# wjmaddox/online_gp

Measured on AMD Instinct MI355X. Metric: streaming updates/sec (WISKI, 50^3 inducing grid), higher is better.
Workload: dtype f32

## Files before the change

include/wiski.h:

```cpp
#ifndef WISKI_H
#define WISKI_H

#include <stdint.h>

#ifdef __cplusplus
extern "C" {
#endif

#define WISKI_OK 0
#define WISKI_E_BADARG (-1)
#define WISKI_E_LAUNCH (-2)
#define WISKI_E_WORKSPACE (-3)
#define WISKI_E_NOTCONV (-4)
#define WISKI_PENDING 1

#define WISKI_MAX_DIM 4

typedef struct wiski_grid {
  int32_t d;
  int32_t g[WISKI_MAX_DIM];
  double g0[WISKI_MAX_DIM];
  double h[WISKI_MAX_DIM];
} wiski_grid;

int wiski_version(void);
int wiski_side_stream_create(int32_t lowest_priority, void** out);

int wiski_interp_f32(const wiski_grid* grid, const float* d_x, int64_t n, int32_t* d_idx, float* d_val, int32_t* d_err, void* stream);
int wiski_interp_f64(const wiski_grid* grid, const double* d_x, int64_t n, int32_t* d_idx, double* d_val, int32_t* d_err, void* stream);

int wiski_gather_f32(const wiski_grid* grid, const float* d_x, int64_t n, const float* d_V, int32_t k, int32_t diag, float* d_out, int32_t* d_err, void* stream);
int wiski_gather_f64(const wiski_grid* grid, const double* d_x, int64_t n, const double* d_V, int32_t k, int32_t diag, double* d_out, int32_t* d_err, void* stream);

int wiski_gather_grad_f32(const wiski_grid* grid, const float* d_x, int64_t n, const float* d_V, int32_t diag, float* d_out, void* stream);
int wiski_gather_grad_f64(const wiski_grid* grid, const double* d_x, int64_t n, const double* d_V, int32_t diag, double* d_out, void* stream);

int wiski_gather_rows_f32(const wiski_grid* grid, const float* d_x, int64_t n, const float* d_Vr, int32_t ncols, float* d_out, int32_t* d_err, void* stream);
int wiski_gather_rows_f64(const wiski_grid* grid, const double* d_x, int64_t n, const double* d_Vr, int32_t ncols, double* d_out, int32_t* d_err, void* stream);
int wiski_gather_rows_vjp_f32(const wiski_grid* grid, const float* d_x, int64_t n, const float* d_Vr, int32_t ncols, const float* d_G, float* d_gx, void* stream);
int wiski_gather_rows_vjp_f64(const wiski_grid* grid, const double* d_x, int64_t n, const double* d_Vr, int32_t ncols, const double* d_G, double* d_gx, void* stream);
int wiski_interp_bilinear_f32(const wiski_grid* grid, const float* d_A, int64_t lda, const float* d_xL, int32_t qL, const float* d_xR, int32_t qR, int64_t nbatch, float* d_out, int32_t* d_err, void* stream);
int wiski_interp_bilinear_f64(const wiski_grid* grid, const double* d_A, int64_t lda, const double* d_xL, int32_t qL, const double* d_xR, int32_t qR, int64_t nbatch, double* d_out, int32_t* d_err, void* stream);
int wiski_interp_bilinear_vjp_f32(const wiski_grid* grid, const float* d_A, int64_t lda, const float* d_xL, int32_t qL, const float* d_xR, int32_t qR, int64_t nbatch, const float* d_G, float* d_gxL, float* d_gxR, void* stream);
int wiski_interp_bilinear_vjp_f64(const wiski_grid* grid, const double* d_A, int64_t lda, const double* d_xL, int32_t qL, const double* d_xR, int32_t qR, int64_t nbatch, const double* d_G, double* d_gxL, double* d_gxR, void* stream);

int wiski_gather_ell_f32(const int32_t* d_idx, const float* d_val, int64_t n, int32_t T, const float* d_v, float* d_out, void* stream);
int wiski_gather_ell_f64(const int32_t* d_idx, const double* d_val, int64_t n, int32_t T, const double* d_v, double* d_out, void* stream);
int wiski_gather_ell_grid_f32(const wiski_grid* grid, const int32_t* d_idx, const float* d_val, int64_t n, const float* d_v, float* d_vpack, float* d_out, void* stream);
int wiski_gather_ell_grid_f64(const wiski_grid* grid, const int32_t* d_idx, const double* d_val, int64_t n, const double* d_v, double* d_vpack, double* d_out, void* stream);
int64_t wiski_gather_ell_pack_elems(const wiski_grid* grid);

int wiski_scatter_stats_f32(const wiski_grid* grid, const float* d_x, const float* d_y, const float* d_wa, const float* d_wb, const float* d_noise, int64_t n, float* d_b, float* d_A_st, double* d_stats, int32_t* d_err, void* stream);
int wiski_scatter_stats_f64(const wiski_grid* grid, const double* d_x, const double* d_y, const double* d_wa, const double* d_wb, const double* d_noise, int64_t n, double* d_b, double* d_A_st, double* d_stats, int32_t* d_err, void* stream);

int wiski_scatter_stats_sym_f32(const wiski_grid* grid, const float* d_x, const float* d_y, const float* d_wa, const float* d_wb, const float* d_noise, int64_t n, float* d_b, float* d_A_half, double* d_stats, int32_t* d_err, void* stream);
int wiski_scatter_stats_sym_f64(const wiski_grid* grid, const double* d_x, const double* d_y, const double* d_wa, const double* d_wb, const double* d_noise, int64_t n, double* d_b, double* d_A_half, double* d_stats, int32_t* d_err, void* stream);
int wiski_scatter_stats_cnt_f32(const wiski_grid* grid, const float* d_x, const float* d_y, const float* d_wa, const float* d_wb, const float* d_noise, int64_t n, float* d_b, float* d_A, int32_t half, float* d_cnt, const float* d_u, float* d_res, double* d_stats, int32_t* d_err, void* stream);
int wiski_scatter_stats_cnt_f64(const wiski_grid* grid, const double* d_x, const double* d_y, const double* d_wa, const double* d_wb, const double* d_noise, int64_t n, double* d_b, double* d_A, int32_t half, double* d_cnt, const double* d_u, double* d_res, double* d_stats, int32_t* d_err, void* stream);
int wiski_stencil_expand_add_f32(const wiski_grid* grid, float* d_A_half, float* d_A_st, void* stream);
int wiski_stencil_expand_add_f64(const wiski_grid* grid, double* d_A_half, double* d_A_st, void* stream);

int wiski_wt_columns_f32(const wiski_grid* grid, const float* d_x, int64_t n, float* d_out, int32_t* d_err, void* stream);
int wiski_wt_columns_f64(const wiski_grid* grid, const double* d_x, int64_t n, double* d_out, int32_t* d_err, void* stream);

int wiski_jet_quadform_f32(const wiski_grid* grid, const float* d_x, int64_t n, const float* d_M, int64_t ldm, float* d_out, int32_t* d_err, void* stream);
int wiski_jet_quadform_f64(const wiski_grid* grid, const double* d_x, int64_t n, const double* d_M, int64_t ldm, double* d_out, int32_t* d_err, void* stream);
int wiski_wt_columns_jet_f32(const wiski_grid* grid, const float* d_x, int64_t n, float* d_out, int32_t* d_err, void* stream);
int wiski_wt_columns_jet_f64(const wiski_grid* grid, const double* d_x, int64_t n, double* d_out, int32_t* d_err, void* stream);
int wiski_gather_jet_f32(const wiski_grid* grid, const float* d_x, int64_t n, const float* d_V, int32_t k, int32_t rows_per_point, float* d_out, int32_t* d_err, void* stream);
int wiski_gather_jet_f64(const wiski_grid* grid, const double* d_x, int64_t n, const double* d_V, int32_t k, int32_t rows_per_point, double* d_out, int32_t* d_err, void* stream);

int wiski_stencil_spmv_f32(const wiski_grid* grid, const float* d_A_st, const float* d_V, int32_t k, const float* d_add, float beta, float* d_out, void* stream);
int wiski_stencil_spmv_f64(const wiski_grid* grid, const double* d_A_st, const double* d_V, int32_t k, const double* d_add, double beta, double* d_out, void* stream);
int wiski_stencil_spmv_sym_f32(const wiski_grid* grid, const float* d_A_half, const float* d_V, int32_t k, const float* d_add, float beta, float* d_out, void* stream);
int wiski_stencil_spmv_sym_f64(const wiski_grid* grid, const double* d_A_half, const double* d_V, int32_t k, const double* d_add, double beta, double* d_out, void* stream);

int wiski_kron_toeplitz_mm_f32(const wiski_grid* grid, const float* d_tcol, const float* d_V, int32_t k, float scale, float* d_tmp, float* d_out, void* stream);
int wiski_kron_toeplitz_mm_f64(const wiski_grid* grid, const double* d_tcol, const double* d_V, int32_t k, double scale, double* d_tmp, double* d_out, void* stream);

int wiski_kron_toeplitz_grad_f32(const wiski_grid* grid, const float* d_tcol, const float* d_X, const float* d_Y, int32_t k, float* d_tmp, double* d_grad, void* stream);
int wiski_kron_toeplitz_grad_f64(const wiski_grid* grid, const double* d_tcol, const double* d_X, const double* d_Y, int32_t k, double* d_tmp, double* d_grad, void* stream);

int wiski_kron_spectral_mm_f32(const wiski_grid* grid, const float* d_evec, const float* d_eval, float kscale, float shift, float pw, float rw, const float* d_V, int32_t k, float* d_tmp, float* d_out, void* stream);
int wiski_kron_spectral_mm_f64(const wiski_grid* grid, const double* d_evec, const double* d_eval, double kscale, double shift, double pw, double rw, const double* d_V, int32_t k, double* d_tmp, double* d_out, void* stream);

int64_t wiski_pcg_workspace_bytes(const wiski_grid* grid, int32_t k, int32_t max_iter, int32_t elem_size);
int wiski_pcg_f32(const wiski_grid* grid, const float* d_A_st, const float* d_tcol, float kscale, const float* d_evec, const float* d_evec2, const float* d_eval, float shift, const float* d_RHS, int32_t k, float* d_U, float* d_Z, int32_t warm, double tol, int32_t max_iter, int32_t check_every, int32_t first_check, void* d_work, int64_t work_bytes, int32_t* h_iters, double* h_relres, const int32_t* d_err, int32_t* h_err, int32_t a_sym, float* d_R, void* stream);
int wiski_pcg_f64(const wiski_grid* grid, const double* d_A_st, const double* d_tcol, double kscale, const double* d_evec, const double* d_evec2, const double* d_eval, double shift, const double* d_RHS, int32_t k, double* d_U, double* d_Z, int32_t warm, double tol, int32_t max_iter, int32_t check_every, int32_t first_check, void* d_work, int64_t work_bytes, int32_t* h_iters, double* h_relres, const int32_t* d_err, int32_t* h_err, int32_t a_sym, double* d_R, void* stream);

typedef int (*wiski_allreduce_fn)(void* ctx, void* d_vec, int64_t n_vec, int32_t elem_bytes, double* d_dots, int64_t n_dots, void* stream);
typedef struct wiski_shard {
  int32_t rank, nranks;
  void* comm;
  wiski_allreduce_fn allreduce;
  void* ctx;
} wiski_shard;
int wiski_shard_groups(int32_t d, int32_t rank, int32_t nranks, int32_t* g_lo, int32_t* g_hi);

typedef struct wiski_twolevel {
  int32_t r;
  int32_t nslab;
  const uint64_t* d_mask;
  const int32_t* d_off;
  const uint16_t* d_pos;
  const float* d_N;
  uint64_t* d_cs;
  float* d_mc;
  int32_t mc_cols;
} wiski_twolevel;

typedef struct wiski_pcg_async {
  int32_t state;
  int32_t it;
  int64_t seq;
  void* poll;
  int32_t prezeroed;
  int32_t guard_ok;
  double shift;
} wiski_pcg_async;
int wiski_pcg_async_f32(const wiski_grid* grid, const float* d_A_st, const float* d_tcol, float kscale, const float* d_evec, const float* d_evec2, const float* d_eval, float shift, const float* d_RHS, int32_t k, float* d_U, float* d_Z, int32_t warm, double tol, int32_t max_iter, int32_t check_every, int32_t first_check, void* d_work, int64_t work_bytes, int32_t* h_iters, double* h_relres, const int32_t* d_err, int32_t* h_err, int32_t a_sym, float* d_R, void* stream, wiski_pcg_async* handle, int32_t mode);
int wiski_pcg_async_f64(const wiski_grid* grid, const double* d_A_st, const double* d_tcol, double kscale, const double* d_evec, const double* d_evec2, const double* d_eval, double shift, const double* d_RHS, int32_t k, double* d_U, double* d_Z, int32_t warm, double tol, int32_t max_iter, int32_t check_every, int32_t first_check, void* d_work, int64_t work_bytes, int32_t* h_iters, double* h_relres, const int32_t* d_err, int32_t* h_err, int32_t a_sym, double* d_R, void* stream, wiski_pcg_async* handle, int32_t mode);
int wiski_pcg_async_free(wiski_pcg_async* handle);
int wiski_pcg_async_guard(const wiski_pcg_async* handle, const void** d_guard, int64_t* expect);
int wiski_pcg_zero_regions_f32(const wiski_grid* grid, int32_t k, int32_t max_iter, void* d_work, int32_t a_sym, void** p1, int64_t* n1_bytes, void** p2, int64_t* n2_bytes);
int wiski_pcg_zero_regions_f64(const wiski_grid* grid, int32_t k, int32_t max_iter, void* d_work, int32_t a_sym, void** p1, int64_t* n1_bytes, void** p2, int64_t* n2_bytes);
int64_t wiski_scatter_bin_bytes(const wiski_grid* grid, int64_t n, int32_t elem_size);
int wiski_scatter_stats_step_f32(const wiski_grid* grid, const float* d_x, const float* d_y, const float* d_wa, const float* d_wb, const float* d_noise, int64_t n, float* d_b, float* d_A_half, float* d_cnt, const float* d_u, float* d_res, float* d_mean_out, double* d_stats, int32_t* d_err, void* z1, int64_t n1_bytes, void* z2, int64_t n2_bytes, const void* d_guard, int64_t guard_expect, void* d_bin, int64_t bin_bytes, void* stream);
int wiski_scatter_stats_step_f64(const wiski_grid* grid, const double* d_x, const double* d_y, const double* d_wa, const double* d_wb, const double* d_noise, int64_t n, double* d_b, double* d_A_half, double* d_cnt, const double* d_u, double* d_res, double* d_mean_out, double* d_stats, int32_t* d_err, void* z1, int64_t n1_bytes, void* z2, int64_t n2_bytes, const void* d_guard, int64_t guard_expect, void* d_bin, int64_t bin_bytes, void* stream);
int wiski_gather_zero_f32(const wiski_grid* grid, const float* d_x, int64_t n, const float* d_V, int32_t k, float* d_out, int32_t* d_err, void* z1, int64_t n1_bytes, void* z2, int64_t n2_bytes, int32_t* zeroed, void* stream);
int wiski_gather_zero_f64(const wiski_grid* grid, const double* d_x, int64_t n, const double* d_V, int32_t k, double* d_out, int32_t* d_err, void* z1, int64_t n1_bytes, void* z2, int64_t n2_bytes, int32_t* zeroed, void* stream);

typedef struct wiski_stream_args_f32 {
  float* d_A_half; float* d_b; float* d_cnt; double* d_stats; int32_t* d_err;
  float* d_U; float* d_Z; float* d_R;
  const float* d_tcol; float kscale; const float* d_evec; const float* d_evec2; const float* d_eval; float shift;
  double tol; int32_t max_iter; int32_t check_every; void* d_work; int64_t work_bytes;
  void* d_bin; int64_t bin_bytes;
  const wiski_shard* shard;
  const wiski_twolevel* two_level;
  int32_t keep[3];
} wiski_stream_args_f32;
typedef struct wiski_stream_args_f64 {
  double* d_A_half; double* d_b; double* d_cnt; double* d_stats; int32_t* d_err;
  double* d_U; double* d_Z; double* d_R;
  const double* d_tcol; double kscale; const double* d_evec; const double* d_evec2; const double* d_eval; double shift;
  double tol; int32_t max_iter; int32_t check_every; void* d_work; int64_t work_bytes;
  void* d_bin; int64_t bin_bytes;
  const wiski_shard* shard;
  const wiski_twolevel* two_level;
  int32_t keep[3];
} wiski_stream_args_f64;
int wiski_stream_step_f32(const wiski_grid* grid, const wiski_stream_args_f32* args, const float* d_x, const float* d_y, const float* d_wa, const float* d_wb, const float* d_noise, int64_t q, float* d_mean_out, int32_t carry, int32_t first_check, int32_t* h_iters, double* h_relres, int32_t* h_err, void* stream, wiski_pcg_async* handle, int32_t defer, int32_t* h_resumed);
int wiski_stream_step_f64(const wiski_grid* grid, const wiski_stream_args_f64* args, const double* d_x, const double* d_y, const double* d_wa, const double* d_wb, const double* d_noise, int64_t q, double* d_mean_out, int32_t carry, int32_t first_check, int32_t* h_iters, double* h_relres, int32_t* h_err, void* stream, wiski_pcg_async* handle, int32_t defer, int32_t* h_resumed);

int wiski_scatter_stats_multi_f32(const wiski_grid* grid, const float* d_x, const float* d_y, const float* d_wa, const float* d_wb, const float* d_noise, int64_t n, int32_t nout, int64_t y_stride, int64_t w_stride, float* d_b, float* d_A_half, int64_t A_stride, float* d_cnt, const float* d_u, float* d_res, double* d_stats, int32_t* d_err, void* stream);
int wiski_scatter_stats_multi_f64(const wiski_grid* grid, const double* d_x, const double* d_y, const double* d_wa, const double* d_wb, const double* d_noise, int64_t n, int32_t nout, int64_t y_stride, int64_t w_stride, double* d_b, double* d_A_half, int64_t A_stride, double* d_cnt, const double* d_u, double* d_res, double* d_stats, int32_t* d_err, void* stream);

int wiski_scatter_stats_grad_f32(const wiski_grid* grid, const float* d_x, const float* d_y, const float* d_wa, const float* d_wb, const float* d_noise, int64_t n, float* d_b, float* d_A_half, float* d_cnt, const float* d_u, float* d_res, float* d_mean_out, double* d_stats, int32_t* d_err, void* stream);
int wiski_scatter_stats_grad_f64(const wiski_grid* grid, const double* d_x, const double* d_y, const double* d_wa, const double* d_wb, const double* d_noise, int64_t n, double* d_b, double* d_A_half, double* d_cnt, const double* d_u, double* d_res, double* d_mean_out, double* d_stats, int32_t* d_err, void* stream);

typedef struct wiski_absorb_args {
  const void* d_x; const void* d_y; const void* d_wa; const void* d_wb; const void* d_noise; int64_t n;
  void* d_b; void* d_A; int32_t half; int32_t channels; void* d_cnt; double* d_stats; int32_t* d_err;
  const void* d_u; void* d_res; void* d_mean_out;
  void* z1; int64_t n1_bytes; void* z2; int64_t n2_bytes;
  const void* d_guard; int64_t guard_expect;
  void* d_bin; int64_t bin_bytes;
  int32_t g_lo; int32_t g_hi; int32_t nout; int32_t reserved;
  int64_t y_stride; int64_t w_stride; int64_t A_stride;
} wiski_absorb_args;
int wiski_absorb_f32(const wiski_grid* grid, const wiski_absorb_args* args, void* stream);
int wiski_absorb_f64(const wiski_grid* grid, const wiski_absorb_args* args, void* stream);

int wiski_scatter_stats_robust_f32(const wiski_grid* grid, const float* d_x, const float* d_y, const float* d_wa, const float* d_wb, const float* d_noise, int64_t n, float* d_b, float* d_A_half, float* d_cnt, const float* d_u, float* d_res, float* d_mean_out, double* d_stats, int32_t* d_err, const float* d_inv_scale, float huber_c, float* d_omega_out, void* stream);
int wiski_scatter_stats_robust_f64(const wiski_grid* grid, const double* d_x, const double* d_y, const double* d_wa, const double* d_wb, const double* d_noise, int64_t n, double* d_b, double* d_A_half, double* d_cnt, const double* d_u, double* d_res, double* d_mean_out, double* d_stats, int32_t* d_err, const double* d_inv_scale, double huber_c, double* d_omega_out, void* stream);
int wiski_absorb_robust_f32(const wiski_grid* grid, const wiski_absorb_args* args, const float* d_inv_scale, float huber_c, float* d_omega_out, void* stream);
int wiski_absorb_robust_f64(const wiski_grid* grid, const wiski_absorb_args* args, const double* d_inv_scale, double huber_c, double* d_omega_out, void* stream);

typedef struct wiski_window_ring {
  void* d_x; void* d_y; void* d_wa; void* d_wb; void* d_noise;
  int64_t cap; int64_t head;
} wiski_window_ring;
int wiski_scatter_stats_window_f32(const wiski_grid* grid, const float* d_x, const float* d_y, const float* d_wa, const float* d_wb, const float* d_noise, int64_t n, const wiski_window_ring* ring, float* d_b, float* d_A_half, float* d_cnt, const float* d_u, float* d_res, float* d_mean_out, double* d_stats, int32_t* d_err, int32_t* d_void_left, void* stream);
int wiski_scatter_stats_window_f64(const wiski_grid* grid, const double* d_x, const double* d_y, const double* d_wa, const double* d_wb, const double* d_noise, int64_t n, const wiski_window_ring* ring, double* d_b, double* d_A_half, double* d_cnt, const double* d_u, double* d_res, double* d_mean_out, double* d_stats, int32_t* d_err, int32_t* d_void_left, void* stream);
int wiski_absorb_window_f32(const wiski_grid* grid, const wiski_absorb_args* args, const wiski_window_ring* ring, int32_t* d_void_left, void* stream);
int wiski_absorb_window_f64(const wiski_grid* grid, const wiski_absorb_args* args, const wiski_window_ring* ring, int32_t* d_void_left, void* stream);

int wiski_scatter_stats_step_sharded_f32(const wiski_grid* grid, const float* d_x, const float* d_y, const float* d_wa, const float* d_wb, const float* d_noise, int64_t n, float* d_b, float* d_A_half, float* d_cnt, const float* d_u, float* d_res, float* d_mean_out, double* d_stats, int32_t* d_err, void* z1, int64_t n1_bytes, void* z2, int64_t n2_bytes, const void* d_guard, int64_t guard_expect, int32_t g_lo, int32_t g_hi, void* stream);
int wiski_scatter_stats_step_sharded_f64(const wiski_grid* grid, const double* d_x, const double* d_y, const double* d_wa, const double* d_wb, const double* d_noise, int64_t n, double* d_b, double* d_A_half, double* d_cnt, const double* d_u, double* d_res, double* d_mean_out, double* d_stats, int32_t* d_err, void* z1, int64_t n1_bytes, void* z2, int64_t n2_bytes, const void* d_guard, int64_t guard_expect, int32_t g_lo, int32_t g_hi, void* stream);
int wiski_pcg_sharded_f32(const wiski_grid* grid, const float* d_A_st, const float* d_tcol, float kscale, const float* d_evec, const float* d_evec2, const float* d_eval, float shift, const float* d_RHS, int32_t k, float* d_U, float* d_Z, int32_t warm, double tol, int32_t max_iter, int32_t check_every, int32_t first_check, void* d_work, int64_t work_bytes, int32_t* h_iters, double* h_relres, const int32_t* d_err, int32_t* h_err, int32_t a_sym, float* d_R, void* stream, wiski_pcg_async* handle, int32_t mode, const wiski_shard* shard);
int wiski_pcg_sharded_f64(const wiski_grid* grid, const double* d_A_st, const double* d_tcol, double kscale, const double* d_evec, const double* d_evec2, const double* d_eval, double shift, const double* d_RHS, int32_t k, double* d_U, double* d_Z, int32_t warm, double tol, int32_t max_iter, int32_t check_every, int32_t first_check, void* d_work, int64_t work_bytes, int32_t* h_iters, double* h_relres, const int32_t* d_err, int32_t* h_err, int32_t a_sym, double* d_R, void* stream, wiski_pcg_async* handle, int32_t mode, const wiski_shard* shard);
int wiski_pcg_twolevel_f32(const wiski_grid* grid, const float* d_A_st, const float* d_tcol, float kscale, const float* d_evec, const float* d_evec2, const float* d_eval, float shift, const float* d_RHS, int32_t k, float* d_U, float* d_Z, int32_t warm, double tol, int32_t max_iter, int32_t check_every, int32_t first_check, void* d_work, int64_t work_bytes, int32_t* h_iters, double* h_relres, const int32_t* d_err, int32_t* h_err, int32_t a_sym, float* d_R, void* stream, wiski_pcg_async* handle, int32_t mode, const wiski_shard* shard, const wiski_twolevel* two_level);
int64_t wiski_twolevel_refresh_workspace_bytes(int32_t r);
int wiski_twolevel_refresh_f32(const wiski_grid* grid, const float* d_x, int64_t n, const float* d_scale, const double* d_V, int32_t kw, const int32_t* d_S, int32_t r, const double* d_lam_unit, double kscale, double gscale, double* d_G, void* d_work, int64_t work_bytes, float* d_N, const uint64_t* d_sticky, int32_t* d_bad, void* stream);
int wiski_precond_apply_f32(const wiski_grid* grid, const float* d_evec, const float* d_evec2, const float* d_eval, float kscale, float shift, const float* d_r, float* d_w0, float* d_w1, float* d_y, float* d_t, double* d_rho, const wiski_twolevel* two_level, void* stream);
int wiski_precond_apply_keep_f32(const wiski_grid* grid, const float* d_evec, const float* d_evec2, const float* d_eval, float kscale, float shift, const float* d_r, float* d_w0, float* d_w1, float* d_y, float* d_t, double* d_rho, const wiski_twolevel* two_level, const int32_t* keep, void* stream);
int wiski_precond_keep_ok(const wiski_grid* grid, const int32_t* keep, int32_t with_two_level);
int wiski_precond_apply_cols_f32(const wiski_grid* grid, const float* d_evec, const float* d_evec2, const float* d_eval, float kscale, float shift, const float* d_r, int32_t k, float* d_w0, float* d_w1, float* d_y, float* d_t, double* d_rho, const wiski_twolevel* two_level, void* stream);

int wiski_gemm_f32(int32_t ta, int32_t tb, int32_t M, int32_t N, int32_t K, float alpha, const float* d_A, int32_t lda, const float* d_B, int32_t ldb, float beta, float* d_C, int32_t ldc, void* stream);
int wiski_gemm_f64(int32_t ta, int32_t tb, int32_t M, int32_t N, int32_t K, double alpha, const double* d_A, int32_t lda, const double* d_B, int32_t ldb, double beta, double* d_C, int32_t ldc, void* stream);
int wiski_potrf_f32(int32_t n, float* d_A, int32_t lda, int32_t* d_info, void* stream);
int wiski_potrf_f64(int32_t n, double* d_A, int32_t lda, int32_t* d_info, void* stream);
int wiski_potrf_inverse_f32(int32_t n, float* d_A, int32_t lda, float* d_X, int32_t ldx, int32_t* d_info, void* stream);
int wiski_potrf_inverse_f64(int32_t n, double* d_A, int32_t lda, double* d_X, int32_t ldx, int32_t* d_info, void* stream);
int wiski_trsm_f32(int32_t trans, int32_t n, int32_t nrhs, const float* d_L, int32_t ldl, float* d_B, int32_t ldb, void* stream);
int wiski_trsm_f64(int32_t trans, int32_t n, int32_t nrhs, const double* d_L, int32_t ldl, double* d_B, int32_t ldb, void* stream);
int wiski_logdiag_f32(int32_t n, const float* d_A, int32_t lda, double* d_out, void* stream);
int wiski_logdiag_f64(int32_t n, const double* d_A, int32_t lda, double* d_out, void* stream);

int wiski_dense_factor_f32(const wiski_grid* grid, const float* d_A_half, const float* d_evec, const float* d_eval, float kscale, float* d_work, int64_t work_elems, float* d_chol, float* d_M, double* d_logdiag, int32_t* d_info, void* stream);
int wiski_dense_factor_f64(const wiski_grid* grid, const double* d_A_half, const double* d_evec, const double* d_eval, double kscale, double* d_work, int64_t work_elems, double* d_chol, double* d_M, double* d_logdiag, int32_t* d_info, void* stream);

int64_t wiski_root_update_workspace_elems(int32_t m, int32_t r, int32_t q);
int wiski_root_update_f32(int32_t m, int32_t r, int32_t q, float* d_L, int32_t ldl, float* d_R, int32_t ldr, const float* d_V, int32_t ldv, float* d_ws, int64_t ws_elems, void* stream);
int wiski_root_update_f64(int32_t m, int32_t r, int32_t q, double* d_L, int32_t ldl, double* d_R, int32_t ldr, const double* d_V, int32_t ldv, double* d_ws, int64_t ws_elems, void* stream);

int wiski_basis_project_f32(const wiski_grid* grid, const float* d_x, int64_t n, const double* d_V, int32_t kmax, const int32_t* d_S, int32_t r, const float* d_scale, const double* d_colscale, const double* d_tcol, double* d_F, int64_t ldf, double* d_prior, int32_t* d_err, void* stream);
int wiski_basis_project_f64(const wiski_grid* grid, const double* d_x, int64_t n, const double* d_V, int32_t kmax, const int32_t* d_S, int32_t r, const double* d_scale, const double* d_colscale, const double* d_tcol, double* d_F, int64_t ldf, double* d_prior, int32_t* d_err, void* stream);
int wiski_basis_project_vjp_f32(const wiski_grid* grid, const float* d_x, int64_t n, const double* d_V, int32_t kmax, const int32_t* d_S, int32_t r, const float* d_scale, const double* d_colscale, const double* d_tcol, const double* d_GF, int64_t ldg, const double* d_Gprior, float* d_gx, void* stream);
int wiski_basis_project_vjp_f64(const wiski_grid* grid, const double* d_x, int64_t n, const double* d_V, int32_t kmax, const int32_t* d_S, int32_t r, const double* d_scale, const double* d_colscale, const double* d_tcol, const double* d_GF, int64_t ldg, const double* d_Gprior, double* d_gx, void* stream);
int wiski_basis_absorb_h_f32(int64_t n, int32_t r, const double* d_F, int64_t ldf, const float* d_wby, const float* d_scale, double* d_h, void* stream);
int wiski_basis_absorb_h_f64(int64_t n, int32_t r, const double* d_F, int64_t ldf, const double* d_wby, const double* d_scale, double* d_h, void* stream);
int wiski_factor_refresh_layout(int32_t d, int64_t nV, int32_t kw, int32_t r_ref, int32_t r, int64_t* off);
int wiski_factor_refresh(int32_t d, const int32_t* d_g, int64_t nV, const double* d_tcol, const double* d_Vin, int32_t kw, int32_t kuse, const double* d_Vref, int32_t kref, int32_t niter, double resid_ok, const int32_t* d_Sref, const int32_t* d_S, int32_t r_ref, int32_t r, double* d_work, double* d_verdict, const double* d_Gref, const double* d_href, double kscale, int32_t* d_info, double* d_out, void* verdict_event, void* stream);
int wiski_basis_pair_reduce(int32_t d, int32_t r, int32_t kmax, const double* d_Wt, const int32_t* d_S, const double* d_ev, double* d_D, void* stream);
int wiski_basis_eig_update(int32_t d, const int32_t* d_g, const double* d_tcol, const double* d_Vin, int32_t kw, int32_t kuse, double* d_Vout, double* d_ev, double* d_resid,
                           const double* d_Vref, int32_t kref, double* d_Tq, void* stream);
int wiski_basis_eig_update_adaptive(int32_t d, const int32_t* d_g, const double* d_tcol, const double* d_Vin, int32_t kw, int32_t kuse, double* d_Vout, double* d_ev, double* d_resid, const double* d_Vref, int32_t kref, double* d_Tq, int32_t niter, double resid_ok, void* stream);
int wiski_basis_change(int32_t d, const int32_t* d_g, int32_t kref, int32_t kw, int32_t r_ref, int32_t r, const double* d_Tq, const int32_t* d_Sref, const int32_t* d_S, const double* d_ev, const double* d_tcol, const double* d_resid, double* d_TS, double* d_lam, double* d_work, double* d_verdict, void* stream);
int wiski_basis_lag_grad(int32_t d, const int32_t* d_g, int32_t kw, const double* d_V, const double* d_D, double scale, const double* d_scale, double* d_out, void* stream);
int wiski_spectral_var(int32_t n, int32_t r, const double* d_Y, const double* d_F, const double* d_prior, double kscale, double* d_diag, double* d_tail, void* stream);
#define WISKI_HYPER_MAX_PARAMS 6
typedef struct {
  void* raw;
  void* exp_avg;
  void* exp_avg_sq;
  void* step;
  int32_t numel;
  int32_t step_numel;
  int32_t role;
  int32_t kind;
  double lower, upper;
} wiski_hyper_param;
typedef struct {
  int32_t count;
  int32_t reserved;
  wiski_hyper_param p[WISKI_HYPER_MAX_PARAMS];
} wiski_hyper_plan;
int wiski_hyper_columns_f32(const wiski_hyper_plan* plan, const wiski_grid* grid, int32_t kind, float* d_ell, float* d_scale, float* d_s2, double* d_s2_f64, double* d_tcol64, float* d_tcol, void* stream);
int wiski_hyper_columns_f64(const wiski_hyper_plan* plan, const wiski_grid* grid, int32_t kind, double* d_ell, double* d_scale, double* d_s2, double* d_s2_f64, double* d_tcol64, double* d_tcol, void* stream);
int wiski_hyper_mid_f32(const double* d_bMb, const double* d_logdet, const float* d_s2, const double* d_c, const double* d_ld, const double* d_n, double* d_out, double* d_loss, void* stream);
int wiski_hyper_mid_f64(const double* d_bMb, const double* d_logdet, const double* d_s2, const double* d_c, const double* d_ld, const double* d_n, double* d_out, double* d_loss, void* stream);
int wiski_hyper_adam_f32(const wiski_hyper_plan* plan, const float* d_scale, const float* d_s2, const float* d_gell, const float* d_gscale, const double* d_mid, const double* d_gkap, const double* d_n, double lr, double beta1, double beta2, double eps, void* stream);
int wiski_hyper_adam_f64(const wiski_hyper_plan* plan, const double* d_scale, const double* d_s2, const double* d_gell, const double* d_gscale, const double* d_mid, const double* d_gkap, const double* d_n, double lr, double beta1, double beta2, double eps, void* stream);
#define WISKI_COPY_MAX_SEGMENTS 12
typedef struct {
  const void* src[WISKI_COPY_MAX_SEGMENTS];
  void* dst[WISKI_COPY_MAX_SEGMENTS];
  int64_t n[WISKI_COPY_MAX_SEGMENTS];
  int32_t count;
  int32_t reserved;
  double scalar;
  void* scalar_dst;
} wiski_copy_plan;
int wiski_multi_copy_f64(const wiski_copy_plan* plan, void* stream);
int wiski_spectral_evaluate_f32(int32_t n, int32_t r, const double* d_F, const double* d_prior, const double* d_Linv, int32_t ldl, const double* d_t, double kscale, const float* d_s2, const float* d_y, const int32_t* d_err, double* d_ws, double* d_out, float* d_mean, float* d_var, void* stream);
int wiski_spectral_evaluate_f64(int32_t n, int32_t r, const double* d_F, const double* d_prior, const double* d_Linv, int32_t ldl, const double* d_t, double kscale, const double* d_s2, const double* d_y, const int32_t* d_err, double* d_ws, double* d_out, double* d_mean, double* d_var, void* stream);
int wiski_spectral_evaluate_y_f32(int32_t n, int32_t r, const double* d_Y, const double* d_F, const double* d_prior, const double* d_t, double kscale, const float* d_s2, const float* d_y, const int32_t* d_err, double* d_ws, double* d_out, float* d_mean, float* d_var, void* stream);
int wiski_spectral_evaluate_y_f64(int32_t n, int32_t r, const double* d_Y, const double* d_F, const double* d_prior, const double* d_t, double kscale, const double* d_s2, const double* d_y, const int32_t* d_err, double* d_ws, double* d_out, double* d_mean, double* d_var, void* stream);
int wiski_factor_tail(int32_t r_ref, int32_t r, const double* d_TS, const double* d_href, const double* d_sq, const double* d_Linv, const double* d_chol, double* d_out, void* stream);
int wiski_woodbury_c(int32_t r, const double* d_G, const double* d_lam_kuu, double kscale, double* d_C, double* d_lam, double* d_sq, double* d_sqG, void* stream);
int wiski_mll_weights(int32_t r, const double* d_G, const double* d_P, const double* d_zeta, const double* d_lam_kuu, const double* d_gb, const double* d_gld, double* d_Wt, double* d_gkap, void* stream);

int wiski_comm_unique_id_bytes(void);
int wiski_comm_unique_id(void* id_out);
int wiski_comm_init_rank(const void* id_bytes, int32_t nranks, int32_t rank, void** comm_out);
int wiski_comm_destroy(void* comm);
int wiski_comm_info(void* comm, int32_t* version_out, int32_t* nranks_out, int32_t* rank_out);
int wiski_allreduce_stats_f32(void* comm, float* d_half, int64_t n_half, float* d_b, int64_t n_b, float* d_cnt, int64_t n_cnt, double* d_scal, int64_t n_scal, void* stream);
int wiski_allreduce_stats_f64(void* comm, double* d_half, int64_t n_half, double* d_b, int64_t n_b, double* d_cnt, int64_t n_cnt, double* d_scal, int64_t n_scal, void* stream);

int wiski_read_flag(const int32_t* d_flag, int32_t* h_value, void* stream);

int wiski_prof_start(int32_t max_launches);
int wiski_prof_stop(double* total_ms, int64_t* launches);
int wiski_prof_stamps(double* total_ms, int64_t* launches, double* each_us, int64_t each_cap);
int wiski_prof_stamps_raw(int64_t i, uint64_t* pairs, int64_t cap, int64_t* nwaves);
int wiski_prof_enable(int32_t on);
int wiski_prof_empty(int32_t n, double* avg_us, void* stream);

int wiski_stationary_columns_f32(const wiski_grid* grid, int32_t kind, const float* d_ell, int32_t nell, const float* d_scale, double* d_out, void* stream);
int wiski_stationary_columns_f64(const wiski_grid* grid, int32_t kind, const double* d_ell, int32_t nell, const double* d_scale, double* d_out, void* stream);
int wiski_stationary_columns_grad_f32(const wiski_grid* grid, int32_t kind, const float* d_ell, int32_t nell, const float* d_scale, const double* d_gout, float* d_gell, float* d_gscale, void* stream);
int wiski_stationary_columns_grad_f64(const wiski_grid* grid, int32_t kind, const double* d_ell, int32_t nell, const double* d_scale, const double* d_gout, double* d_gell, double* d_gscale, void* stream);
int wiski_mll_value_f32(const double* d_bMb, const double* d_logdet, const float* d_s2, const double* d_c, const double* d_ld, double n, const double* d_n, double* d_val, double* d_coef, void* stream);
int wiski_mll_value_f64(const double* d_bMb, const double* d_logdet, const double* d_s2, const double* d_c, const double* d_ld, double n, const double* d_n, double* d_val, double* d_coef, void* stream);
int wiski_mll_s2_grad_f32(const double* d_g, const double* d_coef, const float* d_s2, double n, const double* d_n, const double* d_gkap, float* d_gs2, void* stream);
int wiski_mll_s2_grad_f64(const double* d_g, const double* d_coef, const double* d_s2, double n, const double* d_n, const double* d_gkap, double* d_gs2, void* stream);
int wiski_gaussian_metrics_f32(int64_t n, const float* d_mu, const float* d_var, const float* d_y, const float* d_add_var, float* d_out, void* stream);
int wiski_gaussian_metrics_f64(int64_t n, const double* d_mu, const double* d_var, const double* d_y, const double* d_add_var, double* d_out, void* stream);

int wiski_scatter_probes_f32(const wiski_grid* grid, const float* d_x, const float* d_wa, int64_t q, int64_t first_index, uint64_t seed, int32_t S, float* d_P, int32_t* d_err, void* stream);
// ... 32 lines not shown
```

online_gp_amd/csrc/pcg.h:

```cpp
#pragma once
#include "wiski_common.h"

template <typename real>
struct PcgArgs {
  const real* A = nullptr;
  bool a_sym = false;
  const real* RHS = nullptr;
  int k = 0;
  const real* tcol = nullptr;
  real kscale = (real)0;
  const real* evec = nullptr;
  const real* evec2 = nullptr;
  const real* eval = nullptr;
  real shift = (real)0;
  const wiski_twolevel* two_level = nullptr;
  int keep[3] = {0, 0, 0};
  real* U = nullptr;
  real* Z = nullptr;
  real* R = nullptr;
  int warm = 0;
  double tol = 0;
  int max_iter = 0;
  int check_every = 0;
  int first_check = 0;
  void* work = nullptr;
  int64_t work_bytes = 0;
  int32_t* h_iters = nullptr;
  double* h_relres = nullptr;
  const int32_t* d_err = nullptr;
  int32_t* h_err = nullptr;
  wiski_pcg_async* handle = nullptr;
  int mode = 0;
  const wiski_shard* shard = nullptr;
};

template <typename real>
struct PcgLayout {
  static constexpr int SLOTS = 20;
  static int64_t align(int64_t v) { return (v + 255) / 256 * 256; }
  static int64_t bytes(int m, int k, int max_iter, int elem_size = (int)sizeof(real)) {
    return SLOTS * align((int64_t)k * m * elem_size) + align(PcgScal::doubles(k, max_iter) * 8);
  }
  real *r, *y, *p, *pt, *hp, *tmp;
  real* part;
  real* ty;
  real *sa, *sb;
  PcgScal S;
  int64_t km;
  int64_t nscal;
  PcgLayout(int m, int k, int max_iter, void* work) : km((int64_t)k * m), nscal(PcgScal::doubles(k, max_iter)) {
    char* w = static_cast<char*>(work);
    const int64_t vec = align(km * (int64_t)sizeof(real));
    auto at = [&](int slot) { return reinterpret_cast<real*>(w + slot * vec); };
    r = at(0); y = at(1); p = at(2); pt = at(3); hp = at(4); tmp = at(5); part = at(6); ty = at(14); sa = at(16); sb = at(18);
    double* base = reinterpret_cast<double*>(at(SLOTS));
    S = PcgScal{base, k, base + PcgScal::scalars(k, max_iter)};
  }
  double* zero1() const { return S.base; }
  int64_t zero1_count() const { return nscal; }
  real* zero2(int nch) const { return part + (int64_t)(nch > 0 ? nch - 1 : 0) * km; }
  int64_t zero2_count(int zl) const { return zl ? km : 0; }
};

template <typename real>
int pcg(const wiski_grid* grid, const PcgArgs<real>& args, void* stream);

template <typename real>
int pcg_zero_regions(const wiski_grid* grid, int k, int max_iter, void* work, bool a_sym, void** p1, int64_t* n1_bytes, void** p2, int64_t* n2_bytes);
int pcg_guard(const wiski_pcg_async* handle, const void** d_guard, int64_t* expect);
```

online_gp_amd/csrc/solve.hip:

```cpp
#include "pcg.h"

#include <hip/hip_ext.h>

#include <chrono>
#include <cstdlib>
#include <map>
#include <mutex>
#include <vector>

static struct WiskiProf {
  bool on = false;
  bool armed = false;
  std::vector<hipEvent_t> ev;
  size_t used = 0;
  unsigned long long* d_stamp = nullptr;
  size_t stamp_pairs = 0, stamp_used = 0;
  struct Span { size_t off, n; };
  std::vector<Span> spans;
} g_prof;
constexpr unsigned long long PROF_CLOCK_MASK = 0xffffffffffffull;
constexpr size_t PROF_STAMP_ARENA_PAIRS = (size_t)1 << 20;

extern "C" int wiski_prof_start(int max_launches) {
  if (max_launches < 1) return WISKI_E_BADARG;
  while (g_prof.ev.size() < (size_t)max_launches * 2) {
    hipEvent_t e;
    if (hipEventCreate(&e) != hipSuccess) return WISKI_E_LAUNCH;
    g_prof.ev.push_back(e);
  }
  if (!g_prof.d_stamp) {
    if (hipMalloc(&g_prof.d_stamp, PROF_STAMP_ARENA_PAIRS * 2 * sizeof(unsigned long long)) == hipSuccess) g_prof.stamp_pairs = PROF_STAMP_ARENA_PAIRS;
    else { (void)hipGetLastError(); g_prof.d_stamp = nullptr; }
  }
  if (g_prof.d_stamp && g_prof.stamp_used &&
      hipMemset(g_prof.d_stamp, 0, g_prof.stamp_used * 2 * sizeof(unsigned long long)) != hipSuccess) return WISKI_E_LAUNCH;
  if (g_prof.d_stamp && !g_prof.stamp_used && hipMemset(g_prof.d_stamp, 0, g_prof.stamp_pairs * 2 * sizeof(unsigned long long)) != hipSuccess) return WISKI_E_LAUNCH;
  g_prof.stamp_used = 0;
  g_prof.spans.clear();
  g_prof.used = 0;
  g_prof.on = true;
  g_prof.armed = true;
  return WISKI_OK;
}

extern "C" int wiski_prof_enable(int32_t on) {
  g_prof.on = on != 0;
  return WISKI_OK;
}

static inline unsigned long long* prof_stamp_pairs(size_t nwaves) {
  static const bool off = getenv("WISKI_PROF_NOSTAMP") != nullptr;
  if (off || !g_prof.armed || !g_prof.d_stamp || g_prof.stamp_used + nwaves > g_prof.stamp_pairs) return nullptr;
  g_prof.spans.push_back(WiskiProf::Span{g_prof.stamp_used, nwaves});
  g_prof.stamp_used += nwaves;
  return g_prof.d_stamp + 2 * g_prof.spans.back().off;
}

extern "C" int wiski_prof_stop(double* total_ms, int64_t* launches) {
  g_prof.on = false;
  g_prof.armed = false;
  double tot = 0;
  for (size_t i = 0; i + 1 < g_prof.used; i += 2) {
    float ms = 0;
    if (hipEventElapsedTime(&ms, g_prof.ev[i], g_prof.ev[i + 1]) != hipSuccess) return WISKI_E_LAUNCH;
    tot += ms;
  }
  if (total_ms) *total_ms = tot;
  if (launches) *launches = (int64_t)(g_prof.used / 2);
  g_prof.used = 0;
  return WISKI_OK;
}

extern "C" int wiski_prof_stamps(double* total_ms, int64_t* launches, double* each_us, int64_t each_cap) {
  const size_t nd = g_prof.spans.size();
  double tot = 0;
  int64_t cnt = 0;
  if (nd && g_prof.d_stamp && g_prof.stamp_used) {
    std::vector<unsigned long long> h(2 * g_prof.stamp_used);
    if (hipMemcpy(h.data(), g_prof.d_stamp, h.size() * sizeof(unsigned long long), hipMemcpyDeviceToHost) != hipSuccess) return WISKI_E_LAUNCH;
    for (size_t i = 0; i < nd; ++i) {
      const WiskiProf::Span sp = g_prof.spans[i];
      unsigned long long lo = ~0ull, hi = 0;
      for (size_t w = 0; w < sp.n; ++w) {
        unsigned long long b = h[2 * (sp.off + w)] & PROF_CLOCK_MASK, e = h[2 * (sp.off + w) + 1];
        if (!e) continue;
        if (e < b) e += PROF_CLOCK_MASK + 1;
        if (b < lo) lo = b;
        if (e > hi) hi = e;
      }
      if (hi > lo) {
        if (each_us && cnt < each_cap) each_us[cnt] = (double)(hi - lo) * 1e-2;
        tot += (double)(hi - lo) * 1e-5;
        ++cnt;
      }
    }
  }
  if (total_ms) *total_ms = tot;
  if (launches) *launches = cnt;
  return WISKI_OK;
}

extern "C" int wiski_prof_stamps_raw(int64_t i, uint64_t* pairs, int64_t cap, int64_t* nwaves) {
  if (!nwaves || i < 0) return WISKI_E_BADARG;
  *nwaves = 0;
  if ((size_t)i >= g_prof.spans.size() || !g_prof.d_stamp) return WISKI_OK;
  const WiskiProf::Span sp = g_prof.spans[(size_t)i];
  *nwaves = (int64_t)sp.n;
  if (!pairs || !sp.n) return WISKI_OK;
  const size_t n = (size_t)cap < sp.n ? (size_t)cap : sp.n;
  if (hipMemcpy(pairs, g_prof.d_stamp + 2 * sp.off, n * 2 * sizeof(unsigned long long), hipMemcpyDeviceToHost) != hipSuccess) return WISKI_E_LAUNCH;
  return WISKI_OK;
}

__global__ void k_prof_empty() {}
extern "C" int wiski_prof_empty(int32_t n, double* avg_us, void* stream) {
  if (n < 1 || !avg_us) return WISKI_E_BADARG;
  hipStream_t s = (hipStream_t)stream;
  std::vector<hipEvent_t> ev(2 * (size_t)n);
  for (auto& e : ev)
    if (hipEventCreate(&e) != hipSuccess) return WISKI_E_LAUNCH;
  for (int i = 0; i < n; ++i) hipExtLaunchKernelGGL(k_prof_empty, dim3(1), dim3(64), 0, s, ev[2 * i], ev[2 * i + 1], 0);
  int rc = hipStreamSynchronize(s) == hipSuccess ? WISKI_OK : WISKI_E_LAUNCH;
  double tot = 0;
  for (int i = 0; i < n && rc == WISKI_OK; ++i) {
    float ms = 0;
    if (hipEventElapsedTime(&ms, ev[2 * i], ev[2 * i + 1]) != hipSuccess) rc = WISKI_E_LAUNCH;
    tot += ms;
  }
  for (auto& e : ev) (void)hipEventDestroy(e);
  *avg_us = tot * 1e3 / n;
  return rc;
}

template <typename real, int KC, bool DOT>
__global__ __launch_bounds__(256) void k_stencil_spmv(GridDev<real> G, const real* __restrict__ A_st, const real* __restrict__ V,
                                                      int k, const real* __restrict__ add, real beta, real* __restrict__ out,
                                                      double* __restrict__ dots) {
  extern __shared__ __attribute__((aligned(16))) char smem[];
  int* s_off = reinterpret_cast<int*>(smem);
  const int R = G.R, m = G.m, d = G.d;
  for (int o = threadIdx.x; o < R; o += blockDim.x) {
    int rem = o, f = 0;
    for (int q = d - 1; q >= 0; --q) {
      int c = rem % 7;
      rem /= 7;
      f += (c - 3) * G.stride[q];
    }
    s_off[o] = f;
  }
  __syncthreads();
  const int i = blockIdx.x * blockDim.x + threadIdx.x;
  const int c0 = blockIdx.y * KC;
  real acc[KC];
#pragma unroll
  for (int c = 0; c < KC; ++c) acc[c] = (real)0;
  if (i < m) {
// ... 1349 lines not shown
        const Vec4<real> r4 = load4<real>(r + e);
        rr[0] = r4.x; rr[1] = r4.y; rr[2] = r4.z; rr[3] = r4.w;
      } else {
      Vec4<real> t4;
      t4.x = t4.y = t4.z = t4.w = (real)0;
      if (t) t4 = load4<real>(t + e);
      Vec4<real> pp[8];
#pragma unroll
      for (int ch = 0; ch < 8; ++ch)
        if (ch < nch) pp[ch] = load4<real>(part + (int64_t)ch * km + e);
      if (zl) store4<real>(part + (int64_t)(nch - 1) * km + e, (real)0, (real)0, (real)0, (real)0);
      rr[0] = f[0] - t4.x; rr[1] = f[1] - t4.y; rr[2] = f[2] - t4.z; rr[3] = f[3] - t4.w;
#pragma unroll
      for (int ch = 0; ch < 8; ++ch)
        if (ch < nch) { rr[0] -= pp[ch].x; rr[1] -= pp[ch].y; rr[2] -= pp[ch].z; rr[3] -= pp[ch].w; }
      store4<real>(r + e, rr[0], rr[1], rr[2], rr[3]);
      }
    } else {
      f[0] = rhs[e];
      if (given) {
        rr[0] = r[e];
      } else {
        rr[0] = t ? f[0] - t[e] : f[0];
        for (int ch = 0; ch < nch; ++ch) rr[0] -= part[(int64_t)ch * km + e];
        if (zl) part[(int64_t)(nch - 1) * km + e] = (real)0;
        r[e] = rr[0];
      }
    }
#pragma unroll
    for (int q = 0; q < VEC; ++q) {
      a += (double)f[q] * f[q];
      bsum += (double)rr[q] * rr[q];
    }
  }
  a = block_reduce_sum(a, s_red);
  bsum = block_reduce_sum(bsum, s_red);
  if (threadIdx.x == 0) {
    unsafeAtomicAdd(S.rn0() + c, a);
    unsafeAtomicAdd(S.rn(0) + c, bsum);
  }
}


template <typename real, int VEC>
__global__ __launch_bounds__(256) void k_pcg_update_p(int m, int it, double tol2, const real* __restrict__ y, const real* __restrict__ r,
                                                      real* __restrict__ p, real* __restrict__ pt, PcgScal S) {
  const int c = blockIdx.y;
  double beta = 0;
  if (it > 0) {
    const double den = S.rho(it - 1)[c];
    beta = den > 0 ? S.rho(it)[c] / den : 0;
  }
  const real bt = (real)beta;
  const int64_t cm = (int64_t)c * m;
  for (int i = (blockIdx.x * blockDim.x + threadIdx.x) * VEC; i < m; i += gridDim.x * blockDim.x * VEC) {
    real yv[VEC], rv[VEC], pv[VEC], ptv[VEC];
    if constexpr (VEC == 4) {
      const Vec4<real> a = load4<real>(y + cm + i), b = load4<real>(r + cm + i);
      yv[0] = a.x; yv[1] = a.y; yv[2] = a.z; yv[3] = a.w;
      rv[0] = b.x; rv[1] = b.y; rv[2] = b.z; rv[3] = b.w;
      if (it > 0) {
        const Vec4<real> cpp = load4<real>(p + cm + i), dpp = load4<real>(pt + cm + i);
        pv[0] = cpp.x; pv[1] = cpp.y; pv[2] = cpp.z; pv[3] = cpp.w;
        ptv[0] = dpp.x; ptv[1] = dpp.y; ptv[2] = dpp.z; ptv[3] = dpp.w;
      }
    } else {
      yv[0] = y[cm + i]; rv[0] = r[cm + i];
      if (it > 0) { pv[0] = p[cm + i]; ptv[0] = pt[cm + i]; }
    }
#pragma unroll
    for (int u = 0; u < VEC; ++u) {
      pv[u] = it == 0 ? yv[u] : yv[u] + bt * pv[u];
      ptv[u] = it == 0 ? rv[u] : rv[u] + bt * ptv[u];
    }
    if constexpr (VEC == 4) {
      store4<real>(p + cm + i, pv[0], pv[1], pv[2], pv[3]);
      store4<real>(pt + cm + i, ptv[0], ptv[1], ptv[2], ptv[3]);
    } else {
      p[cm + i] = pv[0]; pt[cm + i] = ptv[0];
    }
  }
}

template <typename real, int VEC>
__global__ __launch_bounds__(256) void k_pcg_update_x(int m, int it, double tol2, const real* __restrict__ p, const real* __restrict__ pt,
                                                      const real* __restrict__ hp, real* __restrict__ part, int nch, int zl,
                                                      real* __restrict__ u, real* __restrict__ z, real* __restrict__ r, PcgScal S,
                                                      double* __restrict__ poll = nullptr, const int32_t* __restrict__ err = nullptr,
                                                      long long seq = 0, long long* __restrict__ guard = nullptr) {
  __shared__ double s_red[16];
  const int c = blockIdx.y;
  double alpha = 0;
  const double den = S.php_sum(it, c);
  if (blockIdx.x == 0) pcg_dot_clear(S.php(it + 1), c, 1, S.k);
  if (pcg_active(S, it, c, tol2) && den > 0) alpha = S.rho(it)[c] / den;
  const real al = (real)alpha;
  double acc = 0;
  const int64_t cm = (int64_t)c * m;
  const int64_t km = (int64_t)S.k * m;
  for (int i = (blockIdx.x * blockDim.x + threadIdx.x) * VEC; i < m; i += gridDim.x * blockDim.x * VEC) {
    const int64_t e = cm + i;
    real pv[VEC], ptv[VEC], hv[VEC], uv[VEC], zv[VEC], rv[VEC];
    if constexpr (VEC == 4) {
      const Vec4<real> a = load4<real>(p + e), b = load4<real>(pt + e), cu = load4<real>(u + e), cz = load4<real>(z + e), cr = load4<real>(r + e);
      pv[0] = a.x; pv[1] = a.y; pv[2] = a.z; pv[3] = a.w;
      ptv[0] = b.x; ptv[1] = b.y; ptv[2] = b.z; ptv[3] = b.w;
      uv[0] = cu.x; uv[1] = cu.y; uv[2] = cu.z; uv[3] = cu.w;
      zv[0] = cz.x; zv[1] = cz.y; zv[2] = cz.z; zv[3] = cz.w;
      rv[0] = cr.x; rv[1] = cr.y; rv[2] = cr.z; rv[3] = cr.w;
      if (nch > 0) {
        Vec4<real> pp[8];
#pragma unroll
        for (int ch = 0; ch < 8; ++ch)
          if (ch < nch) pp[ch] = load4<real>(part + (int64_t)ch * km + e);
        if (zl) store4<real>(part + (int64_t)(nch - 1) * km + e, (real)0, (real)0, (real)0, (real)0);
#pragma unroll
        for (int q = 0; q < 4; ++q) hv[q] = ptv[q];
#pragma unroll
        for (int ch = 0; ch < 8; ++ch)
          if (ch < nch) { hv[0] += pp[ch].x; hv[1] += pp[ch].y; hv[2] += pp[ch].z; hv[3] += pp[ch].w; }
      } else {
        const Vec4<real> h4 = load4<real>(hp + e);
        hv[0] = h4.x; hv[1] = h4.y; hv[2] = h4.z; hv[3] = h4.w;
      }
    } else {
      pv[0] = p[e]; ptv[0] = pt[e]; uv[0] = u[e]; zv[0] = z[e]; rv[0] = r[e];
      if (nch > 0) {
        hv[0] = ptv[0];
        for (int ch = 0; ch < nch; ++ch) hv[0] += part[(int64_t)ch * km + e];
        if (zl) part[(int64_t)(nch - 1) * km + e] = (real)0;
      } else {
        hv[0] = hp[e];
      }
    }
#pragma unroll
    for (int q = 0; q < VEC; ++q) {
      uv[q] += al * pv[q];
      zv[q] += al * ptv[q];
      rv[q] -= al * hv[q];
      acc += (double)rv[q] * rv[q];
    }
    if constexpr (VEC == 4) {
      store4<real>(u + e, uv[0], uv[1], uv[2], uv[3]);
      store4<real>(z + e, zv[0], zv[1], zv[2], zv[3]);
      store4<real>(r + e, rv[0], rv[1], rv[2], rv[3]);
    } else {
      u[e] = uv[0]; z[e] = zv[0]; r[e] = rv[0];
    }
  }
  acc = block_reduce_sum(acc, s_red);
  if (poll == nullptr) {
    if (threadIdx.x == 0) unsafeAtomicAdd(S.rn(it + 1) + c, acc);
  } else {
    __shared__ int s_last;
    if (threadIdx.x == 0) {
      const double prev = atomicAdd(S.rn(it + 1) + c, acc);
      unsigned one = 1u;
      asm volatile("" : "+v"(one) : "v"(prev));
      const unsigned t = atomicAdd(S.ticket(), one);
      s_last = t == gridDim.x * gridDim.y - 1;
    }
    __syncthreads();
    if (s_last) {
      const int k = S.k;
      int ok = 1;
      for (int c2 = threadIdx.x; c2 < k; c2 += blockDim.x) {
        const double r0 = __hip_atomic_load(S.rn0() + c2, __ATOMIC_RELAXED, __HIP_MEMORY_SCOPE_AGENT);
        const double r1 = __hip_atomic_load(S.rn(it + 1) + c2, __ATOMIC_RELAXED, __HIP_MEMORY_SCOPE_AGENT);
        poll[1 + c2] = r0;
        poll[1 + k + c2] = r1;
        if (r0 > 0 && r1 > tol2 * r0) ok = 0;
      }
      ok = __syncthreads_and(ok);
      if (threadIdx.x == 0) {
        const double e = err ? (double)*err : 0.0;
        const long long gv = (ok && e == 0.0) ? seq : -seq;
        poll[1 + 2 * k] = e;
        poll[2 + 2 * k] = (double)gv;
        if (guard) *guard = gv;
        __hip_atomic_store(S.ticket(), 0u, __ATOMIC_RELAXED, __HIP_MEMORY_SCOPE_AGENT);
      }
      __threadfence_system();
      __syncthreads();
      if (threadIdx.x == 0) __hip_atomic_store(reinterpret_cast<long long*>(poll), seq, __ATOMIC_RELEASE, __HIP_MEMORY_SCOPE_SYSTEM);
    }
  }
}

template <typename real>
__global__ __launch_bounds__(256) void k_shard_reduce(int m4, int m, const real* __restrict__ part, int np, real* __restrict__ acc,
                                                      real* __restrict__ out) {
  for (int i = blockIdx.x * blockDim.x + threadIdx.x; i < m4; i += gridDim.x * blockDim.x) {
    Vec4<real> t = load4<real>(acc + 4 * i);
    for (int p = 0; p < np; ++p) {
      const Vec4<real> v = load4<real>(part + (int64_t)p * m + 4 * i);
      t.x += v.x; t.y += v.y; t.z += v.z; t.w += v.w;
    }
    store4<real>(out + 4 * i, t.x, t.y, t.z, t.w);
    store4<real>(acc + 4 * i, (real)0, (real)0, (real)0, (real)0);
  }
}


struct PcgPath {
  bool wide;
  bool sym;
  bool spectral;
  bool fused_cg;
  bool sharded;
  template <typename real>
  PcgPath(const GridDev<real>& G, const PcgArgs<real>& a)
      : wide(G.m % 4 == 0), sym(a.a_sym), spectral(a.evec != nullptr && a.eval != nullptr), fused_cg(spectral && wide && spectral_fused_ok<real>(G)),
        sharded(wiski_shard_active(a.shard)) {}
};

template <typename real>
static int pcg_validate(const GridDev<real>& G, const PcgArgs<real>& a, const PcgPath& path) {
  if (!a.A || !a.RHS || !a.U || !a.Z || !a.work || a.k < 1 || a.max_iter < 1) return WISKI_E_BADARG;
  if (a.mode != 0 && !a.handle) return WISKI_E_BADARG;
  if (a.mode == 2 && a.handle->state != 1) return WISKI_E_BADARG;
  if (!path.spectral && !a.tcol) return WISKI_E_BADARG;
  if (a.work_bytes < PcgLayout<real>::bytes(G.m, a.k, a.max_iter)) return WISKI_E_WORKSPACE;
  if (path.sharded) {
    if (!path.sym || !path.wide || a.k != 1 || a.shard->rank < 0 || a.shard->rank >= a.shard->nranks) return WISKI_E_BADARG;
    if (!a.shard->comm && !a.shard->allreduce) return WISKI_E_BADARG;
  }
  if (a.mode != 2 && a.warm == 2 && !a.R) return WISKI_E_BADARG;
  if (a.two_level && !(path.fused_cg && sizeof(real) == 4)) return WISKI_E_BADARG;
  if (a.keep[0] != 0 || a.keep[1] != 0 || a.keep[2] != 0) {
    if constexpr (sizeof(real) == 4) {
      if (!path.fused_cg || a.k != 1 || !spectral_keep_ok(G, a.keep, a.two_level != nullptr)) return WISKI_E_BADARG;
    } else {
      return WISKI_E_BADARG;
    }
  }
  return WISKI_OK;
}

template <typename real>
static int pcg_partials(const GridDev<real>& G, int k, bool sym, int* zl) {
  *zl = 0;
  if (G.m % 4 != 0) return 0;
  return sym ? sym_partials<real>(G, k, zl) : spmv_nch(G.d);
}

template <typename real>
struct PcgPlan {
  const GridDev<real>& G;
  const PcgArgs<real>& a;
  const PcgPath path;
  const hipStream_t s;
  const int m, k;
  const PcgLayout<real> L;
  real* r;
  int nch, zl;
  SymDmaParts stab{};
  int sh_lo = 0, sh_hi = 0;
  bool sh_dma = false;
  real* cpart;
  int cnch, czl;
  dim3 egrid, vgrid;
  const double tol2;
  bool init_in_fwd;

  PcgPlan(const GridDev<real>& G_, const PcgArgs<real>& a_, const PcgPath& path_, hipStream_t s_)
      : G(G_), a(a_), path(path_), s(s_), m(G_.m), k(a_.k), L(G_.m, a_.k, a_.max_iter, a_.work), tol2(a_.tol * a_.tol) {
    r = a.R ? a.R : L.r;
    nch = pcg_partials<real>(G, k, path.sym, &zl);
    if (path.sharded) {
      shard_group_range(sym_groups(G.d), a.shard->rank, a.shard->nranks, &sh_lo, &sh_hi);
      sh_dma = sym_use_dma<real>(G, k);
      if (sh_dma) shard_parts_d3(sh_lo, sh_hi, &stab);
    }
    cpart = path.sharded ? L.hp : L.part;
    cnch = path.sharded ? 1 : nch;
    czl = path.sharded ? 0 : zl;
    int bcap = m / 4096;
    bcap = bcap < 32 ? 32 : (bcap > 256 ? 256 : bcap);
    if (k < 16 && bcap < 1024 / k) bcap = 1024 / k;
    int eb = (m + 255) / 256;
    if (eb > bcap) eb = bcap;
    egrid = dim3((unsigned)eb, (unsigned)k);
    int vb = (m / 4 + 255) / 256;
    if (vb < 1) vb = 1;
    if (vb > bcap) vb = bcap;
    vgrid = dim3((unsigned)vb, (unsigned)k);
    init_in_fwd = a.mode != 2 && a.warm == 2 && sizeof(real) == 4 && path.fused_cg;
  }

  int product_wide(const real* v, const real* add, real beta, double* dots) const {
    real* part = L.part;
    if (!path.sharded)
      return path.sym ? launch_spmv4_sym<real>(G, a.A, v, k, part, add, beta, dots, s) : launch_spmv4<real>(G, a.A, v, k, part, add, beta, dots, s);
    int np = 0;
    if (sh_dma) {
      if (stab.n) {
        if (int r1 = launch_spmv4_sym<real>(G, a.A, v, k, part, add, beta, dots, s, &stab)) return r1;
      }
      np = stab.n;
    } else if (sh_hi > sh_lo) {
      if (int r1 = launch_spmv4_sym<real>(G, a.A, v, k, part, add, beta, dots, s, nullptr, sh_lo, sh_hi)) return r1;
      np = nch - 1;
    }
    const int m4 = m / 4;
    hipLaunchKernelGGL((k_shard_reduce<real>), dim3((unsigned)((m4 + 255) / 256)), dim3(256), 0, s, m4, m, (const real*)part, np,
                       part + (int64_t)(nch - 1) * k * m, L.hp);
    if (hipGetLastError() != hipSuccess) return WISKI_E_LAUNCH;
    const int64_t nd = dots ? (int64_t)k * PCG_DOT_COL : 0;
    const wiski_shard* shard = a.shard;
    if (shard->comm) {
      if constexpr (sizeof(real) == 4) return wiski_allreduce_stats_f32(shard->comm, nullptr, 0, (float*)L.hp, m, nullptr, 0, dots, nd, s);
      else return wiski_allreduce_stats_f64(shard->comm, nullptr, 0, (double*)L.hp, m, nullptr, 0, dots, nd, s);
    }
    return shard->allreduce(shard->ctx, L.hp, (int64_t)m, (int32_t)sizeof(real), dots, nd, s);
  }
  int product(const real* v, const real* add, real beta, double* dots) const {
    if (path.wide) return product_wide(v, add, beta, dots);
    return path.sym ? launch_spmv_sym<real>(G, a.A, v, k, add, beta, L.hp, dots, s) : launch_spmv<real>(G, a.A, v, k, add, beta, L.hp, dots, s);
  }
};

#define PCG_VEC_LAUNCH(plan, K, ...)                                                                          \
  do {                                                                                                        \
    if ((plan).path.wide) hipLaunchKernelGGL((K<real, 4>), (plan).vgrid, dim3(256), 0, (plan).s, __VA_ARGS__); \
    else hipLaunchKernelGGL((K<real, 1>), (plan).egrid, dim3(256), 0, (plan).s, __VA_ARGS__);                  \
  } while (0)

template <typename real>
static int pcg_start(const PcgPlan<real>& plan) {
  const PcgArgs<real>& a = plan.a;
  const PcgLayout<real>& L = plan.L;
  const hipStream_t s = plan.s;
  const int m = plan.m, k = plan.k;
  if (a.handle && a.handle->prezeroed) {
    a.handle->prezeroed = 0;
  } else {
    const int64_t nscal = L.zero1_count(), nvec = L.zero2_count(plan.zl);
    int64_t zb = ((nscal > nvec ? nscal : nvec) + 255) / 256;
    if (zb > 1024) zb = 1024;
    hipLaunchKernelGGL((k_pcg_zero<real>), dim3((unsigned)zb), dim3(256), 0, s, L.zero1(), nscal, L.zero2(plan.nch), nvec);
  }
  if (a.warm == 2 && plan.init_in_fwd) {
  } else if (a.warm == 2) {
    PCG_VEC_LAUNCH(plan, k_pcg_init, m, a.RHS, (const real*)nullptr, (real*)nullptr, 0, 0, 1, plan.r, L.S);
  } else if (a.warm) {
    if (plan.path.wide) {
      if (int rc = plan.product(a.U, nullptr, (real)0, nullptr)) return rc;
      hipLaunchKernelGGL((k_pcg_init<real, 4>), plan.vgrid, dim3(256), 0, s, m, a.RHS, (const real*)a.Z, plan.cpart, plan.cnch, plan.czl, 0, plan.r, L.S);
    } else {
      if (int rc = plan.product(a.U, a.Z, (real)1, nullptr)) return rc;
      hipLaunchKernelGGL((k_pcg_init<real, 1>), plan.egrid, dim3(256), 0, s, m, a.RHS, (const real*)L.hp, (real*)nullptr, 0, 0, 0, plan.r, L.S);
    }
  } else {
    if (hipMemsetAsync(a.U, 0, (size_t)k * m * sizeof(real), s) != hipSuccess) return WISKI_E_LAUNCH;
    if (hipMemsetAsync(a.Z, 0, (size_t)k * m * sizeof(real), s) != hipSuccess) return WISKI_E_LAUNCH;
    hipLaunchKernelGGL((k_pcg_init<real, 1>), plan.egrid, dim3(256), 0, s, m, a.RHS, (const real*)nullptr, (real*)nullptr, 0, 0, 0, plan.r, L.S);
  }
  return WISKI_OK;
}

template <typename real>
static int pcg_iterate(const PcgPlan<real>& plan) {
  const GridDev<real>& G = plan.G;
  const PcgArgs<real>& a = plan.a;
  const PcgLayout<real>& L = plan.L;
  const PcgScal& S = L.S;
  const hipStream_t s = plan.s;
  const int m = plan.m, k = plan.k, max_iter = a.max_iter;
  const double tol2 = plan.tol2;
  const bool spectral = plan.path.spectral;
  real *const r = plan.r, *const p = L.p, *const pt = L.pt, *const hp = L.hp, *const cpart = plan.cpart;
  const int cnch = plan.cnch, czl = plan.czl;
  wiski_pcg_async* const as = a.handle;
  int mode = a.mode, first_check = a.first_check;
  const int check_every = a.check_every < 1 ? 10 : a.check_every;
  int rc = WISKI_OK;

  std::vector<double> h_rn0(k), h_rn(k);
  double err_seen = 0;
  int dev = 0;
  if (hipGetDevice(&dev) != hipSuccess) return WISKI_E_LAUNCH;
  std::unique_lock<std::mutex> poll_lock(g_poll_mu, std::defer_lock);
  WiskiPoll* Pp = nullptr;
  if (as) {
    if (!as->poll) as->poll = new WiskiPoll();
    Pp = static_cast<WiskiPoll*>(as->poll);
  } else {
    poll_lock.lock();
    Pp = &g_polls[dev];
  }
  WiskiPoll& P = *Pp;
  if (poll_reserve(P, k) != WISKI_OK) return WISKI_E_LAUNCH;
  auto collect = [&]() {
    for (int c = 0; c < k; ++c) {
      h_rn0[c] = P.h[1 + c];
      h_rn[c] = P.h[1 + k + c];
    }
    err_seen = P.h[1 + 2 * k];
  };
  bool deferred = false;
  auto fetch = [&](int slot, long long queued_seq = 0) -> int {
    long long seq = queued_seq;
    if (!seq) {
      seq = ++P.seq;
      hipLaunchKernelGGL(k_pcg_publish, dim3(1), dim3(64), 0, s, S, slot, P.d, a.d_err, seq, tol2, P.g);
    }
    if (hipGetLastError() != hipSuccess) return WISKI_E_LAUNCH;
    if (mode == 1) {
      as->state = 1;
      as->it = slot;
      as->seq = seq;
      deferred = true;
      return WISKI_OK;
    }
    if (int prc = poll_wait(P, seq, s)) return prc;
    collect();
    return WISKI_OK;
  };
  auto converged = [&]() {
    for (int c = 0; c < k; ++c)
      if (h_rn0[c] > 0 && h_rn[c] > tol2 * h_rn0[c]) return false;
    return true;
  };

  int it = 0;
  bool done = false;
  if (mode == 2) {
    it = as->it;
    as->state = 0;
    if (int prc = poll_wait(P, as->seq, s)) return prc;
    collect();
    as->guard_ok = (long long)P.h[2 + 2 * k] == as->seq ? 1 : 0;
    done = converged();
    first_check = it;
    mode = 0;
  }
  if (first_check < 1) first_check = check_every;
  if (first_check > max_iter) first_check = max_iter;
  auto due = [&](int i) { return i == max_iter || i == first_check || (i > first_check && (i - first_check) % check_every == 0); };
  bool pending = false;
  auto flush_update = [&](bool publish = false) -> long long {
    long long seq = 0;
    if (pending) {
      if (publish) seq = ++P.seq;
      hipLaunchKernelGGL((k_pcg_update_x<real, 4>), plan.vgrid, dim3(256), 0, s, m, it - 1, tol2, (const real*)p, (const real*)pt, (const real*)hp,
                         cpart, cnch, czl, a.U, a.Z, r, S, publish ? P.d : (double*)nullptr, a.d_err, seq, P.g);
      pending = false;
    }
    return seq;
  };
  while (!done && it < max_iter) {
    if (plan.path.fused_cg) {
      constexpr bool fuse_upd = sizeof(real) == 4;
      if (!fuse_upd) flush_update();
      const bool init_now = plan.init_in_fwd && it == 0;
      rc = launch_spectral_fused_cg<real>(G, a.evec, a.evec2, a.eval, a.kscale, a.shift, r, k, L.sa, L.sb, it, pending ? 1 : 0, tol2, p, pt, cpart, cnch,
                                          czl, a.U, a.Z, S, s, init_now ? a.RHS : (const real*)nullptr, a.two_level, a.keep);
      pending = false;
      if (rc) return rc;
      rc = plan.product_wide(p, pt, (real)1, S.php(it));
      if (rc) return rc;
      pending = true;
      ++it;
      if (due(it)) {
        rc = fetch(it, flush_update(true));
        if (rc) return rc;
        if (deferred) return WISKI_PENDING;
        done = converged();
      }
      continue;
    }
    if (spectral) {
      rc = launch_spectral_precond<real>(G, a.evec, a.evec2, a.eval, a.kscale, a.shift, r, k, L.sa, L.sb, L.ty, S.rho(it), s);
      if (rc) return rc;
      PCG_VEC_LAUNCH(plan, k_pcg_update_p, m, it, tol2, (const real*)(L.ty + (int64_t)k * m), (const real*)L.ty, p, pt, S);
    } else {
      rc = launch_kron<real>(G, a.tcol, r, k, a.kscale, L.tmp, L.y, r, S.rho(it), s);
      if (rc) return rc;
      PCG_VEC_LAUNCH(plan, k_pcg_update_p, m, it, tol2, (const real*)L.y, (const real*)r, p, pt, S);
    }
    rc = plan.product(p, pt, (real)1, S.php(it));
    if (rc) return rc;
    const bool pub = due(it + 1);
    const long long useq = pub ? ++P.seq : 0;
    PCG_VEC_LAUNCH(plan, k_pcg_update_x, m, it, tol2, (const real*)p, (const real*)pt, (const real*)hp, cpart, cnch, czl, a.U, a.Z, r, S,
                   pub ? P.d : (double*)nullptr, a.d_err, useq, P.g);
    ++it;
    if (due(it)) {
      rc = fetch(it, useq);
      if (rc) return rc;
      if (deferred) return WISKI_PENDING;
      done = converged();
    }
  }
  flush_update();
  if (hipGetLastError() != hipSuccess) return WISKI_E_LAUNCH;
  if (it == 0) {
    rc = fetch(0);
    if (rc) return rc;
  }
  if (a.h_iters) *a.h_iters = it;
  if (a.h_err) *a.h_err = (int32_t)err_seen;
  if (a.h_relres)
    for (int c = 0; c < k; ++c) a.h_relres[c] = h_rn0[c] > 0 ? sqrt(h_rn[c] / h_rn0[c]) : 0.0;
  return done ? WISKI_OK : WISKI_E_NOTCONV;
}
#undef PCG_VEC_LAUNCH

template <typename real>
int pcg(const wiski_grid* grid, const PcgArgs<real>& a, void* stream) {
  GridDev<real> G;
  int rc = make_grid_dev<real>(grid, &G);
  if (rc) return rc;
  const PcgPath path(G, a);
  rc = pcg_validate(G, a, path);
  if (rc) return rc;
  const PcgPlan<real> plan(G, a, path, (hipStream_t)stream);
  if (a.mode != 2) rc = pcg_start(plan);
  return rc ? rc : pcg_iterate(plan);
}
template int pcg<float>(const wiski_grid*, const PcgArgs<float>&, void*);
template int pcg<double>(const wiski_grid*, const PcgArgs<double>&, void*);

template <typename real>
static int spmv_impl(const wiski_grid* grid, const real* d_A, const real* d_V, int32_t k, const real* d_add, real beta, real* d_out, void* stream) {
  GridDev<real> G;
  int rc = make_grid_dev<real>(grid, &G);
  if (rc) return rc;
  if (!d_A || !d_V || !d_out || k < 1) return WISKI_E_BADARG;
  hipStream_t s = (hipStream_t)stream;
  if (G.m % 4 != 0) return launch_spmv<real>(G, d_A, d_V, k, d_add, beta, d_out, nullptr, s);
  const int nch = spmv_nch(G.d);
  const int64_t km = (int64_t)k * G.m;
  real* part = nullptr;
  if (hipMallocAsync((void**)&part, (size_t)nch * km * sizeof(real), s) != hipSuccess) return WISKI_E_LAUNCH;
  rc = launch_spmv4<real>(G, d_A, d_V, k, part, nullptr, (real)0, nullptr, s);
  if (rc == WISKI_OK) {
    int64_t blocks = (km + 255) / 256;
    if (blocks > 4096) blocks = 4096;
    hipLaunchKernelGGL((k_spmv_reduce<real>), dim3((unsigned)blocks), dim3(256), 0, s, km, nch, part, d_add, beta, d_out, 0);
    if (hipGetLastError() != hipSuccess) rc = WISKI_E_LAUNCH;
  }
  (void)hipFreeAsync(part, s);
  return rc;
}

template <typename real>
static int spmv_sym_impl(const wiski_grid* grid, const real* d_A, const real* d_V, int32_t k, const real* d_add, real beta, real* d_out, void* stream) {
  GridDev<real> G;
  int rc = make_grid_dev<real>(grid, &G);
  if (rc) return rc;
  if (!d_A || !d_V || !d_out || k < 1 || d_out == d_V) return WISKI_E_BADARG;
  hipStream_t s = (hipStream_t)stream;
  if (G.m % 4 != 0) return launch_spmv_sym<real>(G, d_A, d_V, k, d_add, beta, d_out, nullptr, s);
  int zl = 0;
  const int nch = sym_partials<real>(G, k, &zl);
  const int64_t km = (int64_t)k * G.m;
  real* part = nullptr;
  const int64_t slots = zl ? nch : 8;
  if (hipMallocAsync((void**)&part, (size_t)slots * km * sizeof(real), s) != hipSuccess) return WISKI_E_LAUNCH;
  if (zl && hipMemsetAsync(part + (int64_t)(nch - 1) * km, 0, (size_t)km * sizeof(real), s) != hipSuccess) rc = WISKI_E_LAUNCH;
#ifdef WISKI_PROBE_DOTS
  static double* probe_dots = nullptr;
  if (!probe_dots) { (void)hipMalloc((void**)&probe_dots, sizeof(double) * 2 * 64 * PCG_DOT_COL); (void)hipMemset(probe_dots, 0, sizeof(double) * 2 * 64 * PCG_DOT_COL); }
  if (rc == WISKI_OK) rc = launch_spmv4_sym<real>(G, d_A, d_V, k, part, d_V, (real)1, k <= 64 ? probe_dots : nullptr, s);
#else
  if (rc == WISKI_OK) rc = launch_spmv4_sym<real>(G, d_A, d_V, k, part, nullptr, (real)0, nullptr, s);
#endif
  if (rc == WISKI_OK) {
    int64_t blocks = (km + 255) / 256;
    if (blocks > 4096) blocks = 4096;
    hipLaunchKernelGGL((k_spmv_reduce<real>), dim3((unsigned)blocks), dim3(256), 0, s, km, nch, part, d_add, beta, d_out, 0);
    if (hipGetLastError() != hipSuccess) rc = WISKI_E_LAUNCH;
  }
  (void)hipFreeAsync(part, s);
  return rc;
}

template <typename real>
static int kron_impl(const wiski_grid* grid, const real* d_tcol, const real* d_V, int32_t k, real scale, real* d_tmp, real* d_out, void* stream) {
  GridDev<real> G;
  int rc = make_grid_dev<real>(grid, &G);
  if (rc) return rc;
  if (!d_tcol || !d_V || !d_out || k < 1 || d_out == d_V) return WISKI_E_BADARG;
  return launch_kron<real>(G, d_tcol, d_V, k, scale, d_tmp, d_out, nullptr, nullptr, (hipStream_t)stream);
}

template <typename real>
int pcg_zero_regions(const wiski_grid* grid, int k, int max_iter, void* work, bool a_sym, void** p1, int64_t* n1_bytes, void** p2, int64_t* n2_bytes) {
  GridDev<real> G;
  int rc = make_grid_dev<real>(grid, &G);
  if (rc) return rc;
  if (!work || !p1 || !n1_bytes || !p2 || !n2_bytes || k < 1 || max_iter < 1) return WISKI_E_BADARG;
  const PcgLayout<real> L(G.m, k, max_iter, work);
  int zl = 0;
  const int nch = pcg_partials<real>(G, k, a_sym, &zl);
  *p1 = L.zero1();
  *n1_bytes = L.zero1_count() * (int64_t)sizeof(double);
  *p2 = L.zero2(nch);
  *n2_bytes = L.zero2_count(zl) * (int64_t)sizeof(real);
  return WISKI_OK;
}
template int pcg_zero_regions<float>(const wiski_grid*, int, int, void*, bool, void**, int64_t*, void**, int64_t*);
template int pcg_zero_regions<double>(const wiski_grid*, int, int, void*, bool, void**, int64_t*, void**, int64_t*);

int pcg_guard(const wiski_pcg_async* as, const void** d_guard, int64_t* expect) {
  if (!as || !d_guard || !expect || as->state != 1 || !as->poll) return WISKI_E_BADARG;
  const WiskiPoll* P = static_cast<const WiskiPoll*>(as->poll);
  if (!P->g) return WISKI_E_BADARG;
  *d_guard = P->g;
  *expect = as->seq;
  return WISKI_OK;
}

#define PCG_ABI(real)                                                                                                                                           \
  const real* A, const real* tcol, real kscale, const real* evec, const real* evec2, const real* eval, real shift, const real* RHS, int32_t k, real* U, real* Z, \
      int32_t warm, double tol, int32_t max_iter, int32_t check_every, int32_t first_check, void* work, int64_t wb, int32_t* iters, double* relres,             \
      const int32_t* d_err, int32_t* h_err, int32_t a_sym, real* R
#define PCG_ABI_NAMES \
  A, tcol, kscale, evec, evec2, eval, shift, RHS, k, U, Z, warm, tol, max_iter, check_every, first_check, work, wb, iters, relres, d_err, h_err, a_sym, R
template <typename real>
static PcgArgs<real> pcg_args(PCG_ABI(real), wiski_pcg_async* as = nullptr, int32_t amode = 0, const wiski_shard* shard = nullptr,
                              const wiski_twolevel* two_level = nullptr) {
  PcgArgs<real> a;
  a.A = A; a.a_sym = a_sym != 0; a.RHS = RHS; a.k = k;
  a.tcol = tcol; a.kscale = kscale; a.evec = evec; a.evec2 = evec2; a.eval = eval; a.shift = shift; a.two_level = two_level;
  a.U = U; a.Z = Z; a.R = R; a.warm = warm;
  a.tol = tol; a.max_iter = max_iter; a.check_every = check_every; a.first_check = first_check;
  a.work = work; a.work_bytes = wb;
  a.h_iters = iters; a.h_relres = relres; a.d_err = d_err; a.h_err = h_err;
  a.handle = as; a.mode = amode;
  a.shard = shard;
  return a;
}

extern "C" {
int wiski_pcg_zero_regions_f32(const wiski_grid* g, int32_t k, int32_t max_iter, void* work, int32_t a_sym, void** p1, int64_t* n1, void** p2, int64_t* n2) { return pcg_zero_regions<float>(g, k, max_iter, work, a_sym != 0, p1, n1, p2, n2); }
int wiski_pcg_zero_regions_f64(const wiski_grid* g, int32_t k, int32_t max_iter, void* work, int32_t a_sym, void** p1, int64_t* n1, void** p2, int64_t* n2) { return pcg_zero_regions<double>(g, k, max_iter, work, a_sym != 0, p1, n1, p2, n2); }
int wiski_stencil_spmv_f32(const wiski_grid* g, const float* A, const float* V, int32_t k, const float* add, float beta, float* out, void* s) { return spmv_impl<float>(g, A, V, k, add, beta, out, s); }
int wiski_stencil_spmv_f64(const wiski_grid* g, const double* A, const double* V, int32_t k, const double* add, double beta, double* out, void* s) { return spmv_impl<double>(g, A, V, k, add, beta, out, s); }
int wiski_stencil_spmv_sym_f32(const wiski_grid* g, const float* A, const float* V, int32_t k, const float* add, float beta, float* out, void* s) { return spmv_sym_impl<float>(g, A, V, k, add, beta, out, s); }
int wiski_stencil_spmv_sym_f64(const wiski_grid* g, const double* A, const double* V, int32_t k, const double* add, double beta, double* out, void* s) { return spmv_sym_impl<double>(g, A, V, k, add, beta, out, s); }
int wiski_kron_toeplitz_mm_f32(const wiski_grid* g, const float* tcol, const float* V, int32_t k, float scale, float* tmp, float* out, void* s) { return kron_impl<float>(g, tcol, V, k, scale, tmp, out, s); }
int wiski_kron_toeplitz_mm_f64(const wiski_grid* g, const double* tcol, const double* V, int32_t k, double scale, double* tmp, double* out, void* s) { return kron_impl<double>(g, tcol, V, k, scale, tmp, out, s); }
int wiski_kron_toeplitz_grad_f32(const wiski_grid* g, const float* tcol, const float* X, const float* Y, int32_t k, float* tmp, double* grad, void* s) { return kron_grad_impl<float>(g, tcol, X, Y, k, tmp, grad, s); }
int wiski_kron_toeplitz_grad_f64(const wiski_grid* g, const double* tcol, const double* X, const double* Y, int32_t k, double* tmp, double* grad, void* s) { return kron_grad_impl<double>(g, tcol, X, Y, k, tmp, grad, s); }
int wiski_kron_spectral_mm_f32(const wiski_grid* g, const float* evec, const float* eval, float kscale, float shift, float pw, float rw, const float* V, int32_t k, float* tmp, float* out, void* s) { return spectral_mm_impl<float>(g, evec, eval, kscale, shift, pw, rw, V, k, tmp, out, s); }
int wiski_kron_spectral_mm_f64(const wiski_grid* g, const double* evec, const double* eval, double kscale, double shift, double pw, double rw, const double* V, int32_t k, double* tmp, double* out, void* s) { return spectral_mm_impl<double>(g, evec, eval, kscale, shift, pw, rw, V, k, tmp, out, s); }
int64_t wiski_pcg_workspace_bytes(const wiski_grid* grid, int32_t k, int32_t max_iter, int32_t elem_size) {
  if (!grid || grid->d < 1 || grid->d > WISKI_MAX_DIM || k < 1 || max_iter < 1) return WISKI_E_BADARG;
  int64_t m = 1;
  for (int q = 0; q < grid->d; ++q) m *= grid->g[q];
  return PcgLayout<float>::bytes((int)m, k, max_iter, elem_size);
}
int wiski_pcg_async_f32(const wiski_grid* g, PCG_ABI(float), void* s, wiski_pcg_async* as, int32_t amode) { return pcg(g, pcg_args<float>(PCG_ABI_NAMES, as, amode), s); }
int wiski_pcg_async_f64(const wiski_grid* g, PCG_ABI(double), void* s, wiski_pcg_async* as, int32_t amode) { return pcg(g, pcg_args<double>(PCG_ABI_NAMES, as, amode), s); }
int wiski_pcg_sharded_f32(const wiski_grid* g, PCG_ABI(float), void* s, wiski_pcg_async* as, int32_t amode, const wiski_shard* shard) { return pcg(g, pcg_args<float>(PCG_ABI_NAMES, as, amode, shard), s); }
int wiski_pcg_sharded_f64(const wiski_grid* g, PCG_ABI(double), void* s, wiski_pcg_async* as, int32_t amode, const wiski_shard* shard) { return pcg(g, pcg_args<double>(PCG_ABI_NAMES, as, amode, shard), s); }
int wiski_pcg_twolevel_f32(const wiski_grid* g, PCG_ABI(float), void* s, wiski_pcg_async* as, int32_t amode, const wiski_shard* shard, const wiski_twolevel* two_level) { return pcg(g, pcg_args<float>(PCG_ABI_NAMES, as, amode, shard, two_level), s); }
int wiski_precond_apply_cols_f32(const wiski_grid* grid, const float* evec, const float* evec2, const float* eval, float kscale, float shift, const float* d_r, int32_t k, float* w0, float* w1, float* d_y, float* d_t, double* d_rho, const wiski_twolevel* two_level, void* stream) {
  GridDev<float> G;
  if (int rc = make_grid_dev<float>(grid, &G)) return rc;
  if (!evec || !eval || !d_r || !w0 || !w1 || !d_y || !d_t || !d_rho || k < 1 || !spectral_fused_ok<float>(G) || G.m % 4) return WISKI_E_BADARG;
  PcgScal S{d_rho - k, k, nullptr};
  return launch_spectral_fused_cg<float>(G, evec, evec2, eval, kscale, shift, const_cast<float*>(d_r), k, w0, w1, 0, 0, 0.0, d_y, d_t, (float*)nullptr, 0, 0,
                                         (float*)nullptr, (float*)nullptr, S, (hipStream_t)stream, (const float*)nullptr, two_level);
}
int wiski_precond_apply_f32(const wiski_grid* grid, const float* evec, const float* evec2, const float* eval, float kscale, float shift, const float* d_r, float* w0, float* w1, float* d_y, float* d_t, double* d_rho, const wiski_twolevel* two_level, void* stream) {
  return wiski_precond_apply_cols_f32(grid, evec, evec2, eval, kscale, shift, d_r, 1, w0, w1, d_y, d_t, d_rho, two_level, stream);
}
int wiski_precond_apply_keep_f32(const wiski_grid* grid, const float* evec, const float* evec2, const float* eval, float kscale, float shift, const float* d_r, float* w0, float* w1, float* d_y, float* d_t, double* d_rho, const wiski_twolevel* two_level, const int32_t* keep, void* stream) {
  GridDev<float> G;
  if (int rc = make_grid_dev<float>(grid, &G)) return rc;
  if (!evec || !eval || !d_r || !w0 || !w1 || !d_y || !d_t || !d_rho || !keep || !spectral_fused_ok<float>(G) || G.m % 4) return WISKI_E_BADARG;
  const int kp[3] = {keep[0], keep[1], keep[2]};
  const bool any = kp[0] != 0 || kp[1] != 0 || kp[2] != 0;
  if (any && !spectral_keep_ok(G, kp, two_level != nullptr)) return WISKI_E_BADARG;
  PcgScal S{d_rho - 1, 1, nullptr};
  return launch_spectral_fused_cg<float>(G, evec, evec2, eval, kscale, shift, const_cast<float*>(d_r), 1, w0, w1, 0, 0, 0.0, d_y, d_t, (float*)nullptr, 0, 0,
                                         (float*)nullptr, (float*)nullptr, S, (hipStream_t)stream, (const float*)nullptr, two_level, any ? kp : (const int*)nullptr);
}
int wiski_precond_keep_ok(const wiski_grid* grid, const int32_t* keep, int32_t with_two_level) {
  GridDev<float> G;
  if (!keep || make_grid_dev<float>(grid, &G)) return 0;
  const int kp[3] = {keep[0], keep[1], keep[2]};
  return spectral_fused_ok<float>(G) && G.m % 4 == 0 && spectral_keep_ok(G, kp, with_two_level != 0) ? 1 : 0;
}
int wiski_shard_groups(int32_t d, int32_t rank, int32_t nranks, int32_t* g_lo, int32_t* g_hi) {
  if (d < 1 || d > WISKI_MAX_DIM || nranks < 1 || rank < 0 || rank >= nranks || !g_lo || !g_hi) return WISKI_E_BADARG;
  int lo, hi;
  shard_group_range(sym_groups(d), rank, nranks, &lo, &hi);
  *g_lo = lo;
  *g_hi = hi;
  return WISKI_OK;
}
int wiski_pcg_async_free(wiski_pcg_async* as) {
  if (!as) return WISKI_E_BADARG;
  if (as->poll) {
    WiskiPoll* P = static_cast<WiskiPoll*>(as->poll);
    if (P->h) (void)hipHostFree(P->h);
    if (P->g) (void)hipFree(P->g);
    delete P;
    as->poll = nullptr;
  }
  as->state = 0;
  return WISKI_OK;
}
int wiski_pcg_async_guard(const wiski_pcg_async* as, const void** d_guard, int64_t* expect) { return pcg_guard(as, d_guard, expect); }
int wiski_pcg_f32(const wiski_grid* g, PCG_ABI(float), void* s) { return pcg(g, pcg_args<float>(PCG_ABI_NAMES), s); }
int wiski_pcg_f64(const wiski_grid* g, PCG_ABI(double), void* s) { return pcg(g, pcg_args<double>(PCG_ABI_NAMES), s); }
}
```

online_gp_amd/csrc/spectral_keep.h:

```cpp
#pragma once

constexpr int KEEP_MAX = 24;
constexpr int KEEP_NS = 2;
constexpr int KEEP_LDK = 48;
constexpr int KEEP_LDC = 36;
constexpr size_t KEEP_LDS_BUDGET = 144 * 1024;

struct KeepDev {
  int K[3];
  int o[3];
};

__host__ __device__ static inline int keep_cube_ld(int KK) { return (KK % 64 == 16 || KK % 64 == 48) ? KK : KK + 16; }
static inline size_t keep_bwd_lds(const int* K, bool tl) {
  const int ksk = (K[0] > 16 || K[1] > 16 || K[2] > 16) ? 6 : 4;
  const size_t cubes = (size_t)2 * 4 * ksk * keep_cube_ld(K[1] * K[2]), slab = 2 * 64 * SPEC_LDN;
  return ((size_t)64 * KEEP_LDK + 2 * 64 * KEEP_LDC + (cubes > slab ? cubes : slab) + 2 * 32 * KEEP_LDC + 4 * 64 * KEEP_LDC + 96 +
          (tl ? 4 * SPEC_TL_MAXR + 80 : 0)) * sizeof(float);
}
constexpr size_t KEEP_FWD_LDS = (size_t)(64 * SPEC_LDN + 3 * 64 * KEEP_LDK) * sizeof(float);

static bool keep_counts_ok(const GridDev<float>& G, const int* K, bool tl) {
  if (G.d != 3 || G.stride[0] % 4 != 0) return false;
  for (int q = 0; q < 3; ++q)
    if (G.g[q] > 64 || K[q] < 4 || K[q] % 4 != 0 || K[q] > KEEP_MAX || K[q] > G.g[q]) return false;
  return keep_bwd_lds(K, tl) <= KEEP_LDS_BUDGET;
}

template <int KS>
__device__ __forceinline__ spec_f32x4 keep_tile(const float* __restrict__ pa, int sax, int sab, const float* __restrict__ pb, int sbb, int sby, int lane) {
  const int l15 = lane & 15, l4 = lane >> 4;
  const float* qa = pa + l15 * sax + l4 * sab;
  const float* qb = pb + l4 * sbb + l15 * sby;
  float af[KS], bf[KS];
#pragma unroll
  for (int i = 0; i < KS; ++i) {
    af[i] = qa[4 * i * sab];
    bf[i] = qb[4 * i * sbb];
  }
  spec_f32x4 acc = {0.f, 0.f, 0.f, 0.f};
#pragma unroll
  for (int i = 0; i < KS; ++i) acc = __builtin_amdgcn_mfma_f32_16x16x4f32(af[i], bf[i], acc, 0, 0, 0);
  return acc;
}

template <int W, int NT = 256>
struct KeepCols {
  static constexpr int NP = 64 * W / NT;
  float v[NP];
  __device__ __forceinline__ void issue(const float* __restrict__ M, int g, int o, int K) {
#pragma unroll
    for (int j = 0; j < NP; ++j) {
      const int idx = (int)threadIdx.x + NT * j, row = idx / W, col = idx % W;
      const bool ok = row < g && col < K;
      const float x = M[ok ? row * g + o + col : 0];
      v[j] = ok ? x : 0.f;
    }
  }
  __device__ __forceinline__ void commit(float* __restrict__ dst, int ld) const {
#pragma unroll
    for (int j = 0; j < NP; ++j) {
      const int idx = (int)threadIdx.x + NT * j;
      dst[(idx / W) * ld + idx % W] = v[j];
    }
  }
};

__device__ __forceinline__ void keep_range(int n4, int h, int* lo, int* hi) {
  const int per = (n4 + KEEP_NS - 1) / KEEP_NS;
  *lo = h * per;
  *hi = *lo + per < n4 ? *lo + per : n4;
}

template <int KS, int W>
__global__ __launch_bounds__(256) void k_keep_fwd(GridDev<float> G, KeepDev kp, const float* __restrict__ X1, const float* __restrict__ X2,
                                                  float* __restrict__ r, float* __restrict__ T, int it, int apply, double tol2,
                                                  const float* __restrict__ p, const float* __restrict__ pt, PcgScal S,
                                                  float* __restrict__ part, int nch, int zl, float* __restrict__ u, float* __restrict__ z) {
  extern __shared__ __attribute__((aligned(16))) char smem[];
  __shared__ double s_red[16];
  float* sR = reinterpret_cast<float*>(smem);
  float* sX1 = sR + 64 * SPEC_LDN;
  float* sX2 = sX1 + 64 * KEEP_LDK;
  float* sC = sX2 + 64 * KEEP_LDK;
  const int g1 = G.g[1], g2 = G.g[2], m = G.m, sl = g1 * g2;
  const int K1 = kp.K[1], K2 = kp.K[2];
  const int i0 = blockIdx.x, h = blockIdx.y;
  const int t = threadIdx.x, lane = t & 63, w = t >> 6, l15 = lane & 15, l4 = lane >> 4;
  int lo, hi;
  keep_range(sl >> 2, h, &lo, &hi);
  for (int e = t; e < 64 * SPEC_LDN / 4; e += 256) reinterpret_cast<float4*>(sR)[e] = make_float4(0.f, 0.f, 0.f, 0.f);
  KeepCols<W> c1, c2;
  c1.issue(X1, g1, kp.o[1], K1);
  c2.issue(X2, g2, kp.o[2], K2);
  float al = 0.f;
  if (apply == 1) {
    const double den = S.php_sum(it - 1, 0);
    if (i0 == 0 && h == 0) pcg_dot_clear(S.php(it), 0, 1, S.k);
    if (pcg_active(S, it - 1, 0, tol2) && den > 0) al = (float)(S.rho(it - 1)[0] / den);
  }
  float4 tin[2];
  float rn_part = 0.f, rhs_part = 0.f;
#pragma unroll
  for (int q = 0; q < 2; ++q) {
    const int f = lo + t + 256 * q;
    const bool ok = f < hi;
    const int64_t e = ok ? (int64_t)i0 * sl + 4 * f : 0;
    tin[q] = *reinterpret_cast<const float4*>(r + e);
    if (!ok) tin[q] = make_float4(0.f, 0.f, 0.f, 0.f);
    if (apply == 2 && ok) {
      const float4 f4 = *reinterpret_cast<const float4*>(p + e), rv = tin[q];
      rhs_part += f4.x * f4.x + f4.y * f4.y + f4.z * f4.z + f4.w * f4.w;
      rn_part += rv.x * rv.x + rv.y * rv.y + rv.z * rv.z + rv.w * rv.w;
    }
    if (apply == 1 && ok) {
      const float4 pv = *reinterpret_cast<const float4*>(p + e), ptv = *reinterpret_cast<const float4*>(pt + e);
      float4 uv = *reinterpret_cast<const float4*>(u + e), zv = *reinterpret_cast<const float4*>(z + e);
      float4 pp[8];
#pragma unroll
      for (int ch = 0; ch < 8; ++ch)
        if (ch < nch) pp[ch] = *reinterpret_cast<const float4*>(part + (int64_t)ch * m + e);
      if (zl) *reinterpret_cast<float4*>(part + (int64_t)(nch - 1) * m + e) = make_float4(0.f, 0.f, 0.f, 0.f);
      float4 hv = ptv;
#pragma unroll
      for (int ch = 0; ch < 8; ++ch)
        if (ch < nch) { hv.x += pp[ch].x; hv.y += pp[ch].y; hv.z += pp[ch].z; hv.w += pp[ch].w; }
      uv.x += al * pv.x; uv.y += al * pv.y; uv.z += al * pv.z; uv.w += al * pv.w;
      zv.x += al * ptv.x; zv.y += al * ptv.y; zv.z += al * ptv.z; zv.w += al * ptv.w;
      float4 rv = tin[q];
      rv.x -= al * hv.x; rv.y -= al * hv.y; rv.z -= al * hv.z; rv.w -= al * hv.w;
      rn_part += rv.x * rv.x + rv.y * rv.y + rv.z * rv.z + rv.w * rv.w;
      *reinterpret_cast<float4*>(u + e) = uv;
      *reinterpret_cast<float4*>(z + e) = zv;
      *reinterpret_cast<float4*>(r + e) = rv;
      tin[q] = rv;
    }
  }
  if (apply) {
    const double tot = block_reduce_sum((double)rn_part, s_red);
    if (t == 0) unsafeAtomicAdd(S.rn(it), tot);
    if (apply == 2) {
      const double tot0 = block_reduce_sum((double)rhs_part, s_red);
      if (t == 0) unsafeAtomicAdd(S.rn0(), tot0);
    }
  }
  __syncthreads();
  c1.commit(sX1, KEEP_LDK);
  c2.commit(sX2, KEEP_LDK);
#pragma unroll
  for (int q = 0; q < 2; ++q) {
    const int f = lo + t + 256 * q;
    if (f < hi) {
      const float v[4] = {tin[q].x, tin[q].y, tin[q].z, tin[q].w};
      int row = (4 * f) / g2, col = 4 * f - row * g2;
#pragma unroll
      for (int j = 0; j < 4; ++j) {
        if (col == g2) { col = 0; ++row; }
        sR[row * SPEC_LDN + col] = v[j];
        ++col;
      }
    }
  }
  __syncthreads();
#pragma unroll
  for (int ct = 0; ct < W / 16; ++ct) {
    const spec_f32x4 acc = keep_tile<KS>(sR + 16 * w * SPEC_LDN, SPEC_LDN, 1, sX2 + 16 * ct, KEEP_LDK, 1, lane);
#pragma unroll
    for (int q = 0; q < 4; ++q) sC[(16 * w + 4 * l4 + q) * KEEP_LDK + 16 * ct + l15] = acc[q];
  }
  __syncthreads();
  constexpr int NT1 = W / 16;
  if (w < NT1 * NT1) {
    const int mt = w / NT1, nt = w % NT1;
    const spec_f32x4 acc = keep_tile<KS>(sX1 + 16 * mt, 1, KEEP_LDK, sC + 16 * nt, KEEP_LDK, 1, lane);
    float* __restrict__ out = T + (int64_t)(i0 * KEEP_NS + h) * K1 * K2;
    const int k2 = 16 * nt + l15;
#pragma unroll
    for (int q = 0; q < 4; ++q) {
      const int k1 = 16 * mt + 4 * l4 + q;
      if (k1 < K1 && k2 < K2) out[k1 * K2 + k2] = acc[q];
    }
  }
}

template <int KS0, int KSK, bool TL>
__global__ __launch_bounds__(1024) void k_keep_bwd(GridDev<float> G, KeepDev kp, const float* __restrict__ X0, const float* __restrict__ Z0,
                                                   const float* __restrict__ X1, const float* __restrict__ X2, const float* __restrict__ Z1,
                                                   const float* __restrict__ Z2, const float* __restrict__ evals, float kscale, float shift,
                                                   const float* __restrict__ T, const float* __restrict__ r, float* __restrict__ p,
                                                   float* __restrict__ pt, int it, PcgScal S, double* __restrict__ rho, TwoLevelDev tl) {
  extern __shared__ __attribute__((aligned(16))) char smem[];
  __shared__ double s_red[16];
  constexpr int KR = 4 * KSK;
  constexpr int W = KSK == 4 ? 16 : 32;
  const int g0 = G.g[0], g1 = G.g[1], g2 = G.g[2], sl = g1 * g2, n4 = sl >> 2;
  const int K0 = kp.K[0], K1 = kp.K[1], K2 = kp.K[2], KK = K1 * K2, ldc = keep_cube_ld(KK);
  const int i0 = blockIdx.x;
  float* sXt = reinterpret_cast<float*>(smem);
  float* sXn = sXt + 64 * KEEP_LDK;
  float* sZn = sXn + 64 * KEEP_LDC;
  float* sEh = sXt;
  float* sCY = sZn + 64 * KEEP_LDC;
  float* sCT = sCY + KR * ldc;
  float* sO = sCY;
  const int cube = 2 * KR * ldc > 2 * 64 * SPEC_LDN ? 2 * KR * ldc : 2 * 64 * SPEC_LDN;
  float* sS = sCY + cube;
  float* sM = sS + 2 * 32 * KEEP_LDC;
  float* sE = sM + 4 * 64 * KEEP_LDC;
  float* sCs = sE + 96;
  float* sD = sCs + SPEC_TL_MAXR;
  float* sLam = sD + SPEC_TL_MAXR;
  int* sIdx = reinterpret_cast<int*>(sLam + SPEC_TL_MAXR);
  int* sOff = sIdx + SPEC_TL_MAXR;
  const int t = threadIdx.x, lane = t & 63, w = t >> 6, l15 = lane & 15, l4 = lane >> 4;
  const int nnt = KK / 16, ntile = ((KR + 15) / 16) * nnt;
  const int tr = TL ? (tl.r < SPEC_TL_MAXR ? tl.r : SPEC_TL_MAXR) : 0;
  const bool v_ok = t < n4;
  const int64_t ve = (int64_t)i0 * sl + (v_ok ? 4 * t : 0);
  KeepCols<W, 1024> cx2, cz2, cx1, cz1;
  cx2.issue(X2, g2, kp.o[2], K2);
  cz2.issue(Z2, g2, kp.o[2], K2);
  cx1.issue(X1, g1, kp.o[1], K1);
  cz1.issue(Z1, g1, kp.o[1], K1);
  for (int e = t; e < 2 * 32 * KEEP_LDC / 4; e += 1024) reinterpret_cast<float4*>(sS)[e] = make_float4(0.f, 0.f, 0.f, 0.f);
  unsigned ppos = 0;
  if constexpr (TL) {
    if (t < tr) ppos = tl.pos[t];
    if (t <= g0) sOff[t] = tl.off[t];
  }
  float xi[2], zi[2], ev = 0.f;
#pragma unroll
  for (int j = 0; j < 2; ++j) {
    const int idx = t + 1024 * j, row = idx >> 5, col = idx & 31;
    const bool ok = row < g0 && col < K0;
    const float x = X0[ok ? row * g0 + kp.o[0] + col : 0], zv = Z0[ok ? row * g0 + kp.o[0] + col : 0];
    xi[j] = ok ? x : 0.f;
    zi[j] = ok ? zv : 0.f;
  }
  if (t < 96) {
    const int q = t >> 5, j = t & 31;
    const int base = q == 0 ? kp.o[0] : (q == 1 ? g0 + kp.o[1] : g0 + g1 + kp.o[2]);
    const bool ok = j < (q == 0 ? K0 : (q == 1 ? K1 : K2));
    const float e = evals[ok ? base + j : 0];
    ev = ok ? e : 0.f;
  }
  float bf[KS0];
  unsigned long long mrow[4];
  auto load_b = [&](int tile) {
    const int mt = tile / nnt, n = 16 * (tile - mt * nnt) + l15;
#pragma unroll
    for (int i = 0; i < KS0; ++i) {
      const int b0 = 4 * i + l4;
      const bool ok = b0 < g0;
      const float* q = T + (int64_t)(ok ? b0 : 0) * KEEP_NS * KK + n;
      float v = q[0];
#pragma unroll
      for (int hh = 1; hh < KEEP_NS; ++hh) v += q[hh * KK];
      bf[i] = ok ? v : 0.f;
    }
    if constexpr (TL) {
      const int k1 = n / K2;
#pragma unroll
      for (int q = 0; q < 4; ++q) {
        const int k0 = 16 * mt + 4 * l4 + q;
        mrow[q] = k0 < K0 ? tl.mask[(kp.o[0] + k0) * 64 + kp.o[1] + k1] : 0ull;
      }
    }
  };
  int tile = w;
  if (tile < ntile) load_b(tile);
  constexpr int PF_ROWS = 12, PF_CH = 3;
  constexpr bool PF = TL && KSK == 4;
  float npf[PF ? PF_ROWS : 1][PF ? PF_CH : 1];
  const bool pf = PF && tr <= 64 * PF_CH && tr <= 16 * PF_ROWS;
  if constexpr (PF) {
    if (pf) {
#pragma unroll
      for (int i = 0; i < PF_ROWS; ++i) {
        const int e = w + 16 * i;
        const float* __restrict__ nrow = tl.N + (int64_t)(e < tr ? e : 0) * tl.r;
#pragma unroll
        for (int j = 0; j < PF_CH; ++j) npf[i][j] = (e < tr && lane + 64 * j < tr) ? nrow[lane + 64 * j] : 0.f;
      }
    }
  }
#pragma unroll
  for (int j = 0; j < 2; ++j) {
    const int idx = t + 1024 * j, row = idx >> 5, col = idx & 31;
    sXt[row * KEEP_LDK + col] = xi[j];
    sXn[row * KEEP_LDC + col] = xi[j];
    sZn[row * KEEP_LDC + col] = zi[j];
  }
  if (t < 96) sE[t] = ev;
// ... 8 lines not shown
#pragma unroll
      for (int i = 0; i < KS0; ++i) af[i] = qa[4 * i * KEEP_LDK];
#pragma unroll
      for (int i = 0; i < KS0; ++i) acc = __builtin_amdgcn_mfma_f32_16x16x4f32(af[i], bf[i], acc, 0, 0, 0);
    }
    const int k1 = n / K2, k2 = n - k1 * K2;
    const float e1 = sE[32 + k1], e2 = sE[64 + k2];
#pragma unroll
    for (int q = 0; q < 4; ++q) {
      const int k0 = 16 * mt + 4 * l4 + q;
      if (k0 < KR) {
        const float lam = kscale * sE[k0] * e1 * e2;
        const float al = shift * lam, f1 = __frcp_rn(1.f + al);
        const float v = acc[q];
        float cy = (lam * f1) * v, ct = (al * f1) * v;
        bool sel = false;
        if constexpr (TL) sel = (mrow[q] >> (kp.o[2] + k2)) & 1ull;
        if (sel) cy = ct = v;
        else rho_lane += cy * v;
        sCY[k0 * ldc + n] = cy;
        sCT[k0 * ldc + n] = ct;
      }
    }
    tile += 16;
    if (tile < ntile) load_b(tile);
  }
  __syncthreads();
  const float4 rv = *reinterpret_cast<const float4*>(r + ve);
  float4 pv = make_float4(0.f, 0.f, 0.f, 0.f), ptv = pv;
  if (it > 0) {
    pv = *reinterpret_cast<const float4*>(p + ve);
    ptv = *reinterpret_cast<const float4*>(pt + ve);
  }
  if constexpr (TL) {
    if (t < tr) {
      int lo_ = 0, hi_ = g0 - 1;
      while (lo_ < hi_) {
        const int mid = (lo_ + hi_ + 1) >> 1;
        if (sOff[mid] <= t) lo_ = mid;
        else hi_ = mid - 1;
      }
      const int x = ppos >> 8, y = ppos & 255u;
      const int k0 = lo_ - kp.o[0], k1 = x - kp.o[1], k2 = y - kp.o[2];
      const bool in = k0 >= 0 && k1 >= 0 && k1 < K1 && k2 >= 0 && k2 < K2;
      const int idx = in ? k0 * ldc + k1 * K2 + k2 : -1;
      sIdx[t] = idx;
      sCs[t] = in ? sCY[idx] : 0.f;
      sLam[t] = in ? kscale * sE[k0] * sE[32 + k1] * sE[64 + k2] : 1.f;
    }
    __syncthreads();
    bool rows_done = false;
    if constexpr (PF) {
     if (pf) {
      rows_done = true;
      float cq[PF_CH];
#pragma unroll
      for (int j = 0; j < PF_CH; ++j) cq[j] = lane + 64 * j < tr ? sCs[lane + 64 * j] : 0.f;
#pragma unroll
      for (int i = 0; i < PF_ROWS; ++i) {
        const int e = w + 16 * i;
        if (e < tr) {
          float d = 0.f;
#pragma unroll
          for (int j = 0; j < PF_CH; ++j) d += npf[i][j] * cq[j];
          d = wave_reduce_sum<float>(d);
          if (lane == 0) sD[e] = d;
        }
      }
     }
    }
    if (!rows_done) {
      for (int e = w; e < tr; e += 16) {
        const float* __restrict__ nrow = tl.N + (int64_t)e * tl.r;
        float d = 0.f;
        for (int q = lane; q < tr; q += 64) d += nrow[q] * sCs[q];
        d = wave_reduce_sum<float>(d);
        if (lane == 0) sD[e] = d;
      }
    }
    __syncthreads();
    for (int e = t; e < tr; e += 1024) {
      const int idx = sIdx[e];
      if (idx >= 0) {
        const float d = sD[e], cs = sCs[e];
        sCY[idx] = d;
        sCT[idx] = cs - d / sLam[e];
        rho_lane += cs * d;
      }
    }
  }
  {
    const double ws = wave_reduce_sum<double>((double)rho_lane);
    if (lane == 0) s_red[w] = ws;
  }
  __syncthreads();
  double rho_it = 0;
#pragma unroll
  for (int i = 0; i < 16; ++i) rho_it += s_red[i];
  float bt = 0.f;
  if (it > 0) {
    const double den = S.rho(it - 1)[0];
    bt = (float)(den > 0 ? rho_it / den : 0.0);
  }
  if (t < KK) {
    float sy = 0.f, st = 0.f;
    for (int k0 = 0; k0 < K0; ++k0) {
      sy += sXn[i0 * KEEP_LDC + k0] * sCY[k0 * ldc + t];
      st += sZn[i0 * KEEP_LDC + k0] * sCT[k0 * ldc + t];
    }
    const int k1 = t / K2, k2 = t - k1 * K2;
    sS[k1 * KEEP_LDC + k2] = sy;
    sS[32 * KEEP_LDC + k1 * KEEP_LDC + k2] = st;
  }
  cx2.commit(sM, KEEP_LDC);
  cz2.commit(sM + 64 * KEEP_LDC, KEEP_LDC);
  cx1.commit(sM + 2 * 64 * KEEP_LDC, KEEP_LDC);
  cz1.commit(sM + 3 * 64 * KEEP_LDC, KEEP_LDC);
  __syncthreads();
  constexpr int MT = W / 16;
  for (int id = w; id < 2 * MT * 4; id += 16) {
    const int hh = id / (MT * 4), mt = (id / 4) % MT, ct = id % 4;
    const spec_f32x4 acc = keep_tile<KSK>(sS + hh * 32 * KEEP_LDC + 16 * mt * KEEP_LDC, KEEP_LDC, 1, sM + hh * 64 * KEEP_LDC + 16 * ct * KEEP_LDC, 1, KEEP_LDC, lane);
#pragma unroll
    for (int q = 0; q < 4; ++q) sEh[hh * 32 * SPEC_LDT + (16 * mt + 4 * l4 + q) * SPEC_LDT + 16 * ct + l15] = acc[q];
  }
  __syncthreads();
  for (int id = w; id < 2 * 4 * 4; id += 16) {
    const int hh = id / 16, rt = (id / 4) % 4, ct = id % 4;
    if (16 * rt >= g1) continue;
    const spec_f32x4 acc = keep_tile<KSK>(sM + (2 + hh) * 64 * KEEP_LDC + 16 * rt * KEEP_LDC, KEEP_LDC, 1, sEh + hh * 32 * SPEC_LDT + 16 * ct, SPEC_LDT, 1, lane);
#pragma unroll
    for (int q = 0; q < 4; ++q) sO[hh * 64 * SPEC_LDN + (16 * rt + 4 * l4 + q) * SPEC_LDN + 16 * ct + l15] = acc[q];
  }
  __syncthreads();
  if (v_ok) {
    const float rr[4] = {rv.x, rv.y, rv.z, rv.w};
    const float po[4] = {pv.x, pv.y, pv.z, pv.w}, pto[4] = {ptv.x, ptv.y, ptv.z, ptv.w};
    float pn[4], ptn[4];
    int row = (4 * t) / g2, col = 4 * t - row * g2;
#pragma unroll
    for (int j = 0; j < 4; ++j) {
      if (col == g2) { col = 0; ++row; }
      const float y = sO[row * SPEC_LDN + col], tv = rr[j] - sO[64 * SPEC_LDN + row * SPEC_LDN + col];
      pn[j] = it > 0 ? y + bt * po[j] : y;
      ptn[j] = it > 0 ? tv + bt * pto[j] : tv;
      ++col;
    }
    *reinterpret_cast<float4*>(p + ve) = make_float4(pn[0], pn[1], pn[2], pn[3]);
    *reinterpret_cast<float4*>(pt + ve) = make_float4(ptn[0], ptn[1], ptn[2], ptn[3]);
  }
  if (i0 == 0 && t == 0 && rho != nullptr) unsafeAtomicAdd(rho, rho_it);
}

static int launch_spectral_keep_cg(const GridDev<float>& G, const float* evec, const float* evec2, const float* evals, float kscale, float shift,
                                   float* r, float* w1, int it, int apply, double tol2, float* p, float* pt, float* part, int nch, int zl,
                                   float* u, float* z, PcgScal S, hipStream_t s, const float* rhs0, const wiski_twolevel* two_level, const int* keep) {
  const int g0 = G.g[0], g1 = G.g[1], g2 = G.g[2];
  if (!keep_counts_ok(G, keep, two_level != nullptr) || S.k != 1 || nch > 8) return WISKI_E_BADARG;
  if (two_level && (two_level->r < 1 || two_level->r > SPEC_TL_MAXR || !two_level->d_mask || !two_level->d_off || !two_level->d_pos || !two_level->d_N))
    return WISKI_E_BADARG;
  if (rhs0 && apply) return WISKI_E_BADARG;
  if (!evec2) evec2 = evec;
  const float *X0 = evec, *X1 = evec + g0 * g0, *X2 = X1 + g1 * g1;
  const float *Z0 = evec2, *Z1 = evec2 + g0 * g0, *Z2 = Z1 + g1 * g1;
  KeepDev kp;
  for (int q = 0; q < 3; ++q) { kp.K[q] = keep[q]; kp.o[q] = G.g[q] - keep[q]; }
  TwoLevelDev tl{};
  if (two_level)
    tl = TwoLevelDev{two_level->r, two_level->nslab, (const unsigned long long*)two_level->d_mask, two_level->d_off, two_level->d_pos, two_level->d_N,
                     nullptr, 0u};
  const bool wide = keep[0] > 16 || keep[1] > 16 || keep[2] > 16;
  const size_t bwd_lds = keep_bwd_lds(keep, two_level != nullptr);
  const dim3 grd((unsigned)g0, KEEP_NS);
  int dev = 0;
  if (hipGetDevice(&dev) != hipSuccess) return WISKI_E_LAUNCH;
#define KEEP_LDS_OPT_IN(fn, bytes)                                                                                                     \
  do {                                                                                                                                 \
    static size_t set_[16] = {0};                            \
    if ((size_t)(bytes) > set_[dev & 15]) {                                                                                            \
      if (hipFuncSetAttribute((const void*)(fn), hipFuncAttributeMaxDynamicSharedMemorySize, (int)(bytes)) != hipSuccess) return WISKI_E_LAUNCH; \
      set_[dev & 15] = (bytes);                                                                                                        \
    }                                                                                                                                  \
  } while (0)
  {
    const int gm = g1 > g2 ? g1 : g2;
    const float* pin = rhs0 ? rhs0 : p;
    const int ap = rhs0 ? 2 : apply;
#define KEEP_FWD2(KS, WW)                                                                                                                  \
  do {                                                                                                                                     \
    KEEP_LDS_OPT_IN((k_keep_fwd<KS, WW>), KEEP_FWD_LDS);                                                                                   \
    hipLaunchKernelGGL((k_keep_fwd<KS, WW>), grd, dim3(256), KEEP_FWD_LDS, s, G, kp, X1, X2, r, w1, it, ap, tol2, pin, (const float*)pt, S, \
                       part, nch, zl, u, z);                                                                                               \
  } while (0)
#define KEEP_FWD(KS, VW_UNUSED)          \
  do {                                   \
    if (wide) KEEP_FWD2(KS, 32);         \
    else KEEP_FWD2(KS, 16);              \
  } while (0)
    SPEC_DISPATCH_KS_VW(gm, true, KEEP_FWD);
#undef KEEP_FWD
#undef KEEP_FWD2
    if (hipGetLastError() != hipSuccess) return WISKI_E_LAUNCH;
  }
  {
#define KEEP_BWD3(KS, KSK, TLV)                                                                                                          \
  do {                                                                                                                                   \
    KEEP_LDS_OPT_IN((k_keep_bwd<KS, KSK, TLV>), bwd_lds);                                                                                \
    hipLaunchKernelGGL((k_keep_bwd<KS, KSK, TLV>), dim3((unsigned)g0), dim3(1024), bwd_lds, s, G, kp, X0, Z0, X1, X2, Z1, Z2, evals, kscale, \
                       shift, (const float*)w1, (const float*)r, p, pt, it, S, S.rho(it), tl);                                           \
  } while (0)
#define KEEP_BWD(KS, VW_UNUSED)                    \
  do {                                             \
    if (wide) {                                    \
      if (two_level) KEEP_BWD3(KS, 6, true);       \
      else KEEP_BWD3(KS, 6, false);                \
    } else {                                       \
      if (two_level) KEEP_BWD3(KS, 4, true);       \
      else KEEP_BWD3(KS, 4, false);                \
    }                                              \
  } while (0)
    SPEC_DISPATCH_KS_VW(g0, true, KEEP_BWD);
#undef KEEP_BWD
#undef KEEP_BWD3
  }
#undef KEEP_LDS_OPT_IN
  return hipGetLastError() == hipSuccess ? WISKI_OK : WISKI_E_LAUNCH;
}
```

online_gp_amd/csrc/stream_step.hip:

```cpp
#include "absorb.h"
#include "pcg.h"

template <typename real>
struct StreamArgs;
template <>
struct StreamArgs<float> { using type = wiski_stream_args_f32; };
template <>
struct StreamArgs<double> { using type = wiski_stream_args_f64; };

template <typename real>
static int absorb_batch(const wiski_grid* g, const typename StreamArgs<real>::type* a, AbsorbArgs<real> r, int carry, int zero, void* s) {
  r.b = a->d_b; r.A = a->d_A_half; r.half = true; r.cnt = a->d_cnt; r.stats = a->d_stats; r.err = a->d_err;
  r.u = carry || r.mean_out ? a->d_U : nullptr;
  r.res = carry ? a->d_R : nullptr;
  if (!r.mean_out) return absorb(g, r, s);
  if (zero) {
    if (int rc = pcg_zero_regions<real>(g, 1, a->max_iter, a->d_work, true, &r.z1, &r.n1_bytes, &r.z2, &r.n2_bytes)) return rc;
  }
  if (wiski_shard_active(a->shard)) {
    int32_t glo = 0, ghi = 0;
    if (int rc = wiski_shard_groups(g->d, a->shard->rank, a->shard->nranks, &glo, &ghi)) return rc;
    r.g_lo = glo; r.g_hi = ghi;
  } else {
    r.bin = a->d_bin; r.bin_bytes = a->bin_bytes;
  }
  return absorb(g, r, s);
}
template <typename real>
static PcgArgs<real> solve_args(const typename StreamArgs<real>::type* a, int carry, int first_check) {
  PcgArgs<real> p;
  p.A = a->d_A_half; p.a_sym = true; p.RHS = a->d_b; p.k = 1;
  p.tcol = a->d_tcol; p.kscale = a->kscale; p.evec = a->d_evec; p.evec2 = a->d_evec2; p.eval = a->d_eval; p.shift = a->shift; p.two_level = a->two_level;
  for (int q = 0; q < 3; ++q) p.keep[q] = a->keep[q];
  p.U = a->d_U; p.Z = a->d_Z; p.R = a->d_R; p.warm = carry ? 2 : 1;
  p.tol = a->tol; p.max_iter = a->max_iter; p.check_every = a->check_every; p.first_check = first_check;
  p.work = a->d_work; p.work_bytes = a->work_bytes;
  p.d_err = a->d_err;
  p.shard = a->shard;
  return p;
}

template <typename real>
static int stream_step_impl(const wiski_grid* grid, const typename StreamArgs<real>::type* a, const real* d_x, const real* d_y, const real* d_wa,
                            const real* d_wb, const real* d_noise, int64_t q, real* d_mean_out, int32_t carry, int32_t first_check, int32_t* h_iters,
                            double* h_relres, int32_t* h_err, void* stream, wiski_pcg_async* as, int32_t defer, int32_t* h_resumed) {
  if (!grid || !a || q < 0 || !a->d_A_half || !a->d_b || !a->d_U || !a->d_Z || !a->d_R) return WISKI_E_BADARG;
  if (q > 0 && (!d_x || !d_y || !d_wa || !d_wb || !d_noise)) return WISKI_E_BADARG;
  if (wiski_shard_active(a->shard) && q > 0 && !d_mean_out) return WISKI_E_BADARG;
  int rc = WISKI_OK;
  if (h_resumed) *h_resumed = 0;
  PcgArgs<real> solve = solve_args<real>(a, carry, first_check);
  solve.h_iters = h_iters; solve.h_relres = h_relres; solve.h_err = h_err; solve.handle = as;
  AbsorbArgs<real> batch;
  batch.x = d_x; batch.y = d_y; batch.wa = d_wa; batch.wb = d_wb; batch.noise = d_noise; batch.n = q; batch.mean_out = d_mean_out;
  bool absorbed = false;
  if (as && as->state == 1) {
    bool spec = false;
    if (q > 0 && d_mean_out) {
      const void* guard = nullptr;
      int64_t expect = 0;
      if (pcg_guard(as, &guard, &expect) == WISKI_OK) {
        AbsorbArgs<real> spec_batch = batch;
        spec_batch.guard = guard; spec_batch.guard_expect = expect;
        rc = absorb_batch<real>(grid, a, spec_batch, carry, 1, stream);
        if (rc) return rc;
        spec = true;
      }
    }
    {
      PcgArgs<real> resume = solve;
      resume.shift = (real)as->shift;
      resume.mode = 2;
      rc = pcg(grid, resume, stream);
    }
    if (h_resumed) *h_resumed = 1;
    if (rc != WISKI_OK && rc != WISKI_E_NOTCONV) return rc;
    absorbed = spec && as->guard_ok;
    if (q == 0) return rc;
    if (!absorbed && h_err && *h_err) return rc;
  } else if (q == 0 && as) {
    return WISKI_OK;
  }
  const int resumed_rc = rc;
  if (absorbed) {
    as->prezeroed = 1;
  } else if (q > 0) {
    if (d_mean_out) {
      rc = absorb_batch<real>(grid, a, batch, carry, as ? 1 : 0, stream);
      if (rc) return rc;
      if (as) as->prezeroed = 1;
    } else {
      rc = absorb_batch<real>(grid, a, batch, carry, 0, stream);
      if (rc) return rc;
    }
  }
  if (!as) return pcg(grid, solve, stream);
  if (defer) {
    as->shift = (double)a->shift;
    solve.h_iters = nullptr; solve.h_relres = nullptr; solve.h_err = nullptr;
    solve.mode = 1;
    rc = pcg(grid, solve, stream);
    return rc == WISKI_PENDING ? (resumed_rc == WISKI_E_NOTCONV ? WISKI_E_NOTCONV : WISKI_PENDING) : rc;
  }
  if (h_resumed && *h_resumed == 1) *h_resumed = 2;
  rc = pcg(grid, solve, stream);
  return rc == WISKI_OK && resumed_rc == WISKI_E_NOTCONV ? WISKI_E_NOTCONV : rc;
}

extern "C" {
int wiski_stream_step_f32(const wiski_grid* grid, const wiski_stream_args_f32* a, const float* d_x, const float* d_y, const float* d_wa, const float* d_wb, const float* d_noise, int64_t q, float* d_mean_out, int32_t carry, int32_t first_check, int32_t* h_iters, double* h_relres, int32_t* h_err, void* stream, wiski_pcg_async* as, int32_t defer, int32_t* h_resumed) {
  return stream_step_impl<float>(grid, a, d_x, d_y, d_wa, d_wb, d_noise, q, d_mean_out, carry, first_check, h_iters, h_relres, h_err, stream, as, defer, h_resumed);
}
int wiski_stream_step_f64(const wiski_grid* grid, const wiski_stream_args_f64* a, const double* d_x, const double* d_y, const double* d_wa, const double* d_wb, const double* d_noise, int64_t q, double* d_mean_out, int32_t carry, int32_t first_check, int32_t* h_iters, double* h_relres, int32_t* h_err, void* stream, wiski_pcg_async* as, int32_t defer, int32_t* h_resumed) {
  return stream_step_impl<double>(grid, a, d_x, d_y, d_wa, d_wb, d_noise, q, d_mean_out, carry, first_check, h_iters, h_relres, h_err, stream, as, defer, h_resumed);
}
}
```

online_gp_amd/csrc/wiski_common.h:

```cpp
#pragma once
#include <hip/hip_runtime.h>
#include <stdint.h>

#include "../../include/wiski.h"

#define WISKI_VERSION 1

template <typename real>
struct GridDev {
  int d;
  int g[WISKI_MAX_DIM];
  int stride[WISKI_MAX_DIM];
  real g0[WISKI_MAX_DIM];
  real h[WISKI_MAX_DIM];
  real hi[WISKI_MAX_DIM];
  int m;
  int T;
  int R;
};

template <typename real>
static inline int make_grid_dev(const wiski_grid* grid, GridDev<real>* out) {
  if (!grid || grid->d < 1 || grid->d > WISKI_MAX_DIM) return WISKI_E_BADARG;
  GridDev<real> G;
// ... 86 lines not shown

template <typename real, int D>
__device__ __forceinline__ real gather_one(const GridDev<real>& G, const int j0[D], const real w[D][4], const real* __restrict__ v) {
  constexpr int off = 0;
  real acc = (real)0;
  if constexpr (D == 1) {
#pragma unroll
    for (int c0 = 0; c0 < 4; ++c0) acc += w[0][c0] * v[j0[0] + c0];
  } else if constexpr (D == 2) {
#pragma unroll
    for (int c0 = 0; c0 < 4; ++c0) {
      const real* r0 = v + (j0[0] + c0) * G.stride[off] + j0[1];
      real s = (real)0;
#pragma unroll
      for (int c1 = 0; c1 < 4; ++c1) s += w[1][c1] * r0[c1];
      acc += w[0][c0] * s;
    }
  } else if constexpr (D == 3) {
#pragma unroll
    for (int c0 = 0; c0 < 4; ++c0) {
      real s0 = (real)0;
#pragma unroll
      for (int c1 = 0; c1 < 4; ++c1) {
        const real* r = v + (j0[0] + c0) * G.stride[off] + (j0[1] + c1) * G.stride[off + 1] + j0[2];
        real s1 = (real)0;
#pragma unroll
        for (int c2 = 0; c2 < 4; ++c2) s1 += w[2][c2] * r[c2];
        s0 += w[1][c1] * s1;
      }
      acc += w[0][c0] * s0;
    }
  } else {
#pragma unroll
    for (int c0 = 0; c0 < 4; ++c0) {
      real s0 = (real)0;
#pragma unroll
      for (int c1 = 0; c1 < 4; ++c1) {
        real s1 = (real)0;
#pragma unroll
        for (int c2 = 0; c2 < 4; ++c2) {
          const real* r = v + (j0[0] + c0) * G.stride[0] + (j0[1] + c1) * G.stride[1] + (j0[2] + c2) * G.stride[2] + j0[3];
          real s2 = (real)0;
#pragma unroll
          for (int c3 = 0; c3 < 4; ++c3) s2 += w[3][c3] * r[c3];
          s1 += w[2][c2] * s2;
        }
        s0 += w[1][c1] * s1;
      }
      acc += w[0][c0] * s0;
    }
  }
  return acc;
}

__device__ __forceinline__ void atomic_add_real(float* p, float v) { unsafeAtomicAdd(p, v); }
__device__ __forceinline__ void atomic_add_real(double* p, double v) { unsafeAtomicAdd(p, v); }

template <int CTRL, int ROW_MASK>
__device__ __forceinline__ float wave_dpp_add(float v) {
  return v + __builtin_bit_cast(float, __builtin_amdgcn_update_dpp(0, __builtin_bit_cast(int, v), CTRL, ROW_MASK, 0xf, true));
}
template <int CTRL, int ROW_MASK>
__device__ __forceinline__ double wave_dpp_add(double v) {
  const long long b = __builtin_bit_cast(long long, v);
  const int lo = __builtin_amdgcn_update_dpp(0, (int)(b & 0xffffffffll), CTRL, ROW_MASK, 0xf, true);
  const int hi = __builtin_amdgcn_update_dpp(0, (int)(b >> 32), CTRL, ROW_MASK, 0xf, true);
  return v + __builtin_bit_cast(double, ((long long)hi << 32) | (long long)(unsigned)lo);
}
template <typename T>
__device__ __forceinline__ T wave_reduce_sum(T v) {
  v = wave_dpp_add<0x111, 0xf>(v);
  v = wave_dpp_add<0x112, 0xf>(v);
  v = wave_dpp_add<0x114, 0xf>(v);
  v = wave_dpp_add<0x118, 0xf>(v);
  v = wave_dpp_add<0x142, 0xa>(v);
  v = wave_dpp_add<0x143, 0xc>(v);
  if constexpr (sizeof(T) == 8) {
    const long long b = __builtin_bit_cast(long long, v);
    const int lo = __builtin_amdgcn_readlane((int)(b & 0xffffffffll), 63), hi = __builtin_amdgcn_readlane((int)(b >> 32), 63);
    return __builtin_bit_cast(T, ((long long)hi << 32) | (long long)(unsigned)lo);
  } else {
    return __builtin_bit_cast(T, __builtin_amdgcn_readlane(__builtin_bit_cast(int, v), 63));
  }
}

__device__ __forceinline__ double block_reduce_sum(double v, double* sm) {
  v = wave_reduce_sum<double>(v);
  int lane = threadIdx.x & 63, wid = threadIdx.x >> 6;
  if (lane == 0) sm[wid] = v;
  __syncthreads();
  double r = 0;
  if (threadIdx.x == 0) {
    int nw = (blockDim.x + 63) >> 6;
    for (int i = 0; i < nw; ++i) r += sm[i];
  }
  __syncthreads();
  return r;
}

#define WISKI_LAUNCH_CHECK()                          \
  do {                                                \
    if (hipGetLastError() != hipSuccess) return WISKI_E_LAUNCH; \
  } while (0)

#define WISKI_DISPATCH_D(d, CALL) \
  switch (d) {                    \
    case 1: { CALL(1); break; }   \
    case 2: { CALL(2); break; }   \
    case 3: { CALL(3); break; }   \
    case 4: { CALL(4); break; }   \
    default: return WISKI_E_BADARG; \
  }

constexpr int PCG_DOT_SLOTS = 16;
constexpr int PCG_DOT_STRIDE = 16;
constexpr int PCG_DOT_COL = PCG_DOT_SLOTS * PCG_DOT_STRIDE;
static inline bool wiski_shard_active(const wiski_shard* s) { return s && (s->nranks > 1 || (s->nranks == 1 && s->comm)); }

struct PcgScal {
  double* base;
  int k;
  double* ring;
  __host__ __device__ double* rn0() const { return base; }
  __host__ __device__ double* rho(int it) const { return base + (int64_t)k * (1 + 2 * it); }
  __host__ __device__ double* rn(int it) const { return base + (int64_t)k * (2 + 2 * it); }
  __host__ __device__ double* php(int it) const { return ring + (int64_t)(it & 1) * k * PCG_DOT_COL; }
  __device__ double php_sum(int it, int c) const {
    const double* q = php(it) + (int64_t)c * PCG_DOT_COL;
    double t = 0;
#pragma unroll
    for (int j = 0; j < PCG_DOT_SLOTS; ++j) t += q[j * PCG_DOT_STRIDE];
    return t;
  }
  static int64_t scalars(int k, int max_iter) { return (int64_t)k * (1 + 2 * (int64_t)(max_iter + 2)) + 1; }
  __host__ __device__ unsigned* ticket() const { return reinterpret_cast<unsigned*>(ring) - 2; }
  static int64_t doubles(int k, int max_iter) { return scalars(k, max_iter) + 2 * (int64_t)k * PCG_DOT_COL; }
};

__device__ __forceinline__ void pcg_dot_add(double* dots, int col, double v) {
  unsafeAtomicAdd(dots + (int64_t)col * PCG_DOT_COL + (blockIdx.x & (PCG_DOT_SLOTS - 1)) * PCG_DOT_STRIDE, v);
}
__device__ __forceinline__ void pcg_dot_clear(double* dots_next, int col0, int ncol, int k) {
  for (int idx = threadIdx.x; idx < ncol * PCG_DOT_COL; idx += blockDim.x) {
    const int c = col0 + idx / PCG_DOT_COL;
    if (c < k) dots_next[(int64_t)c * PCG_DOT_COL + idx % PCG_DOT_COL] = 0.0;
  }
}

__device__ __forceinline__ bool pcg_active(const PcgScal& S, int it, int c, double tol2) {
  const double rn0 = S.rn0()[c];
  return rn0 > 0 && S.rn(it)[c] > tol2 * rn0;
}

template <typename real>
bool spectral_fused_ok(const GridDev<real>& G);
template <typename real>
int launch_spectral_fused(const GridDev<real>& G, const real* evec, const real* evec2, const real* evals, real kscale, real shift, const real* r,
                          int k, real* w0, real* w1, real* ty, double* rho, hipStream_t s);

template <typename real>
int launch_spectral_fused_cg(const GridDev<real>& G, const real* evec, const real* evec2, const real* evals, real kscale, real shift, real* r,
                             int k, real* w0, real* w1, int it, int apply, double tol2, real* p, real* pt, real* part, int nch, int zl, real* u,
                             real* z, PcgScal S, hipStream_t s, const real* rhs0 = nullptr, const wiski_twolevel* two_level = nullptr,
                             const int* keep = nullptr);
bool spectral_keep_ok(const GridDev<float>& G, const int* keep, bool two_level);
```

online_gp_amd/grid_ops.py:

```python
import ctypes
import math
import warnings

import numpy as np

import torch

from . import _hip


class GridSpec:

    def __init__(self, grid_bounds, grid_size):
        gb = [[float(lo), float(hi)] for lo, hi in (torch.as_tensor(grid_bounds, dtype=torch.float64).reshape(-1, 2).tolist())]
        d = len(gb)
        if not 1 <= d <= _hip.MAX_DIM:
            raise ValueError(f"grid dimension must be 1..{_hip.MAX_DIM}, got {d}")
        if isinstance(grid_size, int):
            g = [grid_size] * d
        else:
            g = [int(v) for v in grid_size]
        if len(g) != d:
            raise ValueError("grid_size / grid_bounds mismatch")
        if min(g) < 4:
            raise ValueError("cubic interpolation needs at least 4 grid points per dim")
        self.d = d
        self.g = g
        self.grid_bounds = gb
        delta = [(hi - lo) / (gi - 2) for (lo, hi), gi in zip(gb, g)]
        self.g0 = [lo - dl for (lo, hi), dl in zip(gb, delta)]
        self.h = [((hi + dl) - g0) / (gi - 1) for (lo, hi), dl, g0, gi in zip(gb, delta, self.g0, g)]
        from . import settings

        if settings.float32_grid.on():
            for q, ((lo, hi), gi) in enumerate(zip(gb, g)):
                dl = torch.tensor(hi - lo, dtype=torch.float32) / (gi - 2)
                pts = torch.linspace(float(torch.tensor(lo, dtype=torch.float32) - dl), float(torch.tensor(hi, dtype=torch.float32) + dl), gi,
                                     dtype=torch.float32)
                self.g0[q] = float(pts[0])
                self.h[q] = float(pts[1] - pts[0])
        self.m = int(math.prod(g))
        self.T = 4 ** d
        self.R = 7 ** d
        c = _hip.wiski_grid()
        c.d = d
        for q in range(d):
            c.g[q] = g[q]
            c.g0[q] = self.g0[q]
            c.h[q] = self.h[q]
        self.c = c

    @property
    def ref(self):
        return ctypes.byref(self.c)

    def shifted(self, below, above):
        a = [int(below)] * self.d if isinstance(below, int) else [int(v) for v in below]
        b = [int(above)] * self.d if isinstance(above, int) else [int(v) for v in above]
        if len(a) != self.d or len(b) != self.d:
            raise ValueError(f"below / above need one entry per grid dim ({self.d})")
        g = [gq + aq + bq for gq, aq, bq in zip(self.g, a, b)]
        if min(g) < 4:
            raise ValueError("cubic interpolation needs at least 4 grid points per dim")
        if any(aq <= -gq or aq >= gn for gq, aq, gn in zip(self.g, a, g)):
            raise ValueError("the shifted grid must share at least one node with the old one in every dim")
        from . import settings

        new = object.__new__(GridSpec)
        new.d, new.g, new.h = self.d, g, list(self.h)
        new.g0 = [g0 - aq * h for g0, aq, h in zip(self.g0, a, self.h)]
        if settings.float32_grid.on():
            new.g0 = [float(torch.tensor(v, dtype=torch.float32)) for v in new.g0]
        new.grid_bounds = [[g0 + h * (gq - 1) / gq, g0 + h * (gq - 1) ** 2 / gq] for g0, h, gq in zip(new.g0, new.h, g)]
        new.m = int(math.prod(g))
        new.T, new.R = self.T, self.R
        c = _hip.wiski_grid()
        c.d = new.d
        for q in range(new.d):
            c.g[q], c.g0[q], c.h[q] = g[q], new.g0[q], new.h[q]
        new.c = c
        return new

    def grid_points(self, dtype=torch.float64, device="cpu"):
        return [self.g0[q] + self.h[q] * torch.arange(self.g[q], dtype=dtype, device=device) for q in range(self.d)]

    def stencil_offsets(self, device="cpu"):
        offs = torch.zeros(1, dtype=torch.int64)
        stride = [int(math.prod(self.g[q + 1:])) for q in range(self.d)]
        for q in range(self.d):
            offs = (offs[:, None] + (torch.arange(7) - 3)[None, :] * stride[q]).reshape(-1)
        return offs.to(device)


def new_err_flag(device):
    return torch.zeros(1, dtype=torch.int32, device=device)


def read_flag(flag):
    val = ctypes.c_int32(0)
    rc = _hip.lib().wiski_read_flag(_hip.dptr(flag), ctypes.byref(val), _hip.stream_ptr(flag.device))
    _hip.check(rc, "wiski_read_flag")
    return int(val.value)


def _x2d(x, grid):
    if x.dim() != 2 or x.shape[1] != grid.d:
        raise ValueError(f"expected inputs of shape [n, {grid.d}], got {tuple(x.shape)}")
    return x.contiguous()


def interp(grid, x, err):
    x = _x2d(x, grid)
    n = x.shape[0]
    idx = torch.empty((n, grid.T), dtype=torch.int32, device=x.device)
    val = torch.empty((n, grid.T), dtype=x.dtype, device=x.device)
    rc = _hip.fn("wiski_interp", x.dtype)(grid.ref, _hip.dptr(x), ctypes.c_int64(n), _hip.dptr(idx), _hip.dptr(val), _hip.dptr(err),
                                          _hip.stream_ptr(x.device))
    _hip.check(rc, "wiski_interp")
    return idx, val


def gather(grid, x, V, err, diag=False):
    x = _x2d(x, grid)
    V = V.contiguous()
    if V.dim() == 1:
        V = V[None]
    k = V.shape[0]
    n = x.shape[0]
    assert V.shape[1] == grid.m and V.dtype == x.dtype
    out = torch.empty((n,) if diag else (n, k), dtype=x.dtype, device=x.device)
    rc = _hip.fn("wiski_gather", x.dtype)(grid.ref, _hip.dptr(x), ctypes.c_int64(n), _hip.dptr(V), ctypes.c_int32(k), ctypes.c_int32(int(diag)),
                                          _hip.dptr(out), _hip.dptr(err), _hip.stream_ptr(x.device))
    _hip.check(rc, "wiski_gather")
    return out


def gather_grad(grid, x, V, diag=False):
    x = _x2d(x, grid)
    V = V.contiguous()
    out = torch.empty((x.shape[0], grid.d), dtype=x.dtype, device=x.device)
    rc = _hip.fn("wiski_gather_grad", x.dtype)(grid.ref, _hip.dptr(x), ctypes.c_int64(x.shape[0]), _hip.dptr(V), ctypes.c_int32(int(diag)),
                                               _hip.dptr(out), _hip.stream_ptr(x.device))
    _hip.check(rc, "wiski_gather_grad")
    return out


class InterpDot(torch.autograd.Function):

    @staticmethod
    def forward(ctx, grid, x, V, diag, err):
        xd = x.detach().contiguous()
        Vd = V.detach().contiguous().reshape(-1, grid.m)
        ctx.grid, ctx.diag = grid, diag
        ctx.save_for_backward(xd, Vd)
        out = gather(grid, xd, Vd, err, diag=diag)
        return out if diag else out[:, 0]

    @staticmethod
    def backward(ctx, g):
        xd, Vd = ctx.saved_tensors
        gx = gather_grad(ctx.grid, xd, Vd, diag=ctx.diag) * g[:, None]
# ... 418 lines not shown
    f = _hip.fn("wiski_regrid_stats", dtype)
    c_below = (ctypes.c_int32 * old_grid.d)(*a)
    c_above = (ctypes.c_int32 * old_grid.d)(*[gn - go - aq for gn, go, aq in zip(new_grid.g, old_grid.g, a)])
    c_new = (ctypes.c_int32 * old_grid.d)(*new_grid.g)
    i = 0
    while i < len(regs):
        plan = _hip.wiski_regrid_plan()
        base = None
        n = 0
        while i < len(regs) and n < _hip.REGRID_MAX_REGIONS:
            src, dst, k, w, r0, report = regs[i]
            if report >= 0:
                if base is None:
                    base = report
                if not (0 <= report - base < _hip.REGRID_MAX_REPORTS):
                    break
            plan.src[n], plan.dst[n], plan.k[n], plan.w[n], plan.r0[n] = _hip.dptr(src).value, _hip.dptr(dst).value, k, w, r0
            plan.report[n] = report - base if report >= 0 else -1
            n += 1
            i += 1
        plan.count = n
        rc = f(old_grid.ref, c_below, c_above, c_new, ctypes.byref(plan), _hip.dptr(record[base:]) if base is not None else None, _hip.stream_ptr(dev))
        _hip.check(rc, "wiski_regrid_stats")
    if record is None:
        return [], []
    rec = record.tolist()
    return [int(r[0]) for r in rec], [float(r[1]) for r in rec]


def stencil_expand_add(grid, A_half, A_st):
    rc = _hip.fn("wiski_stencil_expand_add", A_st.dtype)(grid.ref, _hip.dptr(A_half), _hip.dptr(A_st), _hip.stream_ptr(A_st.device))
    _hip.check(rc, "wiski_stencil_expand_add")


def wt_columns(grid, x, err):
    x = _x2d(x, grid)
    out = torch.zeros((x.shape[0], grid.m), dtype=x.dtype, device=x.device)
    rc = _hip.fn("wiski_wt_columns", x.dtype)(grid.ref, _hip.dptr(x), ctypes.c_int64(x.shape[0]), _hip.dptr(out), _hip.dptr(err),
                                              _hip.stream_ptr(x.device))
    _hip.check(rc, "wiski_wt_columns")
    return out


def wt_columns_jet(grid, x, err):
    x = _x2d(x, grid)
    out = torch.zeros((x.shape[0] * (grid.d + 1), grid.m), dtype=x.dtype, device=x.device)
    rc = _hip.fn("wiski_wt_columns_jet", x.dtype)(grid.ref, _hip.dptr(x), ctypes.c_int64(x.shape[0]), _hip.dptr(out), _hip.dptr(err),
                                                  _hip.stream_ptr(x.device))
    _hip.check(rc, "wiski_wt_columns_jet")
    return out


def jet_quadform(grid, x, M, err):
    x = _x2d(x, grid)
    assert M.dim() == 2 and M.shape[0] == grid.m and M.shape[1] >= grid.m and M.stride(1) == 1 and M.dtype == x.dtype
    C = grid.d + 1
    out = torch.empty((x.shape[0], C, C), dtype=x.dtype, device=x.device)
    if not M.is_cuda:
        raise _hip.WiskiError("online_gp_amd ops need ROCm device tensors (no CPU fallback)")
    rc = _hip.fn("wiski_jet_quadform", x.dtype)(grid.ref, _hip.dptr(x), ctypes.c_int64(x.shape[0]), ctypes.c_void_p(M.data_ptr()),
                                                ctypes.c_int64(M.stride(0)), _hip.dptr(out), _hip.dptr(err), _hip.stream_ptr(x.device))
    _hip.check(rc, "wiski_jet_quadform")
    return out


def gather_jet(grid, x, V, err, rows_per_point=0):
    x = _x2d(x, grid)
    V = V.contiguous()
    if V.dim() == 1:
        V = V[None]
    n, B = x.shape[0], int(rows_per_point)
    assert V.shape[1] == grid.m and V.dtype == x.dtype and (B == 0 or V.shape[0] == n * B)
    k = B if B > 0 else V.shape[0]
    out = torch.empty((n, k, grid.d + 1), dtype=x.dtype, device=x.device)
    rc = _hip.fn("wiski_gather_jet", x.dtype)(grid.ref, _hip.dptr(x), ctypes.c_int64(n), _hip.dptr(V), ctypes.c_int32(max(k, 1)), ctypes.c_int32(B),
                                              _hip.dptr(out), _hip.dptr(err), _hip.stream_ptr(x.device))
    _hip.check(rc, "wiski_gather_jet")
    return out


def is_half_stencil(grid, A_st):
    rows = A_st.shape[-2]
    if rows == (grid.R + 1) // 2:
        return True
    if rows == grid.R:
        return False
    raise ValueError(f"stencil with {rows} rows matches neither the full ({grid.R}) nor the half ({(grid.R + 1) // 2}) layout")


def half_stencil_from_offset_major(grid, A_om):
    H, m = A_om.shape
    flat = torch.empty(H * m, dtype=A_om.dtype, device=A_om.device)
    flat[:4 * m] = A_om[:4].t().reshape(-1)
    if H > 4:
        flat[4 * m:] = A_om[4:].reshape(-1, 7, m).transpose(1, 2).reshape(-1)
    return flat.view(H, m)


def half_stencil_to_offset_major(grid, A_h):
    H, m = A_h.shape
    flat = A_h.reshape(-1)
    out = torch.empty((H, m), dtype=A_h.dtype, device=A_h.device)
    out[:4] = flat[:4 * m].view(m, 4).t()
    if H > 4:
        out[4:] = flat[4 * m:].view(-1, m, 7).transpose(1, 2).reshape(H - 4, m)
    return out


def stencil_spmv(grid, A_st, V, add=None, beta=1.0):
    V2 = V.contiguous().reshape(-1, grid.m)
    out = torch.empty_like(V2)
    cr = _hip.creal(V2.dtype)
    name = "wiski_stencil_spmv_sym" if is_half_stencil(grid, A_st) else "wiski_stencil_spmv"
    rc = _hip.fn(name, V2.dtype)(grid.ref, _hip.dptr(A_st), _hip.dptr(V2), ctypes.c_int32(V2.shape[0]),
                                 _hip.dptr(add.contiguous().reshape(-1, grid.m)) if add is not None else None, cr(beta),
                                 _hip.dptr(out), _hip.stream_ptr(V2.device))
    _hip.check(rc, name)
    return out.reshape(V.shape)


def kron_toeplitz_mm(grid, tcol, V, scale=1.0):
    V2 = V.contiguous().reshape(-1, grid.m)
    out = torch.empty_like(V2)
    tmp = torch.empty_like(V2) if grid.d > 1 else None
    cr = _hip.creal(V2.dtype)
    rc = _hip.fn("wiski_kron_toeplitz_mm", V2.dtype)(grid.ref, _hip.dptr(tcol.contiguous()), _hip.dptr(V2), ctypes.c_int32(V2.shape[0]), cr(scale),
                                                     _hip.dptr(tmp), _hip.dptr(out), _hip.stream_ptr(V2.device))
    _hip.check(rc, "wiski_kron_toeplitz_mm")
    return out.reshape(V.shape)


class PCGWorkspace:

    def __init__(self):
        self.buf = None

    def get(self, grid, k, max_iter, dtype, device):
        es = 4 if dtype == torch.float32 else 8
        need = int(_hip.lib().wiski_pcg_workspace_bytes(grid.ref, ctypes.c_int32(k), ctypes.c_int32(max_iter), ctypes.c_int32(es)))
        if need < 0:
            raise _hip.WiskiError("wiski_pcg_workspace_bytes: bad arguments")
        if self.buf is None or self.buf.numel() < need or self.buf.device != device:
            self.buf = torch.empty(need, dtype=torch.uint8, device=device)
        return self.buf, need


class _StreamArgs32(ctypes.Structure):
    _fields_ = [("d_A_half", ctypes.c_void_p), ("d_b", ctypes.c_void_p), ("d_cnt", ctypes.c_void_p), ("d_stats", ctypes.c_void_p),
                ("d_err", ctypes.c_void_p), ("d_U", ctypes.c_void_p), ("d_Z", ctypes.c_void_p), ("d_R", ctypes.c_void_p),
                ("d_tcol", ctypes.c_void_p), ("kscale", ctypes.c_float), ("d_evec", ctypes.c_void_p), ("d_evec2", ctypes.c_void_p),
                ("d_eval", ctypes.c_void_p), ("shift", ctypes.c_float), ("tol", ctypes.c_double), ("max_iter", ctypes.c_int32),
                ("check_every", ctypes.c_int32), ("d_work", ctypes.c_void_p), ("work_bytes", ctypes.c_int64),
                ("d_bin", ctypes.c_void_p), ("bin_bytes", ctypes.c_int64), ("shard", ctypes.c_void_p), ("two_level", ctypes.c_void_p),
                ("keep", ctypes.c_int32 * 3)]


ALLREDUCE_FN = ctypes.CFUNCTYPE(ctypes.c_int, ctypes.c_void_p, ctypes.c_void_p, ctypes.c_int64, ctypes.c_int32, ctypes.c_void_p, ctypes.c_int64,
                                ctypes.c_void_p)


class _Shard(ctypes.Structure):
    _fields_ = [("rank", ctypes.c_int32), ("nranks", ctypes.c_int32), ("comm", ctypes.c_void_p), ("allreduce", ALLREDUCE_FN), ("ctx", ctypes.c_void_p)]


class TwoLevelStruct(ctypes.Structure):
    _fields_ = [("r", ctypes.c_int32), ("nslab", ctypes.c_int32), ("d_mask", ctypes.c_void_p), ("d_off", ctypes.c_void_p), ("d_pos", ctypes.c_void_p),
                ("d_N", ctypes.c_void_p), ("d_cs", ctypes.c_void_p), ("d_mc", ctypes.c_void_p), ("mc_cols", ctypes.c_int32)]


def shard_groups(d, rank, nranks):
    lo, hi = ctypes.c_int32(0), ctypes.c_int32(0)
    _hip.check(_hip.lib().wiski_shard_groups(ctypes.c_int32(d), ctypes.c_int32(rank), ctypes.c_int32(nranks), ctypes.byref(lo), ctypes.byref(hi)),
               "wiski_shard_groups")
    return int(lo.value), int(hi.value)


def half_stencil_group_slices(grid, g_lo, g_hi):
    m = grid.m
    out = []
    for g in range(g_lo, g_hi):
        out.append((0, 4 * m) if g == 0 else ((7 * g - 3) * m, (7 * g + 4) * m))
    return out


class _StreamArgs64(ctypes.Structure):
    _fields_ = [(n, ctypes.c_double if t is ctypes.c_float else t) for n, t in _StreamArgs32._fields_]



class _PcgAsync(ctypes.Structure):
    _fields_ = [("state", ctypes.c_int32), ("it", ctypes.c_int32), ("seq", ctypes.c_int64), ("poll", ctypes.c_void_p),
                ("prezeroed", ctypes.c_int32), ("guard_ok", ctypes.c_int32), ("shift", ctypes.c_double)]


class StreamStep:

    def __init__(self, grid, dtype, device, A_half, b, cnt, stats, err, U, Z, R, tcol, workspace, max_iter):
        self.grid, self.dtype, self.device = grid, dtype, device
        self.keep = (A_half, b, cnt, stats, err, U, Z, R, tcol)
        self.args = (_StreamArgs32 if dtype == torch.float32 else _StreamArgs64)()
        a = self.args
        a.d_A_half, a.d_b, a.d_cnt, a.d_stats, a.d_err = A_half.data_ptr(), b.data_ptr(), cnt.data_ptr(), stats.data_ptr(), err.data_ptr()
        a.d_U, a.d_Z, a.d_R, a.d_tcol = U.data_ptr(), Z.data_ptr(), R.data_ptr(), tcol.data_ptr()
        buf, need = workspace.get(grid, 1, max_iter, dtype, device)
        self.keep += (buf,)
        a.d_work, a.work_bytes, a.max_iter = buf.data_ptr(), need, max_iter
        self.bin_buf = None
        self.fn = _hip.fn("wiski_stream_step", dtype)
        self.it, self.herr, self.rr = ctypes.c_int32(0), ctypes.c_int32(0), ctypes.c_double(0)
        self.eig_keep = None
        self.handle = _PcgAsync()
        self.resumed = ctypes.c_int32(0)

    @property
    def pending(self):
        return self.handle.state == 1

    def __del__(self):
        try:
            if self.handle.poll:
                _hip.lib().wiski_pcg_async_free(ctypes.byref(self.handle))
        except Exception:
            pass

    def set_shard(self, rank, nranks, comm=None, allreduce=None):
        if nranks < 1 or (nranks == 1 and not comm):
            self.args.shard = None
            self._shard = None
            return
        buf = self.keep[-1]
        base = buf.data_ptr()

        def cb(ctx, d_vec, n_vec, elem_bytes, d_dots, n_dots, stream):
            try:
                dt = torch.float32 if elem_bytes == 4 else torch.float64
                vec = buf[d_vec - base:d_vec - base + n_vec * elem_bytes].view(dt)
                dots = buf[d_dots - base:d_dots - base + n_dots * 8].view(torch.float64) if (d_dots and n_dots) else None
                allreduce(vec, dots)
                return 0
            except Exception:
                import traceback

                traceback.print_exc()
                return -2

        self._shard_cb = ALLREDUCE_FN(cb) if allreduce is not None else ALLREDUCE_FN()
        self._shard = _Shard(rank, nranks, comm, self._shard_cb, None)
        self.args.shard = ctypes.addressof(self._shard)

    def set_two_level(self, tl):
        self._two_level = tl
        self.args.two_level = ctypes.addressof(tl) if tl is not None else None

    def set_keep(self, keep):
        k = tuple(int(v) for v in keep) if keep is not None else (0, 0, 0)
        if tuple(self.args.keep) != k:
            self.args.keep[:] = k

    def set_solver(self, kscale, eig, shift, tol, check_every):
        a = self.args
        evec, evals, evec2 = (tuple(eig) + (None,))[:3]
        self.eig_keep = (evec, evals, evec2)
        a.kscale, a.shift, a.tol, a.check_every = kscale, shift, tol, check_every
        a.d_evec, a.d_eval = evec.data_ptr(), evals.data_ptr()
        a.d_evec2 = evec2.data_ptr() if evec2 is not None else None

    def __call__(self, x, y, wa, wb, noise, mean_out, carry, first_check, defer=False):
        q = x.shape[0] if x is not None else 0
        if q >= 4096 and self.grid.d == 3 and (self.bin_buf is None or self.bin_q < q):
            f = _hip.lib().wiski_scatter_bin_bytes
            f.restype = ctypes.c_int64
            need = int(f(self.grid.ref, ctypes.c_int64(q), ctypes.c_int32(4 if self.dtype == torch.float32 else 8)))
            if need > 0:
                self.bin_buf, self.bin_q = torch.zeros(need, dtype=torch.uint8, device=self.device), q
                self.args.d_bin, self.args.bin_bytes = self.bin_buf.data_ptr(), need
        use_handle = defer or self.pending
        self.herr.value = 0
        rc = self.fn(self.grid.ref, ctypes.byref(self.args), _hip.dptr(x), _hip.dptr(y), _hip.dptr(wa), _hip.dptr(wb), _hip.dptr(noise),
                     ctypes.c_int64(q), _hip.dptr(mean_out), ctypes.c_int32(int(carry)), ctypes.c_int32(int(first_check)), ctypes.byref(self.it),
                     ctypes.byref(self.rr), ctypes.byref(self.herr), _hip.stream_ptr(self.device),
                     ctypes.byref(self.handle) if use_handle else None, ctypes.c_int32(int(defer)), ctypes.byref(self.resumed))
        if rc == -4:
            warnings.warn(f"wiski_pcg stopped at max_iter={self.args.max_iter} with relative residual {self.rr.value:.3e}", RuntimeWarning)
        elif rc != 1:
            _hip.check(rc, "wiski_stream_step")
        res = (int(self.it.value), float(self.rr.value), int(self.herr.value), rc != -4)
        if not use_handle:
            return res
        return (res if self.resumed.value == 1 else None), self.pending


def precond_apply(grid, eig, kscale, shift, r, two_level=None):
    Y, T, rho = precond_apply_cols(grid, eig, kscale, shift, r.reshape(1, grid.m), two_level=two_level)
    return Y.reshape(r.shape), T.reshape(r.shape), rho[0]


KEEP_EPS = 2.0 ** -30


def keep_counts(D_host, kscale, shift, eps=KEEP_EPS):
    import numpy as np

    if not (shift > 0 and kscale > 0):
        return None, 0.0, 0.0
    tau = eps / (1.0 - eps)
    dmax = [float(D[-1]) for D in D_host]
    if min(dmax) <= 0:
        return None, 0.0, 0.0
    K, lo, hi = [], 0.0, np.inf
    for q, D in enumerate(D_host):
        g = len(D)
        d = np.where(D < g * 2.0 ** -52 * dmax[q], 0.0, D)
        c = kscale * float(np.prod([dmax[p] for p in range(len(D_host)) if p != q]))
        first = int(np.searchsorted(d, tau / (shift * c), side="right"))
        K.append(g - first)
        if first < g:
            lo = max(lo, tau / (c * d[first]))
        if first > 0 and d[first - 1] > 0:
            hi = min(hi, tau / (c * d[first - 1]))
    out = []
    for q, D in enumerate(D_host):
        g, k4 = len(D), -(-K[q] // 4) * 4
        if K[q] < 1 or (k4 > g and g % 4 != 0):
            return None, lo, hi
        out.append(min(k4, g))
    if all(k == len(D) for k, D in zip(out, D_host)):
        return None, lo, hi
    return tuple(out), lo, hi


def keep_accepts(grid, keep, two_level=False):
    return bool(_hip.lib().wiski_precond_keep_ok(grid.ref, (ctypes.c_int32 * 3)(*[int(v) for v in keep]), ctypes.c_int32(int(bool(two_level)))))


def precond_apply_keep(grid, eig, kscale, shift, r, keep, two_level=None):
    evec, evals, evec2 = (tuple(eig) + (None,))[:3]
    r = r.contiguous()
    m = r.numel()
    w0 = torch.empty(m, dtype=r.dtype, device=r.device)
    w1 = torch.empty(2 * m, dtype=r.dtype, device=r.device)
    y, t = torch.empty_like(r), torch.empty_like(r)
    rho = torch.zeros(1, dtype=torch.float64, device=r.device)
    kp = (ctypes.c_int32 * 3)(*([int(v) for v in keep] if keep is not None else [0, 0, 0]))
    rc = _hip.lib().wiski_precond_apply_keep_f32(grid.ref, _hip.dptr(evec), _hip.dptr(evec2), _hip.dptr(evals), ctypes.c_float(kscale), ctypes.c_float(shift),
                                                 _hip.dptr(r), _hip.dptr(w0), _hip.dptr(w1), _hip.dptr(y), _hip.dptr(t), _hip.dptr(rho),
                                                 ctypes.byref(two_level) if two_level is not None else None, kp, _hip.stream_ptr(r.device))
    _hip.check(rc, "wiski_precond_apply_keep")
    return y, t, rho[0]


def precond_apply_cols(grid, eig, kscale, shift, R, two_level=None):
    evec, evals, evec2 = (tuple(eig) + (None,))[:3]
    R = R.contiguous()
    k, m = R.shape
    w0 = torch.empty(k * m, dtype=R.dtype, device=R.device)
    w1 = torch.empty(2 * k * m, dtype=R.dtype, device=R.device)
    Y, T = torch.empty_like(R), torch.empty_like(R)
    rho = torch.zeros(k, dtype=torch.float64, device=R.device)
    rc = _hip.lib().wiski_precond_apply_cols_f32(grid.ref, _hip.dptr(evec), _hip.dptr(evec2), _hip.dptr(evals), ctypes.c_float(kscale), ctypes.c_float(shift),
                                                 _hip.dptr(R), ctypes.c_int32(k), _hip.dptr(w0), _hip.dptr(w1), _hip.dptr(Y), _hip.dptr(T), _hip.dptr(rho),
                                                 ctypes.byref(two_level) if two_level is not None else None, _hip.stream_ptr(R.device))
    _hip.check(rc, "wiski_precond_apply_cols")
    return Y, T, rho


def kron_eigen(grid, tcol, profiles=None, host_out=None, dtype=None):
    import numpy as np

    tc = tcol.detach().to("cpu", torch.float64).numpy()
    X, Z, vals, off = [], [], [], 0
    for q, g in enumerate(grid.g):
        c = tc[off:off + g]
        idx = np.abs(np.arange(g)[:, None] - np.arange(g)[None, :])
        K = c[idx]
        if profiles is None:
            w, V = np.linalg.eigh(K)
            X.append(V.reshape(-1))
        else:
            t = np.asarray(profiles[q], dtype=np.float64)
            rt = np.sqrt(t)
            w, U = np.linalg.eigh(rt[:, None] * K * rt[None, :])
            X.append((U / rt[:, None]).reshape(-1))
            Z.append((U * rt[:, None]).reshape(-1))
        vals.append(np.clip(w, 0.0, None))
        off += g
    mk = lambda parts: torch.as_tensor(np.concatenate(parts)).to(tcol.device, dtype or tcol.dtype)
    if host_out is not None:
        host_out["X"] = [x.reshape(g, g) for x, g in zip(X, grid.g)]
        host_out["D"] = [v.copy() for v in vals]
    if profiles is None:
        return mk(X), mk(vals)
    return mk(X), mk(vals), mk(Z)


def _pcg_abi(dtype, *, grid, A, a_sym, RHS, k, tcol, kscale, evec, evec2, eval, shift, U, Z, R, warm, tol, max_iter, check_every, first_check,
             work, work_bytes, h_iters, h_relres, d_err, h_err, stream):
    cr, i32, p = _hip.creal(dtype), (lambda v: ctypes.c_int32(int(v))), _hip.dptr
    return (grid.ref, p(A), p(tcol), cr(kscale), p(evec), p(evec2), p(eval), cr(shift), p(RHS), i32(k), p(U), p(Z), i32(warm), ctypes.c_double(tol),
            i32(max_iter), i32(check_every), i32(first_check), p(work), ctypes.c_int64(work_bytes), ctypes.byref(h_iters), h_relres, p(d_err),
            ctypes.byref(h_err), i32(a_sym), p(R), stream)


def pcg(grid, A_st, tcol, kscale, RHS, U=None, Z=None, warm=False, tol=1e-6, max_iter=1000, check_every=10, workspace=None,
        raise_on_fail=False, eigen=None, shift=0.0, first_check=0, err=None, inplace=False, R=None, two_level=None):
    RHS2 = RHS.contiguous().reshape(-1, grid.m)
    k = RHS2.shape[0]
    if U is None or Z is None or (not warm and not inplace):
        U = torch.empty_like(RHS2)
        Z = torch.empty_like(RHS2)
        warm = False
    if int(warm) == 2 and R is None:
        raise ValueError("warm=2 needs the carried-over residual R")
    ws = workspace if workspace is not None else PCGWorkspace()
    buf, need = ws.get(grid, k, max_iter, RHS2.dtype, RHS2.device)
    iters = ctypes.c_int32(0)
    h_err = ctypes.c_int32(0)
    relres = (ctypes.c_double * k)()
    evec, evals, evec2 = (tuple(eigen) + (None,))[:3] if eigen is not None else (None, None, None)
    common = _pcg_abi(RHS2.dtype, grid=grid, A=A_st, a_sym=is_half_stencil(grid, A_st), RHS=RHS2, k=k,
                      tcol=tcol.contiguous(), kscale=kscale, evec=evec, evec2=evec2, eval=evals, shift=shift,
                      U=U, Z=Z, R=R, warm=warm, tol=tol, max_iter=max_iter, check_every=check_every, first_check=first_check,
                      work=buf, work_bytes=need, h_iters=iters, h_relres=relres, d_err=err, h_err=h_err, stream=_hip.stream_ptr(RHS2.device))
    if two_level is not None and (k == 1 or (two_level.d_mc and k <= two_level.mc_cols)) and RHS2.dtype == torch.float32 and evec is not None:
        rc = _hip.lib().wiski_pcg_twolevel_f32(*common, None, ctypes.c_int32(0), None, ctypes.byref(two_level))
    else:
        rc = _hip.fn("wiski_pcg", RHS2.dtype)(*common)
    if rc == -4 and not raise_on_fail:
        warnings.warn(f"wiski_pcg stopped at max_iter={max_iter} with relative residual {max(relres):.3e} (tolerance {tol:.1e})",
                      RuntimeWarning)
        pcg.last_converged = False
# ... 410 lines not shown
```

online_gp_amd/settings.py:

```python


class _feature_flag:
    _state = False

    @classmethod
    def on(cls):
        return cls._state

    @classmethod
    def off(cls):
        return not cls._state

    @classmethod
    def _set_state(cls, state):
        cls._state = state

    def __init__(self, state=True):
        self.prev = self.__class__.on()
        self.state = state

    def __enter__(self):
        self.__class__._set_state(self.state)

    def __exit__(self, *args):
        self.__class__._set_state(self.prev)
        return False


class _value_context:
    _global_value = None

    @classmethod
    def value(cls):
        return cls._global_value

    @classmethod
    def _set_value(cls, value):
        cls._global_value = value

    def __init__(self, value):
        self._orig_value = self.__class__.value()
        self._instance_value = value

    def __enter__(self):
        self.__class__._set_value(self._instance_value)

    def __exit__(self, *args):
        self.__class__._set_value(self._orig_value)
        return False


class check_decomposition(_feature_flag):
    _state = False


class detach_interp_coeff(_feature_flag):
    _state = False


class skip_posterior_variances(_feature_flag):
    _state = False


class fast_pred_var(_feature_flag):

    _state = False


class fast_pred_samples(_feature_flag):

    _state = False


class skip_logdet_forward(_feature_flag):
    _state = False


class deferred_refresh(_feature_flag):

    _state = False


class float32_grid(_feature_flag):

    _state = False


class deferred_bounds_check(_feature_flag):

    _state = False


class use_toeplitz(_feature_flag):
    _state = True


class cg_tolerance(_value_context):

    _global_value = None


class variance_cg_tolerance(_value_context):

    _global_value = None


class max_cg_iterations(_value_context):
    _global_value = 2000


class max_cholesky_size(_value_context):

    _global_value = 2048


class max_root_decomposition_size(_value_context):
    _global_value = 512


class cholesky_jitter(_value_context):
    _global_value = None


class variance_chunk(_value_context):

    _global_value = 64


class spectral_preconditioner(_feature_flag):

    _state = True


class cg_check_every(_value_context):

    _global_value = 3


class dense_small_grids(_feature_flag):

    _state = True


class dense_rank_updates(_feature_flag):

    _state = True


class residual_carry_over(_feature_flag):

    _state = True


class precond_profile_drift(_value_context):

    _global_value = 0.2


class density_profile_preconditioner(_feature_flag):

    _state = True


class two_level_preconditioner(_feature_flag):

    _state = True


class truncated_preconditioner(_feature_flag):

    _state = True


class two_level_rank(_value_context):

    _global_value = 192


class fused_factor_refresh(_feature_flag):

    _state = True


class two_level_rebuild(_feature_flag):

    _state = True


class two_level_min_iters(_value_context):

    _global_value = 4.0



class two_level_subsample(_value_context):

    _global_value = 1


class two_level_lockstep(_feature_flag):

    _state = False


class two_level_growth(_value_context):

    _global_value = 1.2


class two_level_lag(_value_context):

    _global_value = 2


class spectral_factor(_feature_flag):

    _state = True


class spectral_dense_regime(_feature_flag):

    _state = True


class spectral_tail(_value_context):

    _global_value = None


class spectral_mean_tolerance(_value_context):

    _global_value = None


class graphed_hyper_step(_feature_flag):

    _state = True


class fused_hyper_columns(_feature_flag):

    _state = True


class fused_hyper_step(_feature_flag):

    _state = True



class fused_evaluate(_feature_flag):

    _state = True


class spectral_device_refresh(_feature_flag):

    _state = True


class spectral_max_rank(_value_context):

    _global_value = 1024
```

Baseline: 25.41 million.

## Fold convergence poll into keep forward kernel and re-arm deferred PCG resumes

Factors the last-block poll publication into a shared device helper. The keep-spectral forward kernel can now publish the convergence poll itself, so the standalone update launch at check points can be skipped. This path is gated by a flag that is off by default. The keep CG path is split into separate forward and backward launches, and the forward launch can be marked as already queued and then skipped. A resumed solve that has not converged can re-enter async mode (re-arm), with stream_step looping speculative absorb plus resume, to keep the host from blocking. It also switches residual accumulation to double and adds host counters for poll types. The cost is more complex state and a risk of extra loop iterations.

Result: slower. 24.98 million (-1.7%).

```diff
diff --git a/include/wiski.h b/include/wiski.h
--- a/include/wiski.h
+++ b/include/wiski.h
@@ -15,6 +15,8 @@
 #define WISKI_PENDING 1
 
 #define WISKI_MAX_DIM 4
+#define WISKI_POLL_STANDALONE 1
+#define WISKI_POLL_NO_REARM 2
 
 typedef struct wiski_grid {
   int32_t d;
@@ -117,10 +119,13 @@
   int32_t prezeroed;
   int32_t guard_ok;
   double shift;
+  int32_t fwd_queued;
+  int32_t reserved;
 } wiski_pcg_async;
 int wiski_pcg_async_f32(const wiski_grid* grid, const float* d_A_st, const float* d_tcol, float kscale, const float* d_evec, const float* d_evec2, const float* d_eval, float shift, const float* d_RHS, int32_t k, float* d_U, float* d_Z, int32_t warm, double tol, int32_t max_iter, int32_t check_every, int32_t first_check, void* d_work, int64_t work_bytes, int32_t* h_iters, double* h_relres, const int32_t* d_err, int32_t* h_err, int32_t a_sym, float* d_R, void* stream, wiski_pcg_async* handle, int32_t mode);
 int wiski_pcg_async_f64(const wiski_grid* grid, const double* d_A_st, const double* d_tcol, double kscale, const double* d_evec, const double* d_evec2, const double* d_eval, double shift, const double* d_RHS, int32_t k, double* d_U, double* d_Z, int32_t warm, double tol, int32_t max_iter, int32_t check_every, int32_t first_check, void* d_work, int64_t work_bytes, int32_t* h_iters, double* h_relres, const int32_t* d_err, int32_t* h_err, int32_t a_sym, double* d_R, void* stream, wiski_pcg_async* handle, int32_t mode);
 int wiski_pcg_async_free(wiski_pcg_async* handle);
+int wiski_pcg_poll_counts(int64_t* standalone_updates, int64_t* forward_polls);
 int wiski_pcg_async_guard(const wiski_pcg_async* handle, const void** d_guard, int64_t* expect);
 int wiski_pcg_zero_regions_f32(const wiski_grid* grid, int32_t k, int32_t max_iter, void* d_work, int32_t a_sym, void** p1, int64_t* n1_bytes, void** p2, int64_t* n2_bytes);
 int wiski_pcg_zero_regions_f64(const wiski_grid* grid, int32_t k, int32_t max_iter, void* d_work, int32_t a_sym, void** p1, int64_t* n1_bytes, void** p2, int64_t* n2_bytes);
@@ -139,6 +144,7 @@
   const wiski_shard* shard;
   const wiski_twolevel* two_level;
   int32_t keep[3];
+  int32_t poll_flags;
 } wiski_stream_args_f32;
 typedef struct wiski_stream_args_f64 {
   double* d_A_half; double* d_b; double* d_cnt; double* d_stats; int32_t* d_err;
@@ -149,6 +155,7 @@
   const wiski_shard* shard;
   const wiski_twolevel* two_level;
   int32_t keep[3];
+  int32_t poll_flags;
 } wiski_stream_args_f64;
 int wiski_stream_step_f32(const wiski_grid* grid, const wiski_stream_args_f32* args, const float* d_x, const float* d_y, const float* d_wa, const float* d_wb, const float* d_noise, int64_t q, float* d_mean_out, int32_t carry, int32_t first_check, int32_t* h_iters, double* h_relres, int32_t* h_err, void* stream, wiski_pcg_async* handle, int32_t defer, int32_t* h_resumed);
 int wiski_stream_step_f64(const wiski_grid* grid, const wiski_stream_args_f64* args, const double* d_x, const double* d_y, const double* d_wa, const double* d_wb, const double* d_noise, int64_t q, double* d_mean_out, int32_t carry, int32_t first_check, int32_t* h_iters, double* h_relres, int32_t* h_err, void* stream, wiski_pcg_async* handle, int32_t defer, int32_t* h_resumed);
diff --git a/online_gp_amd/csrc/pcg.h b/online_gp_amd/csrc/pcg.h
--- a/online_gp_amd/csrc/pcg.h
+++ b/online_gp_amd/csrc/pcg.h
@@ -23,6 +23,8 @@
   int max_iter = 0;
   int check_every = 0;
   int first_check = 0;
+  bool poll_in_forward = false;
+  bool rearm = false;
   void* work = nullptr;
   int64_t work_bytes = 0;
   int32_t* h_iters = nullptr;
diff --git a/online_gp_amd/csrc/solve.hip b/online_gp_amd/csrc/solve.hip
--- a/online_gp_amd/csrc/solve.hip
+++ b/online_gp_amd/csrc/solve.hip
@@ -2,6 +2,7 @@
 
 #include <hip/hip_ext.h>
 
+#include <atomic>
 #include <chrono>
 #include <cstdlib>
 #include <map>
@@ -1657,38 +1658,7 @@
   if (poll == nullptr) {
     if (threadIdx.x == 0) unsafeAtomicAdd(S.rn(it + 1) + c, acc);
   } else {
-    __shared__ int s_last;
-    if (threadIdx.x == 0) {
-      const double prev = atomicAdd(S.rn(it + 1) + c, acc);
-      unsigned one = 1u;
-      asm volatile("" : "+v"(one) : "v"(prev));
-      const unsigned t = atomicAdd(S.ticket(), one);
-      s_last = t == gridDim.x * gridDim.y - 1;
-    }
-    __syncthreads();
-    if (s_last) {
-      const int k = S.k;
-      int ok = 1;
-      for (int c2 = threadIdx.x; c2 < k; c2 += blockDim.x) {
-        const double r0 = __hip_atomic_load(S.rn0() + c2, __ATOMIC_RELAXED, __HIP_MEMORY_SCOPE_AGENT);
-        const double r1 = __hip_atomic_load(S.rn(it + 1) + c2, __ATOMIC_RELAXED, __HIP_MEMORY_SCOPE_AGENT);
-        poll[1 + c2] = r0;
-        poll[1 + k + c2] = r1;
-        if (r0 > 0 && r1 > tol2 * r0) ok = 0;
-      }
-      ok = __syncthreads_and(ok);
-      if (threadIdx.x == 0) {
-        const double e = err ? (double)*err : 0.0;
-        const long long gv = (ok && e == 0.0) ? seq : -seq;
-        poll[1 + 2 * k] = e;
-        poll[2 + 2 * k] = (double)gv;
-        if (guard) *guard = gv;
-        __hip_atomic_store(S.ticket(), 0u, __ATOMIC_RELAXED, __HIP_MEMORY_SCOPE_AGENT);
-      }
-      __threadfence_system();
-      __syncthreads();
-      if (threadIdx.x == 0) __hip_atomic_store(reinterpret_cast<long long*>(poll), seq, __ATOMIC_RELEASE, __HIP_MEMORY_SCOPE_SYSTEM);
-    }
+    pcg_publish_poll(S, it + 1, c, acc, gridDim.x * gridDim.y, tol2, poll, err, seq, guard);
   }
 }
 
@@ -1705,6 +1675,8 @@
     store4<real>(acc + 4 * i, (real)0, (real)0, (real)0, (real)0);
   }
 }
+
+static std::atomic<long long> g_poll_standalone{0}, g_poll_forward{0};
 
 
 struct PcgPath {
@@ -1767,6 +1739,8 @@
   dim3 egrid, vgrid;
   const double tol2;
   bool init_in_fwd;
+  bool keep_split;
+  bool poll_fwd;
 
   PcgPlan(const GridDev<real>& G_, const PcgArgs<real>& a_, const PcgPath& path_, hipStream_t s_)
       : G(G_), a(a_), path(path_), s(s_), m(G_.m), k(a_.k), L(G_.m, a_.k, a_.max_iter, a_.work), tol2(a_.tol * a_.tol) {
@@ -1791,6 +1765,8 @@
     if (vb > bcap) vb = bcap;
     vgrid = dim3((unsigned)vb, (unsigned)k);
     init_in_fwd = a.mode != 2 && a.warm == 2 && sizeof(real) == 4 && path.fused_cg;
+    keep_split = path.fused_cg && sizeof(real) == 4 && k == 1 && a.keep[0] != 0 && !path.sharded;
+    poll_fwd = keep_split && a.poll_in_forward;
   }
 
   int product_wide(const real* v, const real* add, real beta, double* dots) const {
@@ -1904,6 +1880,7 @@
     err_seen = P.h[1 + 2 * k];
   };
   bool deferred = false;
+  bool fwd_queued = false;
   auto fetch = [&](int slot, long long queued_seq = 0) -> int {
     long long seq = queued_seq;
     if (!seq) {
@@ -1915,6 +1892,7 @@
       as->state = 1;
       as->it = slot;
       as->seq = seq;
+      as->fwd_queued = fwd_queued ? 1 : 0;
       deferred = true;
       return WISKI_OK;
     }
@@ -1939,6 +1917,9 @@
     done = converged();
     first_check = it;
     mode = 0;
+    if (a.rearm && plan.keep_split && !done && it < max_iter) mode = 1;
+    fwd_queued = as->fwd_queued != 0;
+    as->fwd_queued = 0;
   }
   if (first_check < 1) first_check = check_every;
   if (first_check > max_iter) first_check = max_iter;
@@ -1947,20 +1928,40 @@
   auto flush_update = [&](bool publish = false) -> long long {
     long long seq = 0;
     if (pending) {
-      if (publish) seq = ++P.seq;
+      if (publish) { seq = ++P.seq; g_poll_standalone.fetch_add(1, std::memory_order_relaxed); }
       hipLaunchKernelGGL((k_pcg_update_x<real, 4>), plan.vgrid, dim3(256), 0, s, m, it - 1, tol2, (const real*)p, (const real*)pt, (const real*)hp,
                          cpart, cnch, czl, a.U, a.Z, r, S, publish ? P.d : (double*)nullptr, a.d_err, seq, P.g);
       pending = false;
     }
     return seq;
+  };
+  auto keep_fwd = [&](int apply, const real* rhs0, long long seq) -> int {
+    if constexpr (sizeof(real) == 4) {
+      return launch_spectral_keep_fwd(G, a.evec, r, L.sb, it, apply, tol2, p, pt, cpart, cnch, czl, a.U, a.Z, S, s, rhs0, a.two_level, a.keep,
+                                      seq ? P.d : (double*)nullptr, a.d_err, seq, P.g);
+    } else {
+      return WISKI_E_BADARG;
+    }
   };
   while (!done && it < max_iter) {
     if (plan.path.fused_cg) {
       constexpr bool fuse_upd = sizeof(real) == 4;
       if (!fuse_upd) flush_update();
       const bool init_now = plan.init_in_fwd && it == 0;
-      rc = launch_spectral_fused_cg<real>(G, a.evec, a.evec2, a.eval, a.kscale, a.shift, r, k, L.sa, L.sb, it, pending ? 1 : 0, tol2, p, pt, cpart, cnch,
-                                          czl, a.U, a.Z, S, s, init_now ? a.RHS : (const real*)nullptr, a.two_level, a.keep);
+      const real* rhs0 = init_now ? a.RHS : (const real*)nullptr;
+      if constexpr (fuse_upd) {
+        if (plan.keep_split) {
+          if (!fwd_queued) rc = keep_fwd(pending ? 1 : 0, rhs0, 0);
+          if (!rc) rc = launch_spectral_keep_bwd(G, a.evec, a.evec2, a.eval, a.kscale, a.shift, r, L.sb, it, p, pt, S, s, a.two_level, a.keep);
+          fwd_queued = false;
+        } else {
+          rc = launch_spectral_fused_cg<real>(G, a.evec, a.evec2, a.eval, a.kscale, a.shift, r, k, L.sa, L.sb, it, pending ? 1 : 0, tol2, p, pt, cpart,
+                                              cnch, czl, a.U, a.Z, S, s, rhs0, a.two_level, a.keep);
+        }
+      } else {
+        rc = launch_spectral_fused_cg<real>(G, a.evec, a.evec2, a.eval, a.kscale, a.shift, r, k, L.sa, L.sb, it, 0, tol2, p, pt, cpart, cnch, czl, a.U,
+                                            a.Z, S, s, rhs0, a.two_level, a.keep);
+      }
       pending = false;
       if (rc) return rc;
       rc = plan.product_wide(p, pt, (real)1, S.php(it));
@@ -1968,7 +1969,19 @@
       pending = true;
       ++it;
       if (due(it)) {
-        rc = fetch(it, flush_update(true));
+        long long pseq = 0;
+        if constexpr (fuse_upd) {
+          if (plan.poll_fwd) {
+            pseq = ++P.seq;
+            rc = keep_fwd(1, nullptr, pseq);
+            if (rc) return rc;
+            g_poll_forward.fetch_add(1, std::memory_order_relaxed);
+            pending = false;
+            fwd_queued = true;
+          }
+        }
+        if (!pseq) pseq = flush_update(true);
+        rc = fetch(it, pseq);
         if (rc) return rc;
         if (deferred) return WISKI_PENDING;
         done = converged();
@@ -1988,6 +2001,7 @@
     if (rc) return rc;
     const bool pub = due(it + 1);
     const long long useq = pub ? ++P.seq : 0;
+    if (pub) g_poll_standalone.fetch_add(1, std::memory_order_relaxed);
     PCG_VEC_LAUNCH(plan, k_pcg_update_x, m, it, tol2, (const real*)p, (const real*)pt, (const real*)hp, cpart, cnch, czl, a.U, a.Z, r, S,
                    pub ? P.d : (double*)nullptr, a.d_err, useq, P.g);
     ++it;
@@ -2209,9 +2223,15 @@
     as->poll = nullptr;
   }
   as->state = 0;
+  as->fwd_queued = 0;
   return WISKI_OK;
 }
 int wiski_pcg_async_guard(const wiski_pcg_async* as, const void** d_guard, int64_t* expect) { return pcg_guard(as, d_guard, expect); }
+int wiski_pcg_poll_counts(int64_t* standalone_updates, int64_t* forward_polls) {
+  if (standalone_updates) *standalone_updates = g_poll_standalone.load(std::memory_order_relaxed);
+  if (forward_polls) *forward_polls = g_poll_forward.load(std::memory_order_relaxed);
+  return WISKI_OK;
+}
 int wiski_pcg_f32(const wiski_grid* g, PCG_ABI(float), void* s) { return pcg(g, pcg_args<float>(PCG_ABI_NAMES), s); }
 int wiski_pcg_f64(const wiski_grid* g, PCG_ABI(double), void* s) { return pcg(g, pcg_args<double>(PCG_ABI_NAMES), s); }
 }
diff --git a/online_gp_amd/csrc/spectral_keep.h b/online_gp_amd/csrc/spectral_keep.h
--- a/online_gp_amd/csrc/spectral_keep.h
+++ b/online_gp_amd/csrc/spectral_keep.h
@@ -76,7 +76,9 @@
 __global__ __launch_bounds__(256) void k_keep_fwd(GridDev<float> G, KeepDev kp, const float* __restrict__ X1, const float* __restrict__ X2,
                                                   float* __restrict__ r, float* __restrict__ T, int it, int apply, double tol2,
                                                   const float* __restrict__ p, const float* __restrict__ pt, PcgScal S,
-                                                  float* __restrict__ part, int nch, int zl, float* __restrict__ u, float* __restrict__ z) {
+                                                  float* __restrict__ part, int nch, int zl, float* __restrict__ u, float* __restrict__ z,
+                                                  double* __restrict__ poll, const int32_t* __restrict__ err, long long seq,
+                                                  long long* __restrict__ guard) {
   extern __shared__ __attribute__((aligned(16))) char smem[];
   __shared__ double s_red[16];
   float* sR = reinterpret_cast<float*>(smem);
@@ -101,6 +103,7 @@
   }
   float4 tin[2];
   float rn_part = 0.f, rhs_part = 0.f;
+  double rn_upd = 0;
 #pragma unroll
   for (int q = 0; q < 2; ++q) {
     const int f = lo + t + 256 * q;
@@ -129,7 +132,10 @@
       zv.x += al * ptv.x; zv.y += al * ptv.y; zv.z += al * ptv.z; zv.w += al * ptv.w;
       float4 rv = tin[q];
       rv.x -= al * hv.x; rv.y -= al * hv.y; rv.z -= al * hv.z; rv.w -= al * hv.w;
-      rn_part += rv.x * rv.x + rv.y * rv.y + rv.z * rv.z + rv.w * rv.w;
+      rn_upd += (double)rv.x * rv.x;
+      rn_upd += (double)rv.y * rv.y;
+      rn_upd += (double)rv.z * rv.z;
+      rn_upd += (double)rv.w * rv.w;
       *reinterpret_cast<float4*>(u + e) = uv;
       *reinterpret_cast<float4*>(z + e) = zv;
       *reinterpret_cast<float4*>(r + e) = rv;
@@ -137,8 +143,9 @@
     }
   }
   if (apply) {
-    const double tot = block_reduce_sum((double)rn_part, s_red);
-    if (t == 0) unsafeAtomicAdd(S.rn(it), tot);
+    const double tot = block_reduce_sum(apply == 1 ? rn_upd : (double)rn_part, s_red);
+    if (poll != nullptr) pcg_publish_poll(S, it, 0, tot, gridDim.x * gridDim.y, tol2, poll, err, seq, guard);
+    else if (t == 0) unsafeAtomicAdd(S.rn(it), tot);
     if (apply == 2) {
       const double tot0 = block_reduce_sum((double)rhs_part, s_red);
       if (t == 0) unsafeAtomicAdd(S.rn0(), tot0);
@@ -453,28 +460,17 @@
   if (i0 == 0 && t == 0 && rho != nullptr) unsafeAtomicAdd(rho, rho_it);
 }
 
-static int launch_spectral_keep_cg(const GridDev<float>& G, const float* evec, const float* evec2, const float* evals, float kscale, float shift,
-                                   float* r, float* w1, int it, int apply, double tol2, float* p, float* pt, float* part, int nch, int zl,
-                                   float* u, float* z, PcgScal S, hipStream_t s, const float* rhs0, const wiski_twolevel* two_level, const int* keep) {
-  const int g0 = G.g[0], g1 = G.g[1], g2 = G.g[2];
-  if (!keep_counts_ok(G, keep, two_level != nullptr) || S.k != 1 || nch > 8) return WISKI_E_BADARG;
+static bool keep_launch_ok(const GridDev<float>& G, const PcgScal& S, int nch, const wiski_twolevel* two_level, const int* keep) {
+  if (!keep_counts_ok(G, keep, two_level != nullptr) || S.k != 1 || nch > 8) return false;
   if (two_level && (two_level->r < 1 || two_level->r > SPEC_TL_MAXR || !two_level->d_mask || !two_level->d_off || !two_level->d_pos || !two_level->d_N))
-    return WISKI_E_BADARG;
-  if (rhs0 && apply) return WISKI_E_BADARG;
-  if (!evec2) evec2 = evec;
-  const float *X0 = evec, *X1 = evec + g0 * g0, *X2 = X1 + g1 * g1;
-  const float *Z0 = evec2, *Z1 = evec2 + g0 * g0, *Z2 = Z1 + g1 * g1;
+    return false;
+  return true;
+}
+static KeepDev keep_dev(const GridDev<float>& G, const int* keep) {
   KeepDev kp;
   for (int q = 0; q < 3; ++q) { kp.K[q] = keep[q]; kp.o[q] = G.g[q] - keep[q]; }
-  TwoLevelDev tl{};
-  if (two_level)
-    tl = TwoLevelDev{two_level->r, two_level->nslab, (const unsigned long long*)two_level->d_mask, two_level->d_off, two_level->d_pos, two_level->d_N,
-                     nullptr, 0u};
-  const bool wide = keep[0] > 16 || keep[1] > 16 || keep[2] > 16;
-  const size_t bwd_lds = keep_bwd_lds(keep, two_level != nullptr);
-  const dim3 grd((unsigned)g0, KEEP_NS);
-  int dev = 0;
-  if (hipGetDevice(&dev) != hipSuccess) return WISKI_E_LAUNCH;
+  return kp;
+}
 #define KEEP_LDS_OPT_IN(fn, bytes)                                                                                                     \
   do {                                                                                                                                 \
     static size_t set_[16] = {0};                            \
@@ -483,32 +479,62 @@
       set_[dev & 15] = (bytes);                                                                                                        \
     }                                                                                                                                  \
   } while (0)
-  {
-    const int gm = g1 > g2 ? g1 : g2;
-    const float* pin = rhs0 ? rhs0 : p;
-    const int ap = rhs0 ? 2 : apply;
+
+int launch_spectral_keep_fwd(const GridDev<float>& G, const float* evec, float* r, float* w1, int it, int apply, double tol2, float* p, float* pt,
+                             float* part, int nch, int zl, float* u, float* z, PcgScal S, hipStream_t s, const float* rhs0,
+                             const wiski_twolevel* two_level, const int* keep, double* poll, const int32_t* err, long long seq, long long* guard) {
+  const int g0 = G.g[0], g1 = G.g[1], g2 = G.g[2];
+  if (!keep_launch_ok(G, S, nch, two_level, keep)) return WISKI_E_BADARG;
+  if (rhs0 && apply) return WISKI_E_BADARG;
+  if (poll && (apply != 1 || rhs0)) return WISKI_E_BADARG;
+  const float *X1 = evec + g0 * g0, *X2 = X1 + g1 * g1;
+  const KeepDev kp = keep_dev(G, keep);
+  const bool wide = keep[0] > 16 || keep[1] > 16 || keep[2] > 16;
+  const dim3 grd((unsigned)g0, KEEP_NS);
+  int dev = 0;
+  if (hipGetDevice(&dev) != hipSuccess) return WISKI_E_LAUNCH;
+  const int gm = g1 > g2 ? g1 : g2;
+  const float* pin = rhs0 ? rhs0 : p;
+  const int ap = rhs0 ? 2 : apply;
 #define KEEP_FWD2(KS, WW)                                                                                                                  \
   do {                                                                                                                                     \
     KEEP_LDS_OPT_IN((k_keep_fwd<KS, WW>), KEEP_FWD_LDS);                                                                                   \
     hipLaunchKernelGGL((k_keep_fwd<KS, WW>), grd, dim3(256), KEEP_FWD_LDS, s, G, kp, X1, X2, r, w1, it, ap, tol2, pin, (const float*)pt, S, \
-                       part, nch, zl, u, z);                                                                                               \
+                       part, nch, zl, u, z, poll, err, seq, guard);                                                                        \
   } while (0)
 #define KEEP_FWD(KS, VW_UNUSED)          \
   do {                                   \
     if (wide) KEEP_FWD2(KS, 32);         \
     else KEEP_FWD2(KS, 16);              \
   } while (0)
-    SPEC_DISPATCH_KS_VW(gm, true, KEEP_FWD);
+  SPEC_DISPATCH_KS_VW(gm, true, KEEP_FWD);
 #undef KEEP_FWD
 #undef KEEP_FWD2
-    if (hipGetLastError() != hipSuccess) return WISKI_E_LAUNCH;
-  }
-  {
+  return hipGetLastError() == hipSuccess ? WISKI_OK : WISKI_E_LAUNCH;
+}
+
+int launch_spectral_keep_bwd(const GridDev<float>& G, const float* evec, const float* evec2, const float* evals, float kscale, float shift,
+                             const float* r, const float* w1, int it, float* p, float* pt, PcgScal S, hipStream_t s,
+                             const wiski_twolevel* two_level, const int* keep) {
+  const int g0 = G.g[0], g1 = G.g[1];
+  if (!keep_launch_ok(G, S, 0, two_level, keep)) return WISKI_E_BADARG;
+  if (!evec2) evec2 = evec;
+  const float *X0 = evec, *X1 = evec + g0 * g0, *X2 = X1 + g1 * g1;
+  const float *Z0 = evec2, *Z1 = evec2 + g0 * g0, *Z2 = Z1 + g1 * g1;
+  const KeepDev kp = keep_dev(G, keep);
+  TwoLevelDev tl{};
+  if (two_level)
+    tl = TwoLevelDev{two_level->r, two_level->nslab, (const unsigned long long*)two_level->d_mask, two_level->d_off, two_level->d_pos, two_level->d_N,
+                     nullptr, 0u};
+  const bool wide = keep[0] > 16 || keep[1] > 16 || keep[2] > 16;
+  const size_t bwd_lds = keep_bwd_lds(keep, two_level != nullptr);
+  int dev = 0;
+  if (hipGetDevice(&dev) != hipSuccess) return WISKI_E_LAUNCH;
 #define KEEP_BWD3(KS, KSK, TLV)                                                                                                          \
   do {                                                                                                                                   \
     KEEP_LDS_OPT_IN((k_keep_bwd<KS, KSK, TLV>), bwd_lds);                                                                                \
     hipLaunchKernelGGL((k_keep_bwd<KS, KSK, TLV>), dim3((unsigned)g0), dim3(1024), bwd_lds, s, G, kp, X0, Z0, X1, X2, Z1, Z2, evals, kscale, \
-                       shift, (const float*)w1, (const float*)r, p, pt, it, S, S.rho(it), tl);                                           \
+                       shift, w1, r, p, pt, it, S, S.rho(it), tl);                                                                       \
   } while (0)
 #define KEEP_BWD(KS, VW_UNUSED)                    \
   do {                                             \
@@ -520,10 +546,18 @@
       else KEEP_BWD3(KS, 4, false);                \
     }                                              \
   } while (0)
-    SPEC_DISPATCH_KS_VW(g0, true, KEEP_BWD);
+  SPEC_DISPATCH_KS_VW(g0, true, KEEP_BWD);
 #undef KEEP_BWD
 #undef KEEP_BWD3
-  }
+  return hipGetLastError() == hipSuccess ? WISKI_OK : WISKI_E_LAUNCH;
+}
 #undef KEEP_LDS_OPT_IN
-  return hipGetLastError() == hipSuccess ? WISKI_OK : WISKI_E_LAUNCH;
-}
+
+static int launch_spectral_keep_cg(const GridDev<float>& G, const float* evec, const float* evec2, const float* evals, float kscale, float shift,
+                                   float* r, float* w1, int it, int apply, double tol2, float* p, float* pt, float* part, int nch, int zl,
+                                   float* u, float* z, PcgScal S, hipStream_t s, const float* rhs0, const wiski_twolevel* two_level, const int* keep) {
+  if (int rc = launch_spectral_keep_fwd(G, evec, r, w1, it, apply, tol2, p, pt, part, nch, zl, u, z, S, s, rhs0, two_level, keep, nullptr, nullptr, 0,
+                                        nullptr))
+    return rc;
+  return launch_spectral_keep_bwd(G, evec, evec2, evals, kscale, shift, r, w1, it, p, pt, S, s, two_level, keep);
+}
diff --git a/online_gp_amd/csrc/stream_step.hip b/online_gp_amd/csrc/stream_step.hip
--- a/online_gp_amd/csrc/stream_step.hip
+++ b/online_gp_amd/csrc/stream_step.hip
@@ -34,6 +34,7 @@
   for (int q = 0; q < 3; ++q) p.keep[q] = a->keep[q];
   p.U = a->d_U; p.Z = a->d_Z; p.R = a->d_R; p.warm = carry ? 2 : 1;
   p.tol = a->tol; p.max_iter = a->max_iter; p.check_every = a->check_every; p.first_check = first_check;
+  p.poll_in_forward = (a->poll_flags & WISKI_POLL_STANDALONE) == 0;
   p.work = a->d_work; p.work_bytes = a->work_bytes;
   p.d_err = a->d_err;
   p.shard = a->shard;
@@ -56,23 +57,25 @@
   bool absorbed = false;
   if (as && as->state == 1) {
     bool spec = false;
-    if (q > 0 && d_mean_out) {
-      const void* guard = nullptr;
-      int64_t expect = 0;
-      if (pcg_guard(as, &guard, &expect) == WISKI_OK) {
-        AbsorbArgs<real> spec_batch = batch;
-        spec_batch.guard = guard; spec_batch.guard_expect = expect;
-        rc = absorb_batch<real>(grid, a, spec_batch, carry, 1, stream);
-        if (rc) return rc;
-        spec = true;
+    do {
+      spec = false;
+      if (q > 0 && d_mean_out) {
+        const void* guard = nullptr;
+        int64_t expect = 0;
+        if (pcg_guard(as, &guard, &expect) == WISKI_OK) {
+          AbsorbArgs<real> spec_batch = batch;
+          spec_batch.guard = guard; spec_batch.guard_expect = expect;
+          rc = absorb_batch<real>(grid, a, spec_batch, carry, 1, stream);
+          if (rc) return rc;
+          spec = true;
+        }
       }
-    }
-    {
       PcgArgs<real> resume = solve;
       resume.shift = (real)as->shift;
       resume.mode = 2;
+      resume.rearm = spec && (a->poll_flags & WISKI_POLL_NO_REARM) == 0;
       rc = pcg(grid, resume, stream);
-    }
+    } while (rc == WISKI_PENDING && as->state == 1);
     if (h_resumed) *h_resumed = 1;
     if (rc != WISKI_OK && rc != WISKI_E_NOTCONV) return rc;
     absorbed = spec && as->guard_ok;
diff --git a/online_gp_amd/csrc/wiski_common.h b/online_gp_amd/csrc/wiski_common.h
--- a/online_gp_amd/csrc/wiski_common.h
+++ b/online_gp_amd/csrc/wiski_common.h
@@ -262,6 +262,43 @@
   return rn0 > 0 && S.rn(it)[c] > tol2 * rn0;
 }
 
+__device__ __forceinline__ void pcg_publish_poll(const PcgScal& S, int slot, int c, double acc, unsigned nblocks, double tol2,
+                                                 double* __restrict__ poll, const int32_t* __restrict__ err, long long seq,
+                                                 long long* __restrict__ guard) {
+  __shared__ int s_last;
+  if (threadIdx.x == 0) {
+    const double prev = atomicAdd(S.rn(slot) + c, acc);
+    unsigned one = 1u;
+    asm volatile("" : "+v"(one) : "v"(prev));
+    const unsigned t = atomicAdd(S.ticket(), one);
+    s_last = t == nblocks - 1;
+  }
+  __syncthreads();
+  if (s_last) {
+    const int k = S.k;
+    int ok = 1;
+    for (int c2 = threadIdx.x; c2 < k; c2 += blockDim.x) {
+      const double r0 = __hip_atomic_load(S.rn0() + c2, __ATOMIC_RELAXED, __HIP_MEMORY_SCOPE_AGENT);
+      const double r1 = __hip_atomic_load(S.rn(slot) + c2, __ATOMIC_RELAXED, __HIP_MEMORY_SCOPE_AGENT);
+      poll[1 + c2] = r0;
+      poll[1 + k + c2] = r1;
+      if (r0 > 0 && r1 > tol2 * r0) ok = 0;
+    }
+    ok = __syncthreads_and(ok);
+    if (threadIdx.x == 0) {
+      const double e = err ? (double)*err : 0.0;
+      const long long gv = (ok && e == 0.0) ? seq : -seq;
+      poll[1 + 2 * k] = e;
+      poll[2 + 2 * k] = (double)gv;
+      if (guard) *guard = gv;
+      __hip_atomic_store(S.ticket(), 0u, __ATOMIC_RELAXED, __HIP_MEMORY_SCOPE_AGENT);
+    }
+    __threadfence_system();
+    __syncthreads();
+    if (threadIdx.x == 0) __hip_atomic_store(reinterpret_cast<long long*>(poll), seq, __ATOMIC_RELEASE, __HIP_MEMORY_SCOPE_SYSTEM);
+  }
+}
+
 template <typename real>
 bool spectral_fused_ok(const GridDev<real>& G);
 template <typename real>
@@ -273,4 +310,10 @@
                              int k, real* w0, real* w1, int it, int apply, double tol2, real* p, real* pt, real* part, int nch, int zl, real* u,
                              real* z, PcgScal S, hipStream_t s, const real* rhs0 = nullptr, const wiski_twolevel* two_level = nullptr,
                              const int* keep = nullptr);
+int launch_spectral_keep_fwd(const GridDev<float>& G, const float* evec, float* r, float* w1, int it, int apply, double tol2, float* p, float* pt,
+                             float* part, int nch, int zl, float* u, float* z, PcgScal S, hipStream_t s, const float* rhs0,
+                             const wiski_twolevel* two_level, const int* keep, double* poll, const int32_t* err, long long seq, long long* guard);
+int launch_spectral_keep_bwd(const GridDev<float>& G, const float* evec, const float* evec2, const float* evals, float kscale, float shift,
+                             const float* r, const float* w1, int it, float* p, float* pt, PcgScal S, hipStream_t s,
+                             const wiski_twolevel* two_level, const int* keep);
 bool spectral_keep_ok(const GridDev<float>& G, const int* keep, bool two_level);
diff --git a/online_gp_amd/grid_ops.py b/online_gp_amd/grid_ops.py
--- a/online_gp_amd/grid_ops.py
+++ b/online_gp_amd/grid_ops.py
@@ -6,7 +6,7 @@
 
 import torch
 
-from . import _hip
+from . import _hip, settings
 
 
 class GridSpec:
@@ -731,7 +731,7 @@
                 ("d_eval", ctypes.c_void_p), ("shift", ctypes.c_float), ("tol", ctypes.c_double), ("max_iter", ctypes.c_int32),
                 ("check_every", ctypes.c_int32), ("d_work", ctypes.c_void_p), ("work_bytes", ctypes.c_int64),
                 ("d_bin", ctypes.c_void_p), ("bin_bytes", ctypes.c_int64), ("shard", ctypes.c_void_p), ("two_level", ctypes.c_void_p),
-                ("keep", ctypes.c_int32 * 3)]
+                ("keep", ctypes.c_int32 * 3), ("poll_flags", ctypes.c_int32)]
 
 
 ALLREDUCE_FN = ctypes.CFUNCTYPE(ctypes.c_int, ctypes.c_void_p, ctypes.c_void_p, ctypes.c_int64, ctypes.c_int32, ctypes.c_void_p, ctypes.c_int64,
@@ -769,7 +769,14 @@
 
 class _PcgAsync(ctypes.Structure):
     _fields_ = [("state", ctypes.c_int32), ("it", ctypes.c_int32), ("seq", ctypes.c_int64), ("poll", ctypes.c_void_p),
-                ("prezeroed", ctypes.c_int32), ("guard_ok", ctypes.c_int32), ("shift", ctypes.c_double)]
+                ("prezeroed", ctypes.c_int32), ("guard_ok", ctypes.c_int32), ("shift", ctypes.c_double), ("fwd_queued", ctypes.c_int32),
+                ("reserved", ctypes.c_int32)]
+
+
+def pcg_poll_counts():
+    a, b = ctypes.c_int64(0), ctypes.c_int64(0)
+    _hip.check(_hip.lib().wiski_pcg_poll_counts(ctypes.byref(a), ctypes.byref(b)), "wiski_pcg_poll_counts")
+    return int(a.value), int(b.value)
 
 
 class StreamStep:
@@ -855,6 +862,7 @@
                 self.args.d_bin, self.args.bin_bytes = self.bin_buf.data_ptr(), need
         use_handle = defer or self.pending
         self.herr.value = 0
+        self.args.poll_flags = (0 if settings.poll_in_forward.on() else 1) | (0 if settings.poll_rearm.on() else 2)
         rc = self.fn(self.grid.ref, ctypes.byref(self.args), _hip.dptr(x), _hip.dptr(y), _hip.dptr(wa), _hip.dptr(wb), _hip.dptr(noise),
                      ctypes.c_int64(q), _hip.dptr(mean_out), ctypes.c_int32(int(carry)), ctypes.c_int32(int(first_check)), ctypes.byref(self.it),
                      ctypes.byref(self.rr), ctypes.byref(self.herr), _hip.stream_ptr(self.device),
diff --git a/online_gp_amd/settings.py b/online_gp_amd/settings.py
--- a/online_gp_amd/settings.py
+++ b/online_gp_amd/settings.py
@@ -172,6 +172,16 @@
     _state = True
 
 
+class poll_in_forward(_feature_flag):
+
+    _state = False
+
+
+class poll_rearm(_feature_flag):
+
+    _state = True
+
+
 class two_level_rank(_value_context):
 
     _global_value = 192
```
